# jie0530/act-plus-plus

Measured on AMD Instinct MI355X. Metric: policy steps/sec (4x480x640 cams, chunk=100, bs=8), higher is better.
Workload: dtype f32 (f16x3 split products: 3 fp16 MFMAs per fp32 product, fp32 accumulate); 1 GPU; ACT eval policy query: 4 cams 480x640 u8, chunk 100, hidden 512, ff 3200, 4 enc + 7 dec layers (layer 0 live), per-GPU batch 8, + temporal ensemble; per_gpu_batch=8, global_batch=8, parallelism=replicas x1

## Files before the change

act-plus-plus_amd/actmi/lib.py:

```python
import ctypes as C
import os

import torch

_HERE = os.path.dirname(os.path.abspath(__file__))
LIB_PATH = os.environ.get("ACTMI_LIB") or os.path.join(_HERE, "libactmi.so")

IMG_U8_NHWC = 0
IMG_F32_NCHW = 1


class ActmiConfig(C.Structure):
    _fields_ = [("struct_size", C.c_uint32)] + [(n, C.c_int32) for n in (
        "num_cams", "image_h", "image_w", "base_width", "hidden_dim", "nheads", "dim_feedforward", "enc_layers",
        "dec_layers", "num_queries", "state_dim", "action_dim", "latent_dim", "has_cvae_encoder", "max_batch",
        "enable_training")] + [("kl_weight", C.c_float)] + [(n, C.c_int32) for n in ("vq", "vq_class", "vq_dim")]


class ActmiPcdConfig(C.Structure):
    _fields_ = [("struct_size", C.c_uint32), ("max_points", C.c_int32), ("hidden_dim", C.c_int32), ("output_dim", C.c_int32)]


class GemmDesc(C.Structure):
    _fields_ = [
        ("A", C.c_void_p), ("lda", C.c_int64), ("mode", C.c_int32),
        ("H", C.c_int32), ("W", C.c_int32), ("Cin", C.c_int32), ("KH", C.c_int32), ("KW", C.c_int32),
        ("stride", C.c_int32), ("pad", C.c_int32), ("Ho", C.c_int32), ("Wo", C.c_int32),
        ("img_stride", C.c_int64),
        ("A_add", C.c_void_p), ("ld_add", C.c_int64), ("add_mod", C.c_int32), ("add_ncols", C.c_int32),
        ("Bw", C.c_void_p), ("ldb", C.c_int64),
        ("scale", C.c_void_p), ("bias", C.c_void_p), ("res", C.c_void_p), ("ldres", C.c_int64),
        ("res_mod", C.c_int32), ("relu", C.c_int32),
        ("C", C.c_void_p), ("ldc", C.c_int64), ("rowmap", C.c_void_p),
        ("M", C.c_int32), ("N", C.c_int32), ("K", C.c_int32), ("groups", C.c_int32),
        ("gA", C.c_int64), ("gB", C.c_int64), ("gSB", C.c_int64), ("gC", C.c_int64), ("gRes", C.c_int64),
        ("ta", C.c_int32), ("tb", C.c_int32), ("a_rowmap", C.c_void_p),
        ("B_add", C.c_void_p), ("ld_badd", C.c_int64), ("badd_mod", C.c_int32), ("splitk", C.c_int32),
        ("mask", C.c_void_p), ("ldmask", C.c_int64), ("C2", C.c_void_p), ("scale2", C.c_void_p),
        ("alpha", C.c_float), ("groups_inner", C.c_int32),
        ("gA2", C.c_int64), ("gB2", C.c_int64), ("gC2", C.c_int64), ("gRes2", C.c_int64),
        ("gMask", C.c_int64), ("gC2out", C.c_int64),
        ("drop_p", C.c_float), ("drop_seed", C.c_uint64), ("stamps", C.c_void_p), ("prec", C.c_int32), ("b_split", C.c_int32), ("b_scale", C.c_float), ("a_scale", C.c_float), ("a_scale_dev", C.c_void_p), ("b_scale_dev", C.c_void_p),
        ("split_stride", C.c_int64), ("amax_out", C.c_void_p),
        ("epi", C.c_int32), ("epi_scale", C.c_float), ("epi_row", C.c_void_p), ("gRow", C.c_int64), ("gRow2", C.c_int64),
        ("epi_colkill", C.c_void_p), ("gColkill", C.c_int64), ("tile_hint", C.c_int32),
        ("finite_flag", C.c_void_p), ("finite_bit", C.c_uint32),
        ("Ax", C.c_void_p), ("kx_begin", C.c_int32), ("Hx", C.c_int32), ("Wx", C.c_int32), ("Cx", C.c_int32),
        ("stride_x", C.c_int32), ("gAx", C.c_int64),
        ("A_alt", C.c_void_p), ("alt_ncols", C.c_int32), ("k_tap_inner", C.c_int32),
    ]


class AttnBwdDesc(C.Structure):
    _fields_ = [("q", C.c_void_p), ("k", C.c_void_p), ("v", C.c_void_p), ("o", C.c_void_p), ("d_o", C.c_void_p), ("lse", C.c_void_p),
                ("dq", C.c_void_p), ("dk", C.c_void_p), ("dv", C.c_void_p)] + \
               [(n, C.c_int64) for n in ("q_bs", "q_rs", "k_bs", "k_rs", "v_bs", "v_rs", "dq_bs", "dq_rs", "dk_bs", "dk_rs", "dv_bs", "dv_rs")] + \
               [("kpm", C.c_void_p), ("kpm_bs", C.c_int64)] + [(n, C.c_int32) for n in ("B", "H", "Nq", "Nk", "HD")] + \
               [("drop_p", C.c_float), ("drop_seed", C.c_uint64), ("delta_ws", C.c_void_p), ("do_scale", C.c_void_p), ("amax_out", C.c_void_p)]


class AttnDesc(C.Structure):
    _fields_ = [
        ("Q", C.c_void_p), ("q_bs", C.c_int64), ("q_rs", C.c_int64),
        ("K", C.c_void_p), ("k_bs", C.c_int64), ("k_rs", C.c_int64),
        ("V", C.c_void_p), ("v_bs", C.c_int64), ("v_rs", C.c_int64),
        ("O", C.c_void_p), ("o_bs", C.c_int64), ("o_rs", C.c_int64),
        ("kpm", C.c_void_p), ("kpm_bs", C.c_int64), ("lse", C.c_void_p),
        ("B", C.c_int32), ("H", C.c_int32), ("Nq", C.c_int32), ("Nk", C.c_int32), ("HD", C.c_int32),
        ("scale", C.c_float), ("ws", C.c_void_p), ("ws_floats", C.c_int64),
        ("drop_p", C.c_float), ("drop_seed", C.c_uint64), ("prec", C.c_int32), ("causal", C.c_int32),
    ]


_lib = None


def load():
    global _lib
    if _lib is not None:
        return _lib
    if not os.path.isfile(LIB_PATH):
        raise RuntimeError(
            f"{LIB_PATH} is missing: build the HIP extension first (python -c 'import __graft_entry__ as g; g.build()' "
            "or make -C act-plus-plus_amd/csrc). There is no CPU fallback for the ACT path.")
    lib = C.CDLL(LIB_PATH)
    vp, i32, i64, f32, f64 = C.c_void_p, C.c_int32, C.c_int64, C.c_float, C.c_double
    sigs = {
        "actmi_version": ([], i32),
        "actmi_create": ([C.POINTER(ActmiConfig), C.POINTER(vp)], i32),
        "actmi_create_ex": ([C.POINTER(ActmiConfig), C.POINTER(ActmiPcdConfig), C.POINTER(vp)], i32),
        "actmi_set_pointcloud": ([vp, vp, vp, i32, i32], i32),
        "actmi_destroy": ([vp], i32),
        "actmi_last_error": ([vp], C.c_char_p),
        "actmi_num_params": ([vp], i32),
        "actmi_param_info": ([vp, i32, C.POINTER(C.c_char_p), C.POINTER(i64), C.POINTER(i32), C.POINTER(i32)], i32),
        "actmi_set_param": ([vp, C.c_char_p, vp, C.POINTER(i64), i32, i32], i32),
        "actmi_get_param": ([vp, C.c_char_p, vp, i64, i32], i32),
        "actmi_param_ptr": ([vp, C.c_char_p, C.POINTER(vp), C.POINTER(i64)], i32),
        "actmi_finalize": ([vp, vp], i32),
        "actmi_set_forward_phase": ([vp, i32], i32),
        "actmi_forward_infer_vq": ([vp, vp, vp, i32, i32, vp, vp, vp], i32),
        "actmi_forward_infer": ([vp, vp, vp, i32, i32, vp, vp], i32),
        "actmi_forward_train": ([vp, vp, vp, i32, vp, vp, vp, C.c_uint64, f32, i32, vp, vp, vp, vp, vp], i32),
        "actmi_backward": ([vp, f32, vp], i32),
        "actmi_zero_grad": ([vp, vp], i32),
        "actmi_adamw_step": ([vp, f32, f32, f32, f32, f32, f32, i64, vp], i32),
        "actmi_adamw_step_range": ([vp, f32, f32, f32, f32, f32, f32, i64, i64, i64, vp], i32),
        "actmi_refresh_weights": ([vp, vp], i32),
        "actmi_param_arena": ([vp, C.POINTER(vp), C.POINTER(i64)], i32),
        "actmi_grad_ptr": ([vp, C.c_char_p, C.POINTER(vp), C.POINTER(i64)], i32),
        "actmi_grad_arena": ([vp, C.POINTER(vp), C.POINTER(i64)], i32),
        "actmi_grad_phase_range": ([vp, i32, C.POINTER(i64), C.POINTER(i64)], i32),
        "actmi_wait_grad_phase": ([vp, i32, vp], i32),
        "actmi_ensemble_step": ([vp, vp, vp, f64, vp, vp, i32, i32, i32, vp], i32),
        "actmi_op_gemm": ([C.POINTER(GemmDesc), vp], i32),
        "actmi_op_split16": ([vp, vp, C.c_int64, C.c_float, vp], i32),
        "actmi_op_permute_conv_k": ([vp, vp, C.c_int64, i32, i32, i32, vp], i32),
        "actmi_op_sample_onehot": ([vp, i32, i32, C.c_float, C.c_uint64, vp, vp, vp], i32),
        "actmi_op_pow2_scale": ([vp, C.c_int64, i32, i32, vp, vp], i32),
        "actmi_op_splitk_combine": ([vp, i32, C.c_int64, C.c_int64, i32, i32, vp, vp, vp, C.c_int64, i32, vp, C.c_int64, vp], i32),
        "actmi_op_attention": ([C.POINTER(AttnDesc), vp], i32),
        "actmi_op_attention_bwd": ([C.POINTER(AttnBwdDesc), vp], i32),
        "actmi_op_layernorm": ([vp, vp, i32, vp, vp, vp, vp, vp, i32, i32, f32, vp], i32),
        "actmi_op_maxpool3x3s2": ([vp, vp, i32, i32, i32, i32, vp], i32),
        "actmi_op_conv1": ([vp, i32, vp, vp, vp, vp, vp, i32, i32, i32, i32, i32, i32, vp], i32),
        "actmi_op_conv1_workspace_floats": ([i32, i32], C.c_int64),
        "actmi_op_conv1_prepare": ([vp, vp, i32, i32, i32, vp], i32),
        "actmi_op_conv1_prepared": ([vp, vp, vp, vp, vp, i32, i32, i32, i32, i32, i32, vp], i32),
        "actmi_op_conv3x3_c64": ([vp, vp, C.c_float, vp, vp, vp, vp, i32, i32, i32, i32, i32, vp], i32),
        "actmi_op_conv3x3_c64_dgrad": ([vp, vp, C.c_float, vp, vp, vp, vp, vp, vp, i32, i32, i32, i32, vp], i32),
        "actmi_op_wgrad7x7s2": ([vp, vp, vp, vp, C.c_int64, vp, i32, i32, i32, i32, vp], i32),
        "actmi_op_wgrad3x3_c64": ([vp, vp, vp, vp, C.c_int64, vp, i32, i32, i32, i32, vp], i32),
        "actmi_op_groupnorm": ([vp, vp, vp, vp, vp, vp, vp, i32, i32, i32, i32, f32, i32, i32, vp, C.c_int64, vp], i32),
        "actmi_op_spatial_softmax": ([vp, vp, i32, i32, i32, i32, f32, vp], i32),
        "actmi_op_unfold1d": ([vp, vp, i32, i32, i32, i32, i32, i32, i32, i32, vp], i32),
        "actmi_op_ddim_step": ([vp, vp, C.c_int64, f32, f32, f32, f32, i32, vp], i32),
        "actmi_op_mish": ([vp, vp, C.c_int64, vp], i32),
        "actmi_op_gelu": ([vp, vp, C.c_int64, vp], i32),
        "actmi_op_gelu_bwd": ([vp, vp, vp, C.c_int64, vp], i32),
        "actmi_op_dropout": ([vp, vp, C.c_int64, C.c_float, C.c_uint64, vp], i32),
        "actmi_op_small_attention": ([vp, vp, i32, i32, i32, i32, i32, C.c_float, C.c_uint64, vp], i32),
        "actmi_op_small_attention_bwd": ([vp, vp, vp, i32, i32, i32, i32, i32, C.c_float, C.c_uint64, vp], i32),
        "actmi_op_soft_ce_dim1": ([vp, vp, i32, i32, i32, vp, vp, vp, vp], i32),
        "actmi_op_argmax_l1": ([vp, vp, i32, i32, vp, vp, vp], i32),
        "actmi_op_layernorm_bwd": ([vp, vp, vp, vp, vp, vp, vp, i32, i32, C.c_float, vp, C.c_int64, vp], i32),
        "actmi_op_colsum": ([vp, C.c_int64, vp, i32, i32, vp, C.c_int64, vp], i32),
        "actmi_op_pcd_embed": ([vp, vp, vp, vp, vp, C.c_int64, i32, vp], i32),
        "actmi_op_colmax": ([vp, i32, i32, i32, C.c_int64, vp, vp, vp, C.c_int64, vp], i32),
        "actmi_op_sum_batch": ([vp, C.c_int64, C.c_int64, vp, i32, i32, i32, i32, vp], i32),
        "actmi_op_adamw": ([vp, vp, vp, vp, C.c_int64, C.c_float, C.c_float, C.c_float, C.c_float, C.c_float, C.c_int64, vp], i32),
        "actmi_op_u8_to_nhwc4": ([vp, vp, i32, i32, i32, i32, vp], i32),
        "actmi_op_last_error": ([], C.c_char_p),
        "actmi_debug_tensor": ([vp, C.c_char_p, C.POINTER(vp), C.POINTER(i64)], i32),
        "actmi_debug_stop_after": ([vp, C.c_char_p], i32),
        "actmi_set_gemm_prec": ([vp, i32], i32),
        "actmi_set_train_prec": ([vp, i32], i32),
        "actmi_get_flags": ([vp, C.POINTER(C.c_uint32), i32, vp], i32),
        "actmi_flags_ptr": ([vp, C.POINTER(vp)], i32),
        "actmi_profile_enable": ([i32], i32),
        "actmi_profile_reset": ([], i32),
        "actmi_profile_report": ([C.c_char_p, i32], i32),
    }
    for name, (args, res) in sigs.items():
        fn = getattr(lib, name)
        fn.argtypes = args
        fn.restype = res
    _lib = lib
    return lib


def declared_symbols(header_path):
    import re
    txt = open(header_path).read()
    return sorted(set(re.findall(r"\b(actmi_[a-z0-9_]+)\s*\(", txt)))


def current_stream_ptr():
    return C.c_void_p(torch.cuda.current_stream().cuda_stream)


def check(rc, handle=None, what=""):
    if rc != 0:
        lib = load()
        msg = lib.actmi_last_error(handle) if handle is not None else lib.actmi_op_last_error()
        raise RuntimeError(f"libactmi {what} failed (code {rc}): {msg.decode() if msg else ''}")


def profile_enable(on: bool):
    lib = load()
    lib.actmi_profile_reset() if on else None
    lib.actmi_profile_enable(1 if on else 0)


def profile_report():
    import json
    lib = load()
    buf = C.create_string_buffer(1 << 18)
    rc = lib.actmi_profile_report(buf, len(buf))
    if rc != 0:
        raise RuntimeError(f"actmi_profile_report failed ({rc})")
    return json.loads(buf.value.decode())
```

act-plus-plus_amd/actmi/ops.py:

```python
import ctypes as C

import torch

from . import lib as L


def _p(t):
    return C.c_void_p(t.data_ptr()) if t is not None else C.c_void_p(0)


PREC = {None: 0, "f32": 1, "f16x3": 2, "bf16": 3}


def split16(w, scale=1.0):
    lib = L.load()
    w = w.contiguous()
    out = torch.empty_like(w)
    L.check(lib.actmi_op_split16(_p(w), _p(out), w.numel(), float(scale), L.current_stream_ptr()), None, "op_split16")
    return out


def permute_conv_k(w_rows, taps, cin):
    lib = L.load()
    w_rows = w_rows.contiguous()
    out = torch.empty_like(w_rows)
    rows, ld = w_rows.numel() // w_rows.shape[-1], w_rows.shape[-1]
    L.check(lib.actmi_op_permute_conv_k(_p(w_rows), _p(out), rows, int(taps), int(cin), int(ld), L.current_stream_ptr()), None,
            "op_permute_conv_k")
    return out


def pow2_scale(x):
    lib = L.load()
    assert x.dim() == 2 and x.stride(1) == 1
    out = torch.zeros(2, dtype=torch.float32, device=x.device)
    L.check(lib.actmi_op_pow2_scale(_p(x), x.stride(0), x.shape[0], x.shape[1], _p(out), L.current_stream_ptr()), None,
            "op_pow2_scale")
    return out


def auto_splitk(M, N, K):
    tiles = ((M + 63) // 64) * ((N + 63) // 64)
    nk = (K + 31) // 32
    if tiles >= 768 or nk < 24:
        return 0
    s = min(8, (1536 + tiles - 1) // tiles, nk // 12)
    while s >= 2 and (s - 1) * ((nk + s - 1) // s) >= nk:
        s -= 1
    return s if s >= 2 else 0


def gemm(A, W, bias=None, scale=None, res=None, res_mod=0, relu=False, a_add=None, add_mod=0, add_ncols=0, rowmap=None,
         out=None, out_rows=None, drop_p=0.0, drop_seed=0, prec=None, w_split=False, a_scale=0.0, b_scale=0.0,
         a_scale_dev=None, b_scale_dev=None, splitk=0):
    lib = L.load()
    M, K = A.shape
    N = W.shape[0]
    if splitk == "auto":
        splitk = auto_splitk(M, N, K) if (rowmap is None and not res_mod and not drop_p and N % 4 == 0 and a_scale_dev is None
                                          and b_scale_dev is None) else 0
    if splitk and splitk > 1:
        assert rowmap is None and not res_mod and not drop_p
        part = torch.empty((splitk, M, N), dtype=torch.float32, device=A.device)
        d = L.GemmDesc()
        d.A, d.lda, d.mode = A.data_ptr(), A.stride(0), 0
        if a_add is not None:
            d.A_add, d.ld_add, d.add_mod, d.add_ncols = a_add.data_ptr(), a_add.stride(0), add_mod, add_ncols
        d.Bw, d.ldb = W.data_ptr(), W.stride(0)
        d.C, d.ldc = part.data_ptr(), N
        d.M, d.N, d.K, d.groups = M, N, K, 1
        d.splitk, d.split_stride = int(splitk), M * N
        d.prec, d.b_split, d.b_scale = PREC[prec], 1 if w_split else 0, float(w_split) if w_split else float(b_scale)
        d.a_scale = float(a_scale)
        L.check(lib.actmi_op_gemm(C.byref(d), L.current_stream_ptr()), None, "op_gemm")
        if out is None:
            out = torch.empty((M, N), dtype=torch.float32, device=A.device)
        L.check(lib.actmi_op_splitk_combine(part.data_ptr(), int(splitk), M * N, N, M, N, _p(scale), _p(bias), _p(res),
                                            res.stride(0) if res is not None else 0,
                                            2 if relu == "gelu" else (1 if relu else 0), out.data_ptr(), out.stride(0),
                                            L.current_stream_ptr()), None, "op_splitk_combine")
        return out
    if out is None:
        out = torch.zeros((out_rows or M, N), dtype=torch.float32, device=A.device)
    d = L.GemmDesc()
    d.A, d.lda, d.mode = A.data_ptr(), A.stride(0), 0
    if a_add is not None:
        d.A_add, d.ld_add, d.add_mod, d.add_ncols = a_add.data_ptr(), a_add.stride(0), add_mod, add_ncols
    d.Bw, d.ldb = W.data_ptr(), W.stride(0)
    d.scale = scale.data_ptr() if scale is not None else None
    d.bias = bias.data_ptr() if bias is not None else None
    if res is not None:
        d.res, d.ldres, d.res_mod = res.data_ptr(), res.stride(0), res_mod
    d.relu = 2 if relu == "gelu" else (1 if relu else 0)
    d.C, d.ldc = out.data_ptr(), out.stride(0)
    d.rowmap = rowmap.data_ptr() if rowmap is not None else None
    d.M, d.N, d.K, d.groups = M, N, K, 1
    d.drop_p, d.drop_seed = float(drop_p), int(drop_seed)
    d.prec, d.b_split, d.b_scale = PREC[prec], 1 if w_split else 0, float(w_split) if w_split else float(b_scale)
    d.a_scale = float(a_scale)
    d.a_scale_dev = a_scale_dev.data_ptr() if a_scale_dev is not None else None
    d.b_scale_dev = b_scale_dev.data_ptr() if b_scale_dev is not None else None
    L.check(lib.actmi_op_gemm(C.byref(d), L.current_stream_ptr()), None, "op_gemm")
    return out


def conv2d_with_second_source(y1, x, wf_split, w_scale, bias, stride_x=2, relu=True, splitk=0, k_tap_inner=False):
    lib = L.load()
    G, B, H, W, Cc = y1.shape
    _, _, Hx, Wx, Cx = x.shape
    Cout = wf_split.shape[1]
    Kf = 9 * Cc + Cx
    assert wf_split.numel() == G * Cout * Kf
    M = B * H * W

    def desc(C_ptr, ldc, gC):
        d = L.GemmDesc()
        d.A, d.mode = y1.data_ptr(), 1
        d.H, d.W, d.Cin, d.KH, d.KW, d.stride, d.pad, d.Ho, d.Wo = H, W, Cc, 3, 3, 1, 1, H, W
        d.img_stride = H * W * Cc
        d.Ax, d.kx_begin, d.Hx, d.Wx, d.Cx, d.stride_x, d.gAx = x.data_ptr(), 9 * Cc, Hx, Wx, Cx, stride_x, B * Hx * Wx * Cx
        d.Bw, d.ldb = wf_split.data_ptr(), Kf
        d.C, d.ldc = C_ptr, ldc
        d.M, d.N, d.K, d.groups = M, Cout, Kf, G
        d.gA, d.gB, d.gSB, d.gC = B * H * W * Cc, Cout * Kf, Cout, gC
        d.prec, d.b_split, d.b_scale = PREC["f16x3"], 1, float(w_scale)
        d.k_tap_inner = 1 if k_tap_inner else 0
        return d
    out = torch.empty((G, B, H, W, Cout), dtype=torch.float32, device=y1.device)
    if splitk and splitk > 1:
        part = torch.empty((G, splitk, M, Cout), dtype=torch.float32, device=y1.device)
        d = desc(part.data_ptr(), Cout, splitk * M * Cout)
        d.splitk, d.split_stride = int(splitk), M * Cout
        L.check(lib.actmi_op_gemm(C.byref(d), L.current_stream_ptr()), None, "op_gemm(conv + second source, split)")
        for g in range(G):
            L.check(lib.actmi_op_splitk_combine(part[g].data_ptr(), int(splitk), M * Cout, Cout, M, Cout, None, _p(bias[g]), None, 0,
                                                1 if relu else 0, out[g].data_ptr(), Cout, L.current_stream_ptr()), None, "combine")
        return out
    d = desc(out.data_ptr(), Cout, M * Cout)
    d.bias = bias.data_ptr()
    d.relu = 1 if relu else 0
    L.check(lib.actmi_op_gemm(C.byref(d), L.current_stream_ptr()), None, "op_gemm(conv + second source)")
    return out


def conv2d_nhwc(x, w_ohwi, scale=None, bias=None, res=None, relu=False, stride=1, pad=1, prec=None, w_split=False, b_scale=0.0,
                k_tap_inner=False):
    lib = L.load()
    G, B, H, W, Cin = x.shape
    _, Cout, KH, KW, _ = w_ohwi.shape
    Ho, Wo = (H + 2 * pad - KH) // stride + 1, (W + 2 * pad - KW) // stride + 1
    out = torch.empty((G, B, Ho, Wo, Cout), dtype=torch.float32, device=x.device)
    d = L.GemmDesc()
    d.A, d.mode = x.data_ptr(), 1
    d.H, d.W, d.Cin, d.KH, d.KW, d.stride, d.pad, d.Ho, d.Wo = H, W, Cin, KH, KW, stride, pad, Ho, Wo
    d.img_stride = H * W * Cin
    d.Bw, d.ldb = w_ohwi.data_ptr(), KH * KW * Cin
    d.scale = scale.data_ptr() if scale is not None else None
    d.bias = bias.data_ptr() if bias is not None else None
    if res is not None:
        d.res, d.ldres = res.data_ptr(), Cout
    d.relu = 1 if relu else 0
    d.C, d.ldc = out.data_ptr(), Cout
    d.M, d.N, d.K, d.groups = B * Ho * Wo, Cout, KH * KW * Cin, G
    d.gA, d.gB, d.gSB = B * H * W * Cin, Cout * KH * KW * Cin, Cout
    d.gC = d.gRes = B * Ho * Wo * Cout
    d.prec, d.b_split, d.b_scale = PREC[prec], 1 if w_split else 0, float(w_split) if w_split else float(b_scale)
    d.k_tap_inner = 1 if k_tap_inner else 0
    L.check(lib.actmi_op_gemm(C.byref(d), L.current_stream_ptr()), None, "op_gemm(conv)")
    return out


def sample_onehot(logits, temperature=1.0, seed=0, want_probs=False):
    lib = L.load()
    logits = logits.contiguous()
    n, V = logits.shape
    code = torch.empty_like(logits)
    probs = torch.empty_like(logits) if want_probs else None
    L.check(lib.actmi_op_sample_onehot(_p(logits), n, V, float(temperature), C.c_uint64(int(seed)), _p(probs), _p(code),
                                       L.current_stream_ptr()), None, "op_sample_onehot")
    return (code, probs) if want_probs else code


def conv1_prepare(w_oihw, lut_mode=1):
    lib = L.load()
    w_oihw = w_oihw.contiguous()
    Cc, Cout = w_oihw.shape[0], w_oihw.shape[1]
    ws = torch.zeros(int(lib.actmi_op_conv1_workspace_floats(Cc, Cout)), dtype=torch.float32, device=w_oihw.device)
    L.check(lib.actmi_op_conv1_prepare(_p(w_oihw), _p(ws), Cc, Cout, int(lut_mode), L.current_stream_ptr()), None, "op_conv1_prepare")
    return ws


def conv1_prepared(image_u8, ws, Cout, relu=False, scale=None, bias=None):
    lib = L.load()
    image_u8 = image_u8.contiguous()
    B, Cc, H, W, _ = image_u8.shape
    out = torch.empty((Cc, B, (H - 1) // 2 + 1, (W - 1) // 2 + 1, Cout), dtype=torch.float32, device=image_u8.device)
    L.check(lib.actmi_op_conv1_prepared(_p(image_u8), _p(ws), _p(scale), _p(bias), _p(out), B, Cc, H, W, Cout, 1 if relu else 0,
                                        L.current_stream_ptr()), None, "op_conv1_prepared")
    return out


def conv3x3_c64(x, w_ohwi, scale=None, bias=None, res=None, relu=False, w_scale=256.0, w16=None):
    lib = L.load()
    G, B, H, W, Cin = x.shape
    assert Cin == 64 and tuple(w_ohwi.shape[1:]) == (64, 3, 3, 64)
    out = torch.empty_like(x)
    if w16 is None:
        w16 = split16(w_ohwi, w_scale)
    scale = scale if scale is not None else torch.ones(G, 64, device=x.device)
    bias = bias if bias is not None else torch.zeros(G, 64, device=x.device)
    L.check(lib.actmi_op_conv3x3_c64(_p(x.contiguous()), _p(w16), float(w_scale), _p(scale.contiguous()), _p(bias.contiguous()),
                                     _p(res), _p(out), G, B, H, W, 1 if relu else 0, L.current_stream_ptr()), None,
            "op_conv3x3_c64")
    return out


def conv3x3_c64_dgrad(dy, wd_ohwi, dy_scale=None, res=None, mask=None, post_scale=None, amax_out=None, w_scale=256.0):
    lib = L.load()
    G, B, H, W, Cc = dy.shape
    assert Cc == 64 and tuple(wd_ohwi.shape[1:]) == (64, 3, 3, 64)
    dy = dy.contiguous()
    dx = torch.empty_like(dy)
    for t in (res, mask):
        assert t is None or (t.shape == dy.shape and t.is_contiguous())
    assert post_scale is None or (tuple(post_scale.shape) == (G, 64) and post_scale.is_contiguous())
    w16 = split16(wd_ohwi, w_scale)
    L.check(lib.actmi_op_conv3x3_c64_dgrad(_p(dy), _p(w16), float(w_scale), _p(dy_scale), _p(res),
                                           _p(mask), _p(post_scale), _p(amax_out), _p(dx), G, B, H, W, L.current_stream_ptr()),
            None, "op_conv3x3_c64_dgrad")
    return dx


def wgrad3x3_c64(dy, x, dy_scale=None):
    G, B, H, W, Cc = x.shape
    assert Cc == 64 and dy.shape == x.shape
    nwg = max(1, min(256 // G, B * ((W + 31) // 32)))
    ws = torch.empty(G * nwg * 64 * 576, device=x.device, dtype=torch.float32)
    dw = torch.empty(G, 64, 3, 3, 64, device=x.device, dtype=torch.float32)
    lib = L.load()
    L.check(lib.actmi_op_wgrad3x3_c64(_p(dy.contiguous()), _p(x.contiguous()), _p(dw), _p(ws), ws.numel(),
                                      _p(dy_scale) if dy_scale is not None else None, G, B, H, W, L.current_stream_ptr()),
            None, "op_wgrad3x3_c64")
    return dw


def wgrad7x7s2(dy, x4, dy_scale=None):
    G, B, H, W, Cc = x4.shape
    Ho, Wo = (H - 1) // 2 + 1, (W - 1) // 2 + 1
    assert Cc == 4 and tuple(dy.shape) == (G, B, Ho, Wo, 64)
    nwg = max(1, min(512 // G, B * ((Wo + 31) // 32)))
    ws = torch.empty(G * nwg * 64 * 196, device=x4.device, dtype=torch.float32)
    dw = torch.empty(G, 64, 7, 7, 4, device=x4.device, dtype=torch.float32)
    lib = L.load()
    L.check(lib.actmi_op_wgrad7x7s2(_p(dy.contiguous()), _p(x4.contiguous()), _p(dw), _p(ws), ws.numel(),
                                    _p(dy_scale) if dy_scale is not None else None, G, B, H, W, L.current_stream_ptr()),
            None, "op_wgrad7x7s2")
    return dw



def attention(q, k, v, nheads, kpm=None, q_shared=False, want_lse=False, split=True, drop_p=0.0, drop_seed=0, prec=None,
              causal=False):
    lib = L.load()
    B, Nk, D = k.shape
    Nq = q.shape[-2]
    hd = D // nheads
    out = torch.zeros((B, Nq, D), dtype=torch.float32, device=k.device)
    lse = torch.zeros((B, nheads, Nq), dtype=torch.float32, device=k.device) if want_lse else None
    d = L.AttnDesc()
    d.Q, d.q_bs, d.q_rs = q.data_ptr(), (0 if q_shared else q.stride(0)), q.stride(-2)
    d.K, d.k_bs, d.k_rs = k.data_ptr(), k.stride(0), k.stride(1)
    d.V, d.v_bs, d.v_rs = v.data_ptr(), v.stride(0), v.stride(1)
    d.O, d.o_bs, d.o_rs = out.data_ptr(), out.stride(0), out.stride(1)
    if kpm is not None:
        d.kpm, d.kpm_bs = kpm.data_ptr(), kpm.stride(0)
    d.lse = lse.data_ptr() if lse is not None else None
    if split:
        ws = torch.empty(8 * B * Nq * (D + 2 * nheads), dtype=torch.float32, device=k.device)
        d.ws, d.ws_floats = ws.data_ptr(), ws.numel()
    d.B, d.H, d.Nq, d.Nk, d.HD = B, nheads, Nq, Nk, hd
    d.scale = 1.0 / (hd ** 0.5)
    d.drop_p, d.drop_seed = float(drop_p), int(drop_seed)
    d.prec = PREC[prec]
    d.causal = 1 if causal else 0
    L.check(lib.actmi_op_attention(C.byref(d), L.current_stream_ptr()), None, "op_attention")
    return (out, lse) if want_lse else out


def attention_bwd(q, k, v, out, lse, dout, nheads, kpm=None, drop_p=0.0, drop_seed=0, do_scale=None, want_amax=False):
    lib = L.load()
    B, Nk, D = k.shape
    Nq = q.shape[1]
    dq = torch.empty((B, Nq, D), dtype=torch.float32, device=k.device)
    dk = torch.empty((B, Nk, D), dtype=torch.float32, device=k.device)
    dv = torch.empty((B, Nk, D), dtype=torch.float32, device=k.device)
    ws = torch.empty(B * nheads * Nq, dtype=torch.float32, device=k.device)
    amax = torch.zeros(1, dtype=torch.int32, device=k.device) if want_amax else None
    d = L.AttnBwdDesc()
    d.q, d.q_bs, d.q_rs = q.data_ptr(), q.stride(0), q.stride(1)
    d.k, d.k_bs, d.k_rs = k.data_ptr(), k.stride(0), k.stride(1)
    d.v, d.v_bs, d.v_rs = v.data_ptr(), v.stride(0), v.stride(1)
    d.o, d.d_o, d.lse = out.data_ptr(), dout.data_ptr(), lse.data_ptr()
    d.dq, d.dq_bs, d.dq_rs = dq.data_ptr(), dq.stride(0), dq.stride(1)
    d.dk, d.dk_bs, d.dk_rs = dk.data_ptr(), dk.stride(0), dk.stride(1)
    d.dv, d.dv_bs, d.dv_rs = dv.data_ptr(), dv.stride(0), dv.stride(1)
    if kpm is not None:
        d.kpm, d.kpm_bs = kpm.data_ptr(), kpm.stride(0)
    d.B, d.H, d.Nq, d.Nk, d.HD = B, nheads, Nq, Nk, D // nheads
    d.drop_p, d.drop_seed = float(drop_p), int(drop_seed)
    d.delta_ws = ws.data_ptr()
    d.do_scale = do_scale.data_ptr() if do_scale is not None else None
    d.amax_out = amax.data_ptr() if amax is not None else None
    L.check(lib.actmi_op_attention_bwd(C.byref(d), L.current_stream_ptr()), None, "op_attention_bwd")
    return (dq, dk, dv, amax) if want_amax else (dq, dk, dv)


def layernorm(x, w, b, res=None, res_mod=0, w2=None, b2=None, eps=1e-5):
    lib = L.load()
    M, D = x.shape
    y = torch.empty_like(x)
    L.check(lib.actmi_op_layernorm(_p(x), _p(res), res_mod, _p(w), _p(b), _p(w2), _p(b2), _p(y), M, D, eps,
                                   L.current_stream_ptr()), None, "op_layernorm")
    return y


def maxpool3x3s2(x):
    lib = L.load()
    n, H, W, Cc = x.shape
    Ho, Wo = (H + 2 - 3) // 2 + 1, (W + 2 - 3) // 2 + 1
    y = torch.empty((n, Ho, Wo, Cc), dtype=torch.float32, device=x.device)
    L.check(lib.actmi_op_maxpool3x3s2(_p(x), _p(y), n, H, W, Cc, L.current_stream_ptr()), None, "op_maxpool")
    return y


def conv1(image, w_oihw, scale, bias, prec=None):
    lib = L.load()
    image = image.contiguous()
    if image.dtype == torch.uint8:
        B, Cn, H, W, _ = image.shape
        fmt = L.IMG_U8_NHWC
    else:
        B, Cn, _, H, W = image.shape
        fmt = L.IMG_F32_NCHW
    Cout = w_oihw.shape[1]
    Ho, Wo = (H + 6 - 7) // 2 + 1, (W + 6 - 7) // 2 + 1
    out = torch.zeros((Cn, B, Ho, Wo, Cout), dtype=torch.float32, device=image.device)
    ws = torch.empty(Cn * Cout * 148 + 768, dtype=torch.float32, device=image.device)
    L.check(lib.actmi_op_conv1(_p(image), fmt, _p(w_oihw), _p(scale), _p(bias), _p(out), _p(ws), B, Cn, H, W, Cout,
                               PREC[prec], L.current_stream_ptr()), None, "op_conv1")
    return out


ACT = {None: 0, "none": 0, "relu": 1, "mish": 2}


_GN_WS = {}


def groupnorm(x, weight, bias, groups, eps=1e-5, act=None, res=None, res_after=False, film=None, out=None):
    lib = L.load()
    x = x.contiguous()
    n, Cc = x.shape[0], x.shape[-1]
    P = x.numel() // (n * Cc)
    if out is None:
        out = torch.empty_like(x)
    assert out.is_contiguous() and out.shape == x.shape
    fs, fb = (film[0].contiguous(), film[1].contiguous()) if film is not None else (None, None)
    rm = 0 if res is None else (2 if res_after else 1)
    key = (x.device, torch.cuda.current_stream(x.device).cuda_stream)
    ws = _GN_WS.get(key)
    if ws is None:
        ws = _GN_WS[key] = torch.empty(1 << 20, dtype=torch.float32, device=x.device)
    L.check(lib.actmi_op_groupnorm(_p(x), _p(res.contiguous() if res is not None else None), _p(fs), _p(fb), _p(weight), _p(bias),
                                   _p(out), n, P, Cc, int(groups), float(eps), ACT[act], rm, _p(ws), ws.numel(),
                                   L.current_stream_ptr()), None, "op_groupnorm")
    return out


def spatial_softmax(logits, H, W, temperature=1.0):
    lib = L.load()
    logits = logits.contiguous()
    n, P, K = logits.shape
    assert P == H * W
    out = torch.empty((n, K, 2), dtype=torch.float32, device=logits.device)
    L.check(lib.actmi_op_spatial_softmax(_p(logits), _p(out), n, H, W, K, float(temperature), L.current_stream_ptr()), None,
            "op_spatial_softmax")
    return out


def unfold1d(x, k, stride=1, pad=0, transposed=False):
    lib = L.load()
    x = x.contiguous()
    B, T, Cc = x.shape
    To = (T - 1) * stride - 2 * pad + k if transposed else (T + 2 * pad - k) // stride + 1
    out = torch.empty((B, To, k * Cc), dtype=torch.float32, device=x.device)
    L.check(lib.actmi_op_unfold1d(_p(x), _p(out), B, T, Cc, k, stride, pad, To, 1 if transposed else 0, L.current_stream_ptr()),
            None, "op_unfold1d")
    return out


def ddim_step(x, eps, alpha_t, alpha_prev, clip=True):
    lib = L.load()
    assert x.is_contiguous() and eps.is_contiguous() and x.numel() == eps.numel()
    L.check(lib.actmi_op_ddim_step(_p(x), _p(eps), x.numel(), float(alpha_t ** -0.5), float((1.0 - alpha_t) ** 0.5),
                                   float(alpha_prev ** 0.5), float(max(0.0, 1.0 - alpha_prev) ** 0.5), 1 if clip else 0,
                                   L.current_stream_ptr()), None, "op_ddim_step")
    return x


def mish(x):
    lib = L.load()
    x = x.contiguous()
    y = torch.empty_like(x)
    L.check(lib.actmi_op_mish(_p(x), _p(y), x.numel(), L.current_stream_ptr()), None, "op_mish")
    return y


def u8_to_nhwc4(image_u8):
    lib = L.load()
    image_u8 = image_u8.contiguous()
    B, Cam, H, W, _ = image_u8.shape
    out = torch.empty((Cam, B, H, W, 4), dtype=torch.float32, device=image_u8.device)
    L.check(lib.actmi_op_u8_to_nhwc4(_p(image_u8), _p(out), B, Cam, H, W, L.current_stream_ptr()), None, "op_u8_to_nhwc4")
    return out


def gemm_t(A, Bm, ta=False, tb=False, bias=None, res=None, out=None, prec="f32"):
    lib = L.load()
    if ta:
        K, M = A.shape
    else:
        M, K = A.shape
    N = Bm.shape[1] if tb else Bm.shape[0]
    assert (Bm.shape[0] if tb else Bm.shape[1]) == K, (A.shape, Bm.shape, ta, tb)
    if out is None:
        out = torch.empty((M, N), dtype=torch.float32, device=A.device)
    d = L.GemmDesc()
    d.A, d.lda, d.mode, d.ta = A.data_ptr(), A.stride(0), 0, 1 if ta else 0
    d.Bw, d.ldb, d.tb = Bm.data_ptr(), Bm.stride(0), 1 if tb else 0
    d.bias = bias.data_ptr() if bias is not None else None
    if res is not None:
        d.res, d.ldres = res.data_ptr(), res.stride(0)
    d.C, d.ldc = out.data_ptr(), out.stride(0)
    d.M, d.N, d.K, d.groups = M, N, K, 1
    d.prec = PREC[prec]
    L.check(lib.actmi_op_gemm(C.byref(d), L.current_stream_ptr()), None, "op_gemm")
    return out


def gelu(x):
    y = torch.empty_like(x)
    L.check(L.load().actmi_op_gelu(_p(x), _p(y), x.numel(), L.current_stream_ptr()), None, "op_gelu")
    return y


def gelu_bwd(x, dy):
    dx = torch.empty_like(x)
    L.check(L.load().actmi_op_gelu_bwd(_p(x), _p(dy), _p(dx), x.numel(), L.current_stream_ptr()), None, "op_gelu_bwd")
    return dx


def dropout(x, p, seed):
    y = torch.empty_like(x)
    L.check(L.load().actmi_op_dropout(_p(x), _p(y), x.numel(), float(p), int(seed), L.current_stream_ptr()), None, "op_dropout")
    return y


def small_attention(qkv, nheads, causal=True, drop_p=0.0, seed=0):
    n, T, D3 = qkv.shape
    D = D3 // 3
    out = torch.empty((n, T, D), dtype=torch.float32, device=qkv.device)
    L.check(L.load().actmi_op_small_attention(_p(qkv), _p(out), n, T, nheads, D // nheads, 1 if causal else 0, float(drop_p), int(seed),
                                              L.current_stream_ptr()), None, "op_small_attention")
    return out


def small_attention_bwd(qkv, dout, nheads, causal=True, drop_p=0.0, seed=0):
    n, T, D3 = qkv.shape
    D = D3 // 3
    dqkv = torch.empty_like(qkv)
    L.check(L.load().actmi_op_small_attention_bwd(_p(qkv), _p(dout), _p(dqkv), n, T, nheads, D // nheads, 1 if causal else 0,
                                                  float(drop_p), int(seed), L.current_stream_ptr()), None, "op_small_attention_bwd")
    return dqkv


def soft_ce_dim1(logits, target, want_grad=True):
    B, T, V = logits.shape
    loss = torch.empty(1, dtype=torch.float32, device=logits.device)
    ws = torch.empty(B * V, dtype=torch.float32, device=logits.device)
    dl = torch.empty_like(logits) if want_grad else None
    L.check(L.load().actmi_op_soft_ce_dim1(_p(logits), _p(target), B, T, V, _p(loss), _p(dl), _p(ws), L.current_stream_ptr()), None,
            "op_soft_ce_dim1")
    return loss, dl


def argmax_l1(logits, target):
    V = logits.shape[-1]
    rows = logits.numel() // V
    out = torch.empty(1, dtype=torch.float32, device=logits.device)
    ws = torch.empty(rows, dtype=torch.float32, device=logits.device)
    L.check(L.load().actmi_op_argmax_l1(_p(logits), _p(target), rows, V, _p(out), _p(ws), L.current_stream_ptr()), None, "op_argmax_l1")
    return out


def layernorm_bwd(x, w, dy, dw, db, ws, dx_add=None, eps=1e-5):
    M, D = x.shape
    dx = torch.empty_like(x)
    L.check(L.load().actmi_op_layernorm_bwd(_p(x), _p(w), _p(dy), _p(dx_add), _p(dx), _p(dw), _p(db), M, D, eps, _p(ws), ws.numel(),
                                            L.current_stream_ptr()), None, "op_layernorm_bwd")
    return dx


def colsum(src, out, ws):
    M, N = src.shape
    L.check(L.load().actmi_op_colsum(_p(src), src.stride(0), _p(out), M, N, _p(ws), ws.numel(), L.current_stream_ptr()), None, "op_colsum")


def pcd_embed(xyz, rgb, w0, b0):
    xyz, rgb = xyz.contiguous().view(-1, 3), rgb.contiguous().view(-1, 3)
    rows, H = xyz.shape[0], w0.shape[0]
    out = torch.empty((rows, H), dtype=torch.float32, device=xyz.device)
    L.check(L.load().actmi_op_pcd_embed(_p(xyz), _p(rgb), _p(w0.contiguous()), _p(b0.contiguous()), _p(out), rows, H,
                                        L.current_stream_ptr()), None, "op_pcd_embed")
    return out


def colmax(x, O=None, split=True):
    B, P, ld = x.shape
    O = ld if O is None else O
    out = torch.empty((B, O), dtype=torch.float32, device=x.device)
    arg = torch.empty((B, O), dtype=torch.int32, device=x.device)
    ws = torch.empty(2 * B * 64 * O, dtype=torch.float32, device=x.device) if split else None
    L.check(L.load().actmi_op_colmax(_p(x), B, P, O, ld, _p(out), _p(arg), _p(ws), ws.numel() if split else 0,
                                     L.current_stream_ptr()), None, "op_colmax")
    return out, arg


def sum_batch(src, dst, accumulate=False):
    B, Rr, D = src.shape
    L.check(L.load().actmi_op_sum_batch(_p(src), src.stride(0), src.stride(1), _p(dst), B, Rr, D, 1 if accumulate else 0,
                                        L.current_stream_ptr()), None, "op_sum_batch")


def adamw(p, g, m, v, lr, weight_decay, step, betas=(0.9, 0.999), eps=1e-8):
    L.check(L.load().actmi_op_adamw(_p(p), _p(g), _p(m), _p(v), p.numel(), float(lr), float(weight_decay), float(betas[0]),
                                    float(betas[1]), float(eps), int(step), L.current_stream_ptr()), None, "op_adamw")


class TemporalEnsemble:

    def __init__(self, num_episodes, num_queries, action_dim=16, k=0.01, device="cuda:0"):
        self.E, self.Q, self.A, self.k = num_episodes, num_queries, action_dim, float(k)
        self.ring = torch.zeros((self.E, self.Q, self.Q, self.A), dtype=torch.float32, device=device)
        self.t = torch.zeros((self.E,), dtype=torch.int32, device=device)
        self.out = torch.zeros((self.E, self.A), dtype=torch.float64, device=device)
        self.populated = torch.zeros((self.E, self.Q), dtype=torch.uint8, device=device)

    def reset(self):
        self.ring.zero_()
        self.t.zero_()

    def step(self, all_actions):
        lib = L.load()
        a = all_actions.contiguous()
        dev = self.ring.device
        if a.device != dev:
            raise ValueError(f"all_actions lives on {a.device} but this ensemble is bound to {dev}")
        with torch.cuda.device(dev):
            L.check(lib.actmi_ensemble_step(_p(self.ring), _p(self.t), _p(a), self.k, _p(self.out), _p(self.populated),
                                            self.E, self.Q, self.A, L.current_stream_ptr()), None, "ensemble_step")
        return self.out
```

act-plus-plus_amd/csrc/attn.hip:

```cpp
#include "common.h"
#include "dropout.h"
#include "split16.h"
#include <cstdio>
#include <cstdlib>

namespace {

constexpr bool ATTN_NOPF = true;
constexpr int KT = 64;
typedef _Float16 h16x8 __attribute__((ext_vector_type(8)));

__device__ __forceinline__ void attn_block_coords(int& bx, int& by, int& bz) {
    const int gx = gridDim.x, gy = gridDim.y;
    const int total = gx * gy * (int)gridDim.z;
    const int lin = ((int)blockIdx.z * gy + (int)blockIdx.y) * gx + (int)blockIdx.x;
    const int xcd = lin & 7, q = total >> 3, r = total & 7;
    const int base = (xcd < r) ? xcd * (q + 1) : r * (q + 1) + (xcd - r) * q;
    const int flat = base + (lin >> 3);
    bx = flat % gx;
    const int rest = flat / gx;
    by = rest % gy;
    bz = rest / gy;
}

template <int HD>
__global__ __launch_bounds__(256) void attn_f32_kernel(AttnArgs p, int nsplit, int chunk) {
    constexpr int HH = HD / 2;
    constexpr int DT = (HD + 31) / 32;
    constexpr int VD = DT * 32;
    constexpr int KS = HD + 4;
    __shared__ __attribute__((aligned(16))) float s_k[KT * KS];
    __shared__ __attribute__((aligned(16))) float s_v[KT * VD];

    const int t = threadIdx.x, lane = t & 63, wave = t >> 6;
    const int li = lane & 31, lh = lane >> 5;
    int bx, h, b;
    attn_block_coords(bx, h, b);
    const int split = bx % nsplit;
    const int q = (bx / nsplit) * 128 + wave * 32 + li;
    const int k_begin = split * chunk;
    const int k_end = (k_begin + chunk < p.Nk) ? k_begin + chunk : p.Nk;
    const bool qok = q < p.Nq;

    const float qscale = p.scale * 1.4426950408889634f;
    const float* Qp = p.Q + (int64_t)b * p.q_bs + (int64_t)(qok ? q : 0) * p.q_rs + h * HD + lh * HH;
    float qreg[HH];
#pragma unroll
    for (int s = 0; s < HH; s += 4) {
        f32x4 v = *reinterpret_cast<const f32x4*>(Qp + s);
#pragma unroll
        for (int j = 0; j < 4; ++j) qreg[s + j] = qok ? v[j] * qscale : 0.f;
    }
    const float* Kb = p.K + (int64_t)b * p.k_bs + h * HD;
    const float* Vb = p.V + (int64_t)b * p.v_bs + h * HD;
    const uint8_t* kpm = p.kpm ? p.kpm + (int64_t)b * p.kpm_bs : nullptr;

    f32x16 O[DT];
#pragma unroll
    for (int d = 0; d < DT; ++d)
#pragma unroll
        for (int e = 0; e < 16; ++e) O[d][e] = 0.f;
    float m_run = -INFINITY, l_run = 0.f;

    if (HD < VD) {
        for (int e = t; e < KT * VD; e += 256) s_v[e] = 0.f;
        __syncthreads();
    }

    __shared__ uint8_t s_dead[KT];
    constexpr int C4 = HD / 4;
    constexpr int NLD = (KT * C4 + 255) / 256;
    f32x4 pk[NLD], pv[NLD];
    auto fetch = [&](int kt0) {
#pragma unroll
        for (int i = 0; i < NLD; ++i) {
            const int e = t + 256 * i;
            const int kr = e / C4, c = e - kr * C4;
            const int key = kt0 + kr;
            const bool ok = e < KT * C4 && key < k_end;
            const int64_t koff = ok ? (int64_t)key * p.k_rs + c * 4 : 0;
            const int64_t voff = ok ? (int64_t)key * p.v_rs + c * 4 : 0;
            const f32x4 kv = *reinterpret_cast<const f32x4*>(Kb + koff);
            const f32x4 vv = *reinterpret_cast<const f32x4*>(Vb + voff);
            const f32x4 z = {0.f, 0.f, 0.f, 0.f};
            pk[i] = ok ? kv : z;
            pv[i] = ok ? vv : z;
        }
    };
    fetch(k_begin);
    for (int kt0 = k_begin; kt0 < k_end; kt0 += KT) {
#pragma unroll
        for (int i = 0; i < NLD; ++i) {
            const int e = t + 256 * i;
            if (e < KT * C4) {
                const int kr = e / C4, c = e - kr * C4;
                *reinterpret_cast<f32x4*>(&s_k[kr * KS + c * 4]) = pk[i];
                *reinterpret_cast<f32x4*>(&s_v[kr * VD + c * 4]) = pv[i];
            }
        }
        const bool ragged = kt0 + KT > k_end || kpm != nullptr;
        if (ragged && t < KT) {
            const int key = kt0 + t;
            s_dead[t] = (key >= k_end) || (kpm && kpm[key] != 0);
        }
        __syncthreads();
        if (kt0 + KT < k_end) fetch(kt0 + KT);
#pragma unroll
        for (int sub = 0; sub < KT / 32; ++sub) {
            const int kb = kt0 + sub * 32;
            if (kb < k_end) {
                f32x16 S;
#pragma unroll
                for (int e = 0; e < 16; ++e) S[e] = 0.f;
                const float* krow = &s_k[(sub * 32 + li) * KS + lh * HH];
#pragma unroll
                for (int s = 0; s < HH; s += 4) {
                    const f32x4 kv = *reinterpret_cast<const f32x4*>(krow + s);
#pragma unroll
                    for (int j = 0; j < 4; ++j)
                        S = __builtin_amdgcn_mfma_f32_32x32x2f32(kv[j], qreg[s + j], S, 0, 0, 0);
                }
                if (ragged) {
#pragma unroll
                    for (int e = 0; e < 16; ++e)
                        if (s_dead[sub * 32 + (e & 3) + 8 * (e >> 2) + 4 * lh]) S[e] = -INFINITY;
                }
                if (p.causal) {
#pragma unroll
                    for (int e = 0; e < 16; ++e)
                        if (kb + (e & 3) + 8 * (e >> 2) + 4 * lh > q) S[e] = -INFINITY;
                }
                float mt = S[0];
#pragma unroll
                for (int e = 1; e < 16; ++e) mt = fmaxf(mt, S[e]);
                mt = fmaxf(mt, __shfl_xor(mt, 32, 64));
                const float m_new = fmaxf(m_run, mt);
                const float m_safe = (m_new == -INFINITY) ? 0.f : m_new;
                const float alpha = __builtin_amdgcn_exp2f(m_run - m_safe);
                float rs = 0.f;
#pragma unroll
                for (int e = 0; e < 16; ++e) {
                    S[e] = __builtin_amdgcn_exp2f(S[e] - m_safe);
                    rs += S[e];
                }
                rs += __shfl_xor(rs, 32, 64);
                l_run = l_run * alpha + rs;
                m_run = m_new;
                if (p.drop_p > 0.f) {
                    const float ds = 1.f / (1.f - p.drop_p);
                    const uint64_t rowbase = (((uint64_t)b * p.H + h) * p.Nq + (qok ? q : 0)) * (uint64_t)p.Nk;
#pragma unroll
                    for (int e = 0; e < 16; ++e) {
                        const int key = kb + (e & 3) + 8 * (e >> 2) + 4 * lh;
                        S[e] = actmi_keep(p.drop_seed, rowbase + key, p.drop_p) ? S[e] * ds : 0.f;
                    }
                }
#pragma unroll
                for (int d = 0; d < DT; ++d)
#pragma unroll
                    for (int e = 0; e < 16; ++e) O[d][e] *= alpha;
#pragma unroll
                for (int e = 0; e < 16; ++e) {
                    const int kl = sub * 32 + (e & 3) + 8 * (e >> 2) + 4 * lh;
#pragma unroll
                    for (int d = 0; d < DT; ++d) {
                        const float vv = s_v[kl * VD + d * 32 + li];
                        O[d] = __builtin_amdgcn_mfma_f32_32x32x2f32(vv, S[e], O[d], 0, 0, 0);
                    }
                }
            }
        }
        __syncthreads();
    }
    if (qok) {
        if (nsplit == 1) {
            const float inv = 1.f / l_run;
            float* Op = p.O + (int64_t)b * p.o_bs + (int64_t)q * p.o_rs + h * HD;
#pragma unroll
            for (int d = 0; d < DT; ++d)
#pragma unroll
                for (int g = 0; g < 4; ++g) {
                    const int d0 = d * 32 + 8 * g + 4 * lh;
                    if (d0 < HD) {
                        f32x4 o = {O[d][4 * g] * inv, O[d][4 * g + 1] * inv, O[d][4 * g + 2] * inv, O[d][4 * g + 3] * inv};
                        *reinterpret_cast<f32x4*>(Op + d0) = o;
                    }
                }
            if (p.lse && lh == 0) p.lse[((int64_t)b * p.H + h) * p.Nq + q] = m_run * 0.6931471805599453f + logf(l_run);
        } else {
            const int64_t row = (((int64_t)split * p.B + b) * p.H + h) * p.Nq + q;
            float* Op = p.ws + row * HD;
            float* ml = p.ws + (int64_t)nsplit * p.B * p.H * p.Nq * HD + row * 2;
#pragma unroll
            for (int d = 0; d < DT; ++d)
#pragma unroll
                for (int g = 0; g < 4; ++g) {
                    const int d0 = d * 32 + 8 * g + 4 * lh;
                    if (d0 < HD) {
                        f32x4 o = {O[d][4 * g], O[d][4 * g + 1], O[d][4 * g + 2], O[d][4 * g + 3]};
                        *reinterpret_cast<f32x4*>(Op + d0) = o;
                    }
                }
            if (lh == 0) { ml[0] = m_run; ml[1] = l_run; }
        }
    }
}

template <int HD>
__global__ __launch_bounds__(256, 3) void attn_f16x3_kernel(AttnArgs p, int nsplit, int chunk) {
    constexpr int NS = HD / 16;
    constexpr int DT = (HD + 31) / 32;
    constexpr int VD = DT * 32;
    constexpr int KROW = 4 * HD + 16;
    constexpr int VROW = 4 * KT + 16;
    __shared__ __attribute__((aligned(16))) unsigned char s_k[KT * KROW];
    __shared__ __attribute__((aligned(16))) unsigned char s_vt[VD * VROW];
    __shared__ uint8_t s_dead[KT];

    const int t = threadIdx.x, lane = t & 63, wave = t >> 6;
    const int li = lane & 31, lh = lane >> 5;
    int bx, h, b;
    attn_block_coords(bx, h, b);
    const int split = bx % nsplit;
    const int q = (bx / nsplit) * 128 + wave * 32 + li;
    const int k_begin = split * chunk;
    const int k_end = (k_begin + chunk < p.Nk) ? k_begin + chunk : p.Nk;
    const bool qok = q < p.Nq;

    const float qscale = p.scale * 1.4426950408889634f;
    const float* Qp = p.Q + (int64_t)b * p.q_bs + (int64_t)(qok ? q : 0) * p.q_rs + h * HD + lh * 8;
    h16x8 qh[NS], ql[NS];
#pragma unroll
    for (int s = 0; s < NS; ++s) {
        f32x4 v0 = *reinterpret_cast<const f32x4*>(Qp + s * 16);
        f32x4 v1 = *reinterpret_cast<const f32x4*>(Qp + s * 16 + 4);
        const float sc = qok ? qscale : 0.f;
        v0 *= sc; v1 *= sc;
        uint2 h0, l0, h1, l1;
        split16(v0, h0, l0);
        split16(v1, h1, l1);
        qh[s] = __builtin_bit_cast(h16x8, uint4{h0.x, h0.y, h1.x, h1.y});
        ql[s] = __builtin_bit_cast(h16x8, uint4{l0.x, l0.y, l1.x, l1.y});
    }
    const float* Kb = p.K + (int64_t)b * p.k_bs + h * HD;
    const float* Vb = p.V + (int64_t)b * p.v_bs + h * HD;
    const uint8_t* kpm = p.kpm ? p.kpm + (int64_t)b * p.kpm_bs : nullptr;

    f32x16 O[DT];
#pragma unroll
    for (int d = 0; d < DT; ++d)
#pragma unroll
        for (int e = 0; e < 16; ++e) O[d][e] = 0.f;
    float m_run = -INFINITY, l_run = 0.f;

    if (HD < VD) {
        for (int e = t; e < VD * VROW / 4; e += 256) reinterpret_cast<uint32_t*>(s_vt)[e] = 0u;
        __syncthreads();
    }

    constexpr int C4 = HD / 4;
    constexpr int NLK = (KT * C4 + 255) / 256;
    constexpr int NLV = (KT / 2 * C4 + 255) / 256;
    f32x4 pk[NLK], pv[NLV][2];
    auto vc = [&](int e) { return ((e >> 5) % (C4 / 4)) * 4 + (e & 3); };
    auto vkp = [&](int e) { return ((e >> 5) / (C4 / 4)) * 8 + ((e >> 2) & 7); };
    auto fetch = [&](int kt0) {
        const f32x4 z = {0.f, 0.f, 0.f, 0.f};
#pragma unroll
        for (int i = 0; i < NLK; ++i) {
            const int e = t + 256 * i;
            const int kr = e / C4, c = e - kr * C4;
            const int key = kt0 + kr;
            const bool ok = e < KT * C4 && key < k_end;
            const f32x4 kv = *reinterpret_cast<const f32x4*>(Kb + (ok ? (int64_t)key * p.k_rs + c * 4 : 0));
            pk[i] = ok ? kv : z;
        }
#pragma unroll
        for (int i = 0; i < NLV; ++i) {
            const int e = t + 256 * i;
            const int kp = vkp(e), c = vc(e);
#pragma unroll
            for (int u = 0; u < 2; ++u) {
                const int key = kt0 + 2 * kp + u;
                const bool ok = e < KT / 2 * C4 && key < k_end;
                const f32x4 vv = *reinterpret_cast<const f32x4*>(Vb + (ok ? (int64_t)key * p.v_rs + c * 4 : 0));
                pv[i][u] = ok ? vv : z;
            }
        }
    };
    if (!ATTN_NOPF) fetch(k_begin);
    for (int kt0 = k_begin; kt0 < k_end; kt0 += KT) {
        if (ATTN_NOPF) fetch(kt0);
#pragma unroll
        for (int i = 0; i < NLK; ++i) {
            const int e = t + 256 * i;
            if (e < KT * C4) {
                const int kr = e / C4, c = e - kr * C4;
                uint2 hi, lo;
                split16(pk[i], hi, lo);
                *reinterpret_cast<uint2*>(s_k + kr * KROW + c * 8) = hi;
                *reinterpret_cast<uint2*>(s_k + kr * KROW + 2 * HD + c * 8) = lo;
            }
        }
#pragma unroll
        for (int i = 0; i < NLV; ++i) {
            const int e = t + 256 * i;
            if (e < KT / 2 * C4) {
                const int kp = vkp(e), c = vc(e);
                uint2 ha, la, hb, lb;
                split16(pv[i][0], ha, la);
                split16(pv[i][1], hb, lb);
                const int kl = 2 * kp, r = kl & 15;
                const int pos = (kl & ~15) | (r & 3) | ((r & 8) >> 1) | ((r & 4) << 1);
                unsigned char* dst = s_vt + (c * 4) * VROW + pos * 2;
                *reinterpret_cast<uint32_t*>(dst + 0 * VROW) = (ha.x & 0xffffu) | (hb.x << 16);
                *reinterpret_cast<uint32_t*>(dst + 1 * VROW) = (ha.x >> 16) | (hb.x & 0xffff0000u);
                *reinterpret_cast<uint32_t*>(dst + 2 * VROW) = (ha.y & 0xffffu) | (hb.y << 16);
                *reinterpret_cast<uint32_t*>(dst + 3 * VROW) = (ha.y >> 16) | (hb.y & 0xffff0000u);
                *reinterpret_cast<uint32_t*>(dst + 0 * VROW + 2 * KT) = (la.x & 0xffffu) | (lb.x << 16);
                *reinterpret_cast<uint32_t*>(dst + 1 * VROW + 2 * KT) = (la.x >> 16) | (lb.x & 0xffff0000u);
                *reinterpret_cast<uint32_t*>(dst + 2 * VROW + 2 * KT) = (la.y & 0xffffu) | (lb.y << 16);
                *reinterpret_cast<uint32_t*>(dst + 3 * VROW + 2 * KT) = (la.y >> 16) | (lb.y & 0xffff0000u);
            }
        }
        const bool ragged = kt0 + KT > k_end || kpm != nullptr;
        if (ragged && t < KT) {
            const int key = kt0 + t;
            s_dead[t] = (key >= k_end) || (kpm && kpm[key] != 0);
        }
        __syncthreads();
        if (!ATTN_NOPF && kt0 + KT < k_end) fetch(kt0 + KT);
#pragma unroll
        for (int sub = 0; sub < KT / 32; ++sub) {
            const int kb = kt0 + sub * 32;
            if (kb < k_end) {
                f32x16 S;
#pragma unroll
                for (int e = 0; e < 16; ++e) S[e] = 0.f;
                const unsigned char* krow = s_k + (sub * 32 + li) * KROW + lh * 16;
#pragma unroll
                for (int s = 0; s < NS; ++s) {
                    const h16x8 kh = __builtin_bit_cast(h16x8, *reinterpret_cast<const f32x4*>(krow + s * 32));
                    const h16x8 kl = __builtin_bit_cast(h16x8, *reinterpret_cast<const f32x4*>(krow + 2 * HD + s * 32));
                    S = __builtin_amdgcn_mfma_f32_32x32x16_f16(kl, qh[s], S, 0, 0, 0);
                    S = __builtin_amdgcn_mfma_f32_32x32x16_f16(kh, ql[s], S, 0, 0, 0);
                    S = __builtin_amdgcn_mfma_f32_32x32x16_f16(kh, qh[s], S, 0, 0, 0);
                }
                if (ragged) {
#pragma unroll
                    for (int e = 0; e < 16; ++e)
                        if (s_dead[sub * 32 + (e & 3) + 8 * (e >> 2) + 4 * lh]) S[e] = -INFINITY;
                }
                if (p.causal) {
#pragma unroll
                    for (int e = 0; e < 16; ++e)
                        if (kb + (e & 3) + 8 * (e >> 2) + 4 * lh > q) S[e] = -INFINITY;
                }
                float mt = S[0];
#pragma unroll
                for (int e = 1; e < 16; ++e) mt = fmaxf(mt, S[e]);
                mt = fmaxf(mt, __shfl_xor(mt, 32, 64));
                const float m_new = fmaxf(m_run, mt);
                const float m_safe = (m_new == -INFINITY) ? 0.f : m_new;
                const float alpha = __builtin_amdgcn_exp2f(m_run - m_safe);
                float rs = 0.f;
#pragma unroll
                for (int e = 0; e < 16; ++e) {
                    S[e] = __builtin_amdgcn_exp2f(S[e] - m_safe);
                    rs += S[e];
                }
                rs += __shfl_xor(rs, 32, 64);
                l_run = l_run * alpha + rs;
                m_run = m_new;
                if (p.drop_p > 0.f) {
                    const float ds = 1.f / (1.f - p.drop_p);
                    const uint64_t rowbase = (((uint64_t)b * p.H + h) * p.Nq + (qok ? q : 0)) * (uint64_t)p.Nk;
#pragma unroll
                    for (int e = 0; e < 16; ++e) {
                        const int key = kb + (e & 3) + 8 * (e >> 2) + 4 * lh;
                        S[e] = actmi_keep(p.drop_seed, rowbase + key, p.drop_p) ? S[e] * ds : 0.f;
                    }
                }
                h16x8 ph[2], pl[2];
#pragma unroll
                for (int g2 = 0; g2 < 2; ++g2) {
                    const f32x4 a0 = {S[8 * g2], S[8 * g2 + 1], S[8 * g2 + 2], S[8 * g2 + 3]};
                    const f32x4 a1 = {S[8 * g2 + 4], S[8 * g2 + 5], S[8 * g2 + 6], S[8 * g2 + 7]};
                    uint2 h0, l0, h1, l1;
                    split16(a0, h0, l0);
                    split16(a1, h1, l1);
                    ph[g2] = __builtin_bit_cast(h16x8, uint4{h0.x, h0.y, h1.x, h1.y});
                    pl[g2] = __builtin_bit_cast(h16x8, uint4{l0.x, l0.y, l1.x, l1.y});
                }
#pragma unroll
                for (int d = 0; d < DT; ++d) {
#pragma unroll
                    for (int e = 0; e < 16; ++e) O[d][e] *= alpha;
                    const unsigned char* vrow = s_vt + (d * 32 + li) * VROW + sub * 64 + lh * 16;
#pragma unroll
                    for (int g2 = 0; g2 < 2; ++g2) {
                        const h16x8 vh = __builtin_bit_cast(h16x8, *reinterpret_cast<const f32x4*>(vrow + g2 * 32));
                        const h16x8 vl = __builtin_bit_cast(h16x8, *reinterpret_cast<const f32x4*>(vrow + 2 * KT + g2 * 32));
                        O[d] = __builtin_amdgcn_mfma_f32_32x32x16_f16(vl, ph[g2], O[d], 0, 0, 0);
                        O[d] = __builtin_amdgcn_mfma_f32_32x32x16_f16(vh, pl[g2], O[d], 0, 0, 0);
                        O[d] = __builtin_amdgcn_mfma_f32_32x32x16_f16(vh, ph[g2], O[d], 0, 0, 0);
                    }
                }
            }
        }
        __syncthreads();
    }
    if (qok) {
        if (nsplit == 1) {
            const float inv = 1.f / l_run;
            float* Op = p.O + (int64_t)b * p.o_bs + (int64_t)q * p.o_rs + h * HD;
#pragma unroll
            for (int d = 0; d < DT; ++d)
#pragma unroll
                for (int g = 0; g < 4; ++g) {
                    const int d0 = d * 32 + 8 * g + 4 * lh;
                    if (d0 < HD) {
                        f32x4 o = {O[d][4 * g] * inv, O[d][4 * g + 1] * inv, O[d][4 * g + 2] * inv, O[d][4 * g + 3] * inv};
                        *reinterpret_cast<f32x4*>(Op + d0) = o;
                    }
                }
            if (p.lse && lh == 0) p.lse[((int64_t)b * p.H + h) * p.Nq + q] = m_run * 0.6931471805599453f + logf(l_run);
        } else {
            const int64_t row = (((int64_t)split * p.B + b) * p.H + h) * p.Nq + q;
            float* Op = p.ws + row * HD;
            float* ml = p.ws + (int64_t)nsplit * p.B * p.H * p.Nq * HD + row * 2;
#pragma unroll
            for (int d = 0; d < DT; ++d)
#pragma unroll
                for (int g = 0; g < 4; ++g) {
                    const int d0 = d * 32 + 8 * g + 4 * lh;
                    if (d0 < HD) {
                        f32x4 o = {O[d][4 * g], O[d][4 * g + 1], O[d][4 * g + 2], O[d][4 * g + 3]};
                        *reinterpret_cast<f32x4*>(Op + d0) = o;
                    }
                }
            if (lh == 0) { ml[0] = m_run; ml[1] = l_run; }
        }
    }
}


__global__ void attn_combine_kernel(AttnArgs p, int nsplit, int HD) {
    const int64_t idx = (int64_t)blockIdx.x * blockDim.x + threadIdx.x;
    const int D4 = HD / 4;
    const int64_t total = (int64_t)p.B * p.H * p.Nq * D4;
    if (idx >= total) return;
    const int d4 = (int)(idx % D4);
    const int64_t bhq = idx / D4;
    const int q = (int)(bhq % p.Nq);
    const int h = (int)((bhq / p.Nq) % p.H);
    const int b = (int)(bhq / ((int64_t)p.Nq * p.H));
    const int64_t per = (int64_t)p.B * p.H * p.Nq;
    const float* mlb = p.ws + (int64_t)nsplit * per * HD;
    float m = -INFINITY;
    for (int s = 0; s < nsplit; ++s) m = fmaxf(m, mlb[(s * per + bhq) * 2]);
    const float msafe = (m == -INFINITY) ? 0.f : m;
    float L = 0.f;
    f32x4 acc = {0.f, 0.f, 0.f, 0.f};
    for (int s = 0; s < nsplit; ++s) {
        const float w = __builtin_amdgcn_exp2f(mlb[(s * per + bhq) * 2] - msafe);
        L += mlb[(s * per + bhq) * 2 + 1] * w;
        acc += *reinterpret_cast<const f32x4*>(p.ws + (s * per + bhq) * HD + d4 * 4) * w;
    }
    const float inv = 1.f / L;
    *reinterpret_cast<f32x4*>(p.O + (int64_t)b * p.o_bs + (int64_t)q * p.o_rs + h * HD + d4 * 4) = acc * inv;
    if (p.lse && d4 == 0) p.lse[bhq] = msafe * 0.6931471805599453f + logf(L);
}

}

int launch_attention(const AttnArgs& a, hipStream_t st, std::string* err) {
    auto fail = [&](const char* m) { if (err) *err = std::string("attention: ") + m; return -2; };
    if (a.B <= 0 || a.Nq <= 0) return 0;
    if (a.Nk <= 0) return fail("Nk must be positive");
    if (a.causal && a.Nq != a.Nk) return fail("causal needs Nq == Nk");
    if ((a.q_rs & 3) || (a.k_rs & 3) || (a.v_rs & 3) || (a.o_rs & 3) || (a.q_bs & 3) || (a.k_bs & 3) || (a.v_bs & 3) ||
        (a.o_bs & 3))
        return fail("strides must be multiples of 4 floats");
    if (((uintptr_t)a.Q & 15) || ((uintptr_t)a.K & 15) || ((uintptr_t)a.V & 15) || ((uintptr_t)a.O & 15))
        return fail("pointers must be 16-byte aligned");
    static const int env_prec = env_gemm_prec(ACTMI_PREC_F32);
    const int prec = a.prec ? a.prec : env_prec;
    if (prec != ACTMI_PREC_F32 && prec != ACTMI_PREC_F16X3) return fail("bad prec");
    const bool f16 = prec == ACTMI_PREC_F16X3;
    const int qblocks = (a.Nq + 127) / 128;
    const int tiles = (a.Nk + KT - 1) / KT;
    int nsplit = 1;
    if (a.ws) {
        const long blocks = (long)qblocks * a.H * a.B;
        static const long target = getenv("ACTMI_ATTN_SPLIT_TARGET") ? atol(getenv("ACTMI_ATTN_SPLIT_TARGET")) : 1024;
        nsplit = (int)((target + blocks - 1) / blocks);
        if (nsplit < 1) nsplit = 1;
        if (nsplit > 8) nsplit = 8;
        if (nsplit > tiles / 2) nsplit = tiles / 2 > 0 ? tiles / 2 : 1;
        while (nsplit > 1 && (int64_t)nsplit * a.B * a.Nq * ((int64_t)a.H * a.HD + 2 * a.H) > a.ws_floats) --nsplit;
    }
    const int chunk = ((tiles + nsplit - 1) / nsplit) * KT;
    dim3 grid(qblocks * nsplit, a.H, a.B);
    if (prof_enabled()) {
        char nm[48];
        snprintf(nm, sizeof(nm), "attn_%s_kernel<%d>", f16 ? "f16x3" : "f32", a.HD);
        prof_begin(nm, 4.0 * a.B * a.H * (double)a.Nq * a.Nk * a.HD,
                   4.0 * a.B * a.H * a.HD * (2.0 * a.Nq + 2.0 * a.Nk), st);
    }
    if (f16) {
        switch (a.HD) {
            case 64: hipLaunchKernelGGL(attn_f16x3_kernel<64>, grid, dim3(256), 0, st, a, nsplit, chunk); break;
            case 32: hipLaunchKernelGGL(attn_f16x3_kernel<32>, grid, dim3(256), 0, st, a, nsplit, chunk); break;
            case 16: hipLaunchKernelGGL(attn_f16x3_kernel<16>, grid, dim3(256), 0, st, a, nsplit, chunk); break;
            default: return fail("head_dim must be 16, 32 or 64");
        }
    } else
    switch (a.HD) {
        case 64: hipLaunchKernelGGL(attn_f32_kernel<64>, grid, dim3(256), 0, st, a, nsplit, chunk); break;
        case 32: hipLaunchKernelGGL(attn_f32_kernel<32>, grid, dim3(256), 0, st, a, nsplit, chunk); break;
        case 16: hipLaunchKernelGGL(attn_f32_kernel<16>, grid, dim3(256), 0, st, a, nsplit, chunk); break;
        default: return fail("head_dim must be 16, 32 or 64");
    }
    if (nsplit > 1) {
        const int64_t total = (int64_t)a.B * a.H * a.Nq * (a.HD / 4);
        hipLaunchKernelGGL(attn_combine_kernel, dim3((unsigned)((total + 255) / 256)), dim3(256), 0, st, a, nsplit, a.HD);
    }
    prof_end(st);
    hipError_t e = hipGetLastError();
    if (e != hipSuccess) { if (err) *err = std::string("attention launch: ") + hipGetErrorString(e); return -3; }
    return 0;
}
```

act-plus-plus_amd/csrc/engine.hip:

```cpp
#include "engine.h"

#include <algorithm>
#include <cmath>
#include <cstdio>
#include <cstring>

namespace {

thread_local std::string g_create_error;

int conv_out(int x, int k, int s, int p) { return (x + 2 * p - k) / s + 1; }

void add_param(actmi_ctx* c, const std::string& key, std::vector<int64_t> shape, bool is_buffer) {
    Param p;
    p.key = key;
    p.shape = shape;
    p.numel = 1;
    for (auto d : shape) p.numel *= d;
    p.off = c->ptotal;
    p.is_buffer = is_buffer;
    c->ptotal += (p.numel + 63) & ~int64_t(63);
    c->index[key] = (int)c->params.size();
    c->params.push_back(p);
}

void add_mha(actmi_ctx* c, const std::string& p, int D) {
    add_param(c, p + "in_proj_weight", {3 * D, D}, false);
    add_param(c, p + "in_proj_bias", {3 * D}, false);
    add_param(c, p + "out_proj.weight", {D, D}, false);
    add_param(c, p + "out_proj.bias", {D}, false);
}

void add_ffn_norms(actmi_ctx* c, const std::string& p, int D, int F, int nnorm) {
    add_param(c, p + "linear1.weight", {F, D}, false);
    add_param(c, p + "linear1.bias", {F}, false);
    add_param(c, p + "linear2.weight", {D, F}, false);
    add_param(c, p + "linear2.bias", {D}, false);
    for (int i = 1; i <= nnorm; ++i) {
        add_param(c, p + "norm" + std::to_string(i) + ".weight", {D}, false);
        add_param(c, p + "norm" + std::to_string(i) + ".bias", {D}, false);
    }
}

void add_fbn(actmi_ctx* c, const std::string& p, int n) {
    for (const char* s : {"weight", "bias", "running_mean", "running_var"}) add_param(c, p + s, {n}, true);
}

void build_spec(actmi_ctx* c) {
    const actmi_config& g = c->cfg;
    const int D = g.hidden_dim, F = g.dim_feedforward, Q = g.num_queries, S = g.state_dim, A = g.action_dim,
              L = g.latent_dim, w0 = g.base_width;
    add_param(c, "pos_table", {1, Q + 2, D}, true);
    for (int i = 0; i < g.enc_layers; ++i) {
        std::string p = "transformer.encoder.layers." + std::to_string(i) + ".";
        add_mha(c, p + "self_attn.", D);
        add_ffn_norms(c, p, D, F, 2);
    }
    for (int i = 0; i < g.dec_layers; ++i) {
        std::string p = "transformer.decoder.layers." + std::to_string(i) + ".";
        add_mha(c, p + "self_attn.", D);
        add_mha(c, p + "multihead_attn.", D);
        add_ffn_norms(c, p, D, F, 3);
    }
    add_param(c, "transformer.decoder.norm.weight", {D}, false);
    add_param(c, "transformer.decoder.norm.bias", {D}, false);
    if (g.has_cvae_encoder) {
        for (int i = 0; i < g.enc_layers; ++i) {
            std::string p = "encoder.layers." + std::to_string(i) + ".";
            add_mha(c, p + "self_attn.", D);
            add_ffn_norms(c, p, D, F, 2);
        }
    }
    add_param(c, "action_head.weight", {A, D}, false);
    add_param(c, "action_head.bias", {A}, false);
    add_param(c, "is_pad_head.weight", {1, D}, false);
    add_param(c, "is_pad_head.bias", {1}, false);
    add_param(c, "query_embed.weight", {Q, D}, false);
    add_param(c, "input_proj.weight", {D, 8 * w0, 1, 1}, false);
    add_param(c, "input_proj.bias", {D}, false);
    for (int cam = 0; cam < g.num_cams; ++cam) {
        std::string p = "backbones." + std::to_string(cam) + ".0.body.";
        add_param(c, p + "conv1.weight", {w0, 3, 7, 7}, false);
        add_fbn(c, p + "bn1.", w0);
        int cin = w0;
        for (int li = 1; li <= 4; ++li) {
            const int cout = w0 << (li - 1);
            for (int bi = 0; bi < 2; ++bi) {
                std::string bp = p + "layer" + std::to_string(li) + "." + std::to_string(bi) + ".";
                add_param(c, bp + "conv1.weight", {cout, cin, 3, 3}, false);
                add_fbn(c, bp + "bn1.", cout);
                add_param(c, bp + "conv2.weight", {cout, cout, 3, 3}, false);
                add_fbn(c, bp + "bn2.", cout);
                if (bi == 0 && li > 1) {
                    add_param(c, bp + "downsample.0.weight", {cout, cin, 1, 1}, false);
                    add_fbn(c, bp + "downsample.1.", cout);
                }
                cin = cout;
            }
        }
    }
    add_param(c, "input_proj_robot_state.weight", {D, S}, false);
    add_param(c, "input_proj_robot_state.bias", {D}, false);
    if (c->has_pcd) {
        add_param(c, "input_proj_pointnet.weight", {D, c->pcd.output_dim}, false);
        add_param(c, "input_proj_pointnet.bias", {D}, false);
    }
    add_param(c, "cls_embed.weight", {1, D}, false);
    add_param(c, "encoder_action_proj.weight", {D, A}, false);
    add_param(c, "encoder_action_proj.bias", {D}, false);
    add_param(c, "encoder_joint_proj.weight", {D, S}, false);
    add_param(c, "encoder_joint_proj.bias", {D}, false);
    const int Lp = g.vq ? g.vq_class * g.vq_dim : 2 * L, Li = g.vq ? g.vq_class * g.vq_dim : L;
    add_param(c, "latent_proj.weight", {Lp, D}, false);
    add_param(c, "latent_proj.bias", {Lp}, false);
    add_param(c, "latent_out_proj.weight", {D, Li}, false);
    add_param(c, "latent_out_proj.bias", {D}, false);
    if (c->has_pcd) {
        const int Hp = c->pcd.hidden_dim, Op = c->pcd.output_dim;
        const int idx[4] = {0, 3, 6, 9}, nout[4] = {Hp, Hp, Hp, Op}, nin[4] = {6, Hp, Hp, Hp};
        for (int i = 0; i < 4; ++i) {
            const std::string p = "pcl_backbone.pointnet._mlp." + std::to_string(idx[i]) + ".";
            add_param(c, p + "weight", {nout[i], nin[i]}, false);
            add_param(c, p + "bias", {nout[i]}, false);
        }
    }
    add_param(c, "additional_pos_embed.weight", {c->n_extra, D}, false);
}

}

int dev_alloc_bytes(actmi_ctx* ctx, void** p, size_t bytes) {
    hipError_t e = hipMalloc(p, (bytes + 15) & ~(size_t)15);
    if (e != hipSuccess) {
        ctx->err = std::string("hipMalloc: ") + hipGetErrorString(e);
        return ACTMI_E_NOMEM;
    }
    ctx->allocs.push_back(*p);
    return 0;
}

int ctx_gemm(actmi_ctx* ctx, GemmArgs a, hipStream_t st, int ws_half, LnFuse* ln) {
    if (ln) ln->done = false;
    a.prec = engine_prec(ctx);
    const int64_t ws_part = (ctx->splitk_ws_floats / ctx->nbranch) & ~(int64_t)3;
    float* const ws = ctx->splitk_ws ? ctx->splitk_ws + (ws_half > 0 ? ws_half * ws_part : 0) : nullptr;
    const int64_t ws_floats = ws_half >= 0 ? ws_part : ctx->splitk_ws_floats;
    if (a.prec == ACTMI_PREC_F16X3 && a.tb == 0 && !a.b_split && a.Bw >= ctx->pbase && a.Bw < ctx->pbase + ctx->ptotal) {
        a.b_scale = engine_weight_scale(ctx, a.Bw);
        a.Bw = ctx->p16base + (a.Bw - ctx->pbase);
        a.b_split = 1;
    }
    constexpr int sk_target = 1536, sk_minnk = 12, sk_maxtiles = 768;
    constexpr int sk_target_long = 4864, sk_maxtiles_long = 1300, sk_long_nk = 128;
    if (ctx->fwd_splitk && ctx->splitk_ws && a.splitk <= 1 && a.tb == 0 && a.ta == 0 && (a.mode == 0 || a.mode == 1) &&
        !a.rowmap && !a.C2 && !a.mask && a.drop_p == 0.f && a.res_mod == 0 && a.groups_inner == 0 && !a.stamps) {
        const int groups = a.groups > 0 ? a.groups : 1;
        const int64_t tiles = (int64_t)((a.M + 63) / 64) * ((a.N + 63) / 64) * groups * (ws_half >= 0 ? ctx->policy_mult : 1);
        const int nk = (a.K + 31) / 32;
        int S = tiles < sk_maxtiles ? (int)((sk_target + tiles - 1) / tiles) : 1;
        if (S == 1 && tiles < sk_maxtiles_long && nk >= sk_long_nk) S = (int)((sk_target_long + tiles - 1) / tiles);
        if (ln && S == 1 && ctx->ln_split > 1 && nk >= 64 && tiles < 2 * sk_maxtiles) S = ctx->ln_split;
        if (S > 8) S = 8;
        if (S > nk / sk_minnk) S = nk / sk_minnk;
        while (S >= 2 && (S - 1) * ((nk + S - 1) / S) >= nk) --S;
        if (S >= 2 && (int64_t)a.M * a.N * groups * S <= ws_floats && (a.N & 3) == 0) return gemm_slices(ctx, a, S, ws, st, ln);
    }
    return launch_gemm(a, st, &ctx->err);
}

int gemm_slices(actmi_ctx* ctx, const GemmArgs& a, int S, float* ws, hipStream_t st, LnFuse* ln) {
    const int groups = a.groups > 0 ? a.groups : 1;
    const int64_t slice = (int64_t)a.M * a.N;
    GemmArgs p = a;
    p.scale = p.bias = p.res = nullptr;
    p.relu = 0;
    p.C = ws;
    p.ldc = a.N;
    p.gC = slice * S;
    p.splitk = S;
    p.split_stride = slice;
    int rc = launch_gemm(p, st, &ctx->err);
    if (rc) return rc;
    if (ln && groups == 1 && !a.scale && !a.relu && (!a.res || a.ldres == a.N)) {
        rc = launch_layernorm(ws, a.res, 0, ln->w, ln->b, ln->w2, ln->b2, ln->out, a.M, a.N, ln->eps, st, &ctx->err, S, slice,
                              a.bias, ln->extra);
        ln->done = rc == 0;
        return rc;
    }
    SplitCombineArgs c{};
    c.part = ws; c.nsplit = S; c.split_stride = slice; c.gP = slice * S; c.ldp = a.N;
    c.scale = a.scale; c.bias = a.bias; c.gSB = a.gSB;
    c.res = a.res; c.ldres = a.ldres; c.gRes = a.gRes;
    c.relu = a.relu;
    c.C = a.C; c.ldc = a.ldc; c.gC = a.gC;
    c.M = a.M; c.N = a.N; c.groups = groups;
    rc = launch_splitk_combine(c, st);
    if (rc) ctx->err = "splitk combine launch failed";
    return rc;
}

float engine_weight_scale(const actmi_ctx* ctx, const float* w) {
    const int64_t off = w - ctx->pbase;
    size_t lo = 0, hi = ctx->params.size();
    while (hi - lo > 1) {
        const size_t mid = (lo + hi) / 2;
        if (ctx->params[mid].off <= off) lo = mid; else hi = mid;
    }
    return lo < ctx->pscale.size() ? ctx->pscale[lo] : W16_SCALE;
}

int engine_calibrate_weight_scales(actmi_ctx* ctx, hipStream_t st) {
    const int np = (int)ctx->params.size();
    ctx->pscale.assign(np, W16_SCALE);
    if (ctx->gemm_prec != ACTMI_PREC_F16X3) return 0;
    CHK(launch_seg_amax(ctx->pbase, ctx->poff_dev, ctx->pnumel_dev, np, ctx->pamax_dev, st));
    std::vector<unsigned> bits(np);
    HIPCHK(hipMemcpyAsync(bits.data(), ctx->pamax_dev, np * sizeof(unsigned), hipMemcpyDeviceToHost, st));
    HIPCHK(hipStreamSynchronize(st));
    float gmax = 0.f;
    for (int i = 0; i < np; ++i) {
        float amax;
        memcpy(&amax, &bits[i], 4);
        if (!(amax <= 3.0e38f)) {
            ctx->err = "parameter " + ctx->params[i].key + " is not finite";
            return ACTMI_E_INVALID;
        }
        float sc = 4096.f;
        if (amax > 0.f) {
            int e;
            frexpf(amax, &e);
            const float fit = ldexpf(1.f, 14 - e);
            sc = fit < 4096.f ? fit : 4096.f;
        }
        if (!(sc >= 1.17549435e-38f) || !(amax * sc < 65504.f)) {
            ctx->err = "parameter " + ctx->params[i].key + " is too large for the f16x3 path (use gemm_prec f32)";
            return ACTMI_E_INVALID;
        }
        ctx->pscale[i] = sc;
        if (!ctx->params[i].is_buffer && amax > gmax) gmax = amax;
    }
    HIPCHK(hipMemcpyAsync(ctx->pscale_dev, ctx->pscale.data(), np * sizeof(float), hipMemcpyHostToDevice, st));
    auto key_scale = [&](const std::string& key) {
        auto it = ctx->index.find(key);
        return it == ctx->index.end() ? W16_SCALE : ctx->pscale[it->second];
    };
    ctx->conv1_wscale = 4096.f;
    for (auto& cl : ctx->convs) cl.w16_scale = 4096.f;
    for (int cam = 0; cam < ctx->cfg.num_cams; ++cam) {
        const std::string p = "backbones." + std::to_string(cam) + ".0.body.";
        ctx->conv1_wscale = std::min(ctx->conv1_wscale, key_scale(p + "conv1.weight"));
        for (auto& cl : ctx->convs) cl.w16_scale = std::min(cl.w16_scale, key_scale(p + cl.name + ".weight"));
    }
    ctx->bwd_wscale = W16_SCALE;
    while (gmax * ctx->bwd_wscale >= 16384.f && ctx->bwd_wscale > 1.f / 65536.f) ctx->bwd_wscale *= 0.5f;
    HIPCHK(hipStreamSynchronize(st));
    return 0;
}

namespace {

MhaW mha_w(actmi_ctx* c, const std::string& p) {
    MhaW m;
    m.in_w = c->P(p + "in_proj_weight");
    m.in_b = c->P(p + "in_proj_bias");
    m.out_w = c->P(p + "out_proj.weight");
    m.out_b = c->P(p + "out_proj.bias");
    return m;
}

void resolve_layers(actmi_ctx* c) {
    const actmi_config& g = c->cfg;
    auto enc = [&](const std::string& p) {
        EncW e;
        e.attn = mha_w(c, p + "self_attn.");
        e.l1w = c->P(p + "linear1.weight"); e.l1b = c->P(p + "linear1.bias");
        e.l2w = c->P(p + "linear2.weight"); e.l2b = c->P(p + "linear2.bias");
        e.n1w = c->P(p + "norm1.weight"); e.n1b = c->P(p + "norm1.bias");
        e.n2w = c->P(p + "norm2.weight"); e.n2b = c->P(p + "norm2.bias");
        return e;
    };
    c->enc.clear(); c->cvae.clear(); c->dec.clear();
    for (int i = 0; i < g.enc_layers; ++i) c->enc.push_back(enc("transformer.encoder.layers." + std::to_string(i) + "."));
    if (g.has_cvae_encoder)
        for (int i = 0; i < g.enc_layers; ++i) c->cvae.push_back(enc("encoder.layers." + std::to_string(i) + "."));
    for (int i = 0; i < g.dec_layers; ++i) {
        std::string p = "transformer.decoder.layers." + std::to_string(i) + ".";
        DecW d;
        d.self_attn = mha_w(c, p + "self_attn.");
        d.cross = mha_w(c, p + "multihead_attn.");
        d.l1w = c->P(p + "linear1.weight"); d.l1b = c->P(p + "linear1.bias");
        d.l2w = c->P(p + "linear2.weight"); d.l2b = c->P(p + "linear2.bias");
        d.n1w = c->P(p + "norm1.weight"); d.n1b = c->P(p + "norm1.bias");
        d.n2w = c->P(p + "norm2.weight"); d.n2b = c->P(p + "norm2.bias");
        d.n3w = c->P(p + "norm3.weight"); d.n3b = c->P(p + "norm3.bias");
        c->dec.push_back(d);
    }
    if (c->has_pcd) {
        const std::string p = "pcl_backbone.pointnet._mlp.";
        c->pcdw = PcdW{c->P(p + "0.weight"), c->P(p + "0.bias"), c->P(p + "3.weight"), c->P(p + "3.bias"),
                       c->P(p + "6.weight"), c->P(p + "6.bias"), c->P(p + "9.weight"), c->P(p + "9.bias"),
                       c->P("input_proj_pointnet.weight"), c->P("input_proj_pointnet.bias")};
    }
}

}

GemmArgs linear_args(const float* A, int64_t lda, int M, int K, const float* W, int N, const float* bias, float* C,
                     int64_t ldc) {
    GemmArgs a;
    memset(&a, 0, sizeof(a));
    a.A = A; a.lda = lda; a.M = M; a.K = K; a.N = N; a.Bw = W; a.ldb = K; a.bias = bias; a.C = C; a.ldc = ldc;
    a.groups = 1;
    return a;
}

static GemmArgs conv_args(const actmi_ctx* ctx, const ConvLayer& cl, int B, int c0, int nc, const float* in, float* out, int K,
                          const float* w, const float* w16, float w16_scale) {
    GemmArgs a;
    memset(&a, 0, sizeof(a));
    a.mode = 1;
    a.A = in; a.H = cl.H; a.W = cl.W; a.Cin = cl.cin; a.KH = a.KW = cl.k; a.stride = cl.stride; a.pad = cl.pad;
    a.Ho = cl.Ho; a.Wo = cl.Wo; a.img_stride = (int64_t)cl.H * cl.W * cl.cin;
    a.M = B * cl.Ho * cl.Wo; a.N = cl.cout; a.K = K;
    const bool split = engine_prec(ctx) == ACTMI_PREC_F16X3;
    a.Bw = (split ? w16 : w) + (int64_t)c0 * cl.cout * K; a.ldb = K;
    if (split) { a.b_split = 1; a.b_scale = w16_scale; a.k_tap_inner = cl.k_tap_inner ? 1 : 0; }
    a.C = out; a.ldc = cl.cout;
    a.groups = nc;
    a.gA = (int64_t)B * cl.H * cl.W * cl.cin; a.gB = (int64_t)cl.cout * K; a.gSB = cl.cout;
    a.gC = (int64_t)a.M * cl.cout;
    return a;
}

GemmArgs conv_gemm_args(const actmi_ctx* ctx, const ConvLayer& cl, int B, int c0, int nc, const float* in, float* out,
                        const float* res, int relu) {
    GemmArgs a = conv_args(ctx, cl, B, c0, nc, in, out, cl.K, cl.w, cl.w16, cl.w16_scale);
    a.scale = cl.scale + (int64_t)c0 * cl.cout; a.bias = cl.bias + (int64_t)c0 * cl.cout; a.res = res; a.ldres = cl.cout; a.relu = relu;
    a.gRes = a.gC;
    return a;
}

GemmArgs conv_fused_args(const actmi_ctx* ctx, const ConvLayer& cl, int B, int c0, int nc, const float* y1, const float* x,
                         float* out) {
    const ConvLayer& ds = ctx->convs[cl.ds_index];
    GemmArgs a = conv_args(ctx, cl, B, c0, nc, y1, out, cl.K + cl.Kx, cl.wf, cl.wf16, cl.wf16_scale);
    a.Ax = x; a.kx_begin = cl.K; a.Hx = ds.H; a.Wx = ds.W; a.Cx = ds.cin; a.stride_x = ds.stride;
    a.gAx = (int64_t)B * ds.H * ds.W * ds.cin;
    a.bias = cl.bias_f + (int64_t)c0 * cl.cout; a.relu = 1;
    return a;
}

Conv3Args conv3_args(const ConvLayer& cl, int B, int c0, int nc, const float* in, float* out, const float* res, int relu) {
    Conv3Args c;
    c.x = in; c.w16 = cl.w16 + (int64_t)c0 * cl.cout * cl.K; c.scale = cl.scale + (int64_t)c0 * cl.cout;
    c.bias = cl.bias + (int64_t)c0 * cl.cout; c.res = res; c.out = out;
    c.G = nc; c.B = B; c.H = cl.H; c.W = cl.W; c.relu = relu; c.w_scale = cl.w16_scale;
    return c;
}

Conv1Args stem_args(const actmi_ctx* ctx, const void* image, int fmt, int B) {
    const actmi_config& g = ctx->cfg;
    Conv1Args c1;
    c1.image = image; c1.fmt = fmt; c1.lut = ctx->lut; c1.w = ctx->conv1_w; c1.scale = ctx->conv1_scale;
    c1.bias = ctx->conv1_bias; c1.out = ctx->act1; c1.B = B; c1.C = g.num_cams; c1.H = g.image_h; c1.W = g.image_w;
    c1.Ho = ctx->H1; c1.Wo = ctx->W1; c1.Cout = g.base_width;
    c1.prec = ctx->gemm_prec;
    c1.wimg = ctx->conv1_wimg;
    c1.wscale = ctx->conv1_wscale;
    return c1;
}

AttnArgs packed_self_attn_args(const actmi_ctx* ctx, const float* qkv, float* out, int B, int n) {
    const int H = ctx->cfg.nheads, D = ctx->cfg.hidden_dim, hd = D / H;
    AttnArgs at;
    memset(&at, 0, sizeof(at));
    at.Q = qkv; at.q_bs = (int64_t)n * 3 * D; at.q_rs = 3 * D;
    at.K = qkv + D; at.k_bs = at.q_bs; at.k_rs = 3 * D;
    at.V = qkv + 2 * D; at.v_bs = at.q_bs; at.v_rs = 3 * D;
    at.O = out; at.o_bs = (int64_t)n * D; at.o_rs = D;
    at.kpm_bs = n;
    at.B = B; at.H = H; at.Nq = n; at.Nk = n; at.HD = hd; at.scale = 1.0f / sqrtf((float)hd);
    return at;
}

AttnArgs cross_attn_args(const actmi_ctx* ctx, const float* q, bool per_sample_q, const float* kv, float* out, int B) {
    const int H = ctx->cfg.nheads, D = ctx->cfg.hidden_dim, hd = D / H, Q = ctx->cfg.num_queries, N = ctx->N;
    AttnArgs at;
    memset(&at, 0, sizeof(at));
    at.Q = q; at.q_bs = per_sample_q ? (int64_t)Q * D : 0; at.q_rs = D;
    at.K = kv; at.k_bs = (int64_t)N * 2 * D; at.k_rs = 2 * D;
    at.V = kv + D; at.v_bs = at.k_bs; at.v_rs = 2 * D;
    at.O = out; at.o_bs = (int64_t)Q * D; at.o_rs = D;
    at.B = B; at.H = H; at.Nq = Q; at.Nk = N; at.HD = hd; at.scale = 1.0f / sqrtf((float)hd);
    return at;
}

void u8_lut(float* lut, bool normalize) {
    const float mean[3] = {0.485f, 0.456f, 0.406f}, stdv[3] = {0.229f, 0.224f, 0.225f};
    for (int c = 0; c < 3; ++c)
        for (int v = 0; v < 256; ++v) {
            const float x = (float)((double)v / 255.0);
            lut[c * 256 + v] = normalize ? (x - mean[c]) / stdv[c] : x;
        }
}

int64_t backbone_cam_stride(actmi_ctx* ctx) {
    const std::string p1 = "backbones." + std::to_string(ctx->cfg.num_cams > 1 ? 1 : 0) + ".0.body.";
    return ctx->P(p1 + "conv1.weight") - ctx->P("backbones.0.0.body.conv1.weight");
}

float* actmi_ctx::P(const std::string& key) {
    auto it = index.find(key);
    if (it == index.end()) return nullptr;
    return pbase + params[it->second].off;
}


namespace {

bool env_on(const char* name) {
    const char* e = getenv(name);
    return !(e && e[0] == '0');
}
int env_int(const char* name, int unset) {
    const char* e = getenv(name);
    return e ? atoi(e) : unset;
}

void read_switches(actmi_ctx* ctx) {
    ctx->gemm_prec = env_gemm_prec(ACTMI_PREC_F16X3);
    const char* tp = getenv("ACTMI_TRAIN_PREC");
    if (tp && tp[0] == 'b') ctx->train_prec = ACTMI_PREC_BF16;
    ctx->conv1_vpool = env_on("ACTMI_CONV1_VPOOL");
    ctx->fwd_splitk = env_on("ACTMI_FWD_SPLITK");
    ctx->act_calib = env_on("ACTMI_ACT_CALIB");
    ctx->cam_pipe = env_on("ACTMI_CAM_PIPE");
    ctx->ln_split = env_int("ACTMI_LN_SPLIT", ctx->ln_split);
    ctx->nbranch = std::min(std::max(env_int("ACTMI_BRANCHES", ctx->nbranch), 2), 4);
}

int create_device_state(actmi_ctx* ctx) {
    const actmi_config& g = ctx->cfg;
    if (ctx->ptotal & 3) { ctx->err = "parameter arena not a multiple of 4 floats"; return ACTMI_E_LAUNCH; }
    ALLOC(ctx->pbase, ctx->ptotal);
    HIPCHK(hipMemset(ctx->pbase, 0, ctx->ptotal * sizeof(float)));
    ALLOC(ctx->p16base, ctx->ptotal);
    ctx->splitk_ws_floats = (int64_t)256 << 18;
    ALLOC(ctx->splitk_ws, ctx->splitk_ws_floats);
    {
        const int np = (int)ctx->params.size();
        std::vector<int> seg((size_t)(ctx->ptotal / 64), 0);
        std::vector<int64_t> off(np), numel(np);
        for (int i = 0; i < np; ++i) {
            off[i] = ctx->params[i].off; numel[i] = ctx->params[i].numel;
            const int64_t g0 = ctx->params[i].off / 64, g1 = (i + 1 < np ? ctx->params[i + 1].off : ctx->ptotal) / 64;
            for (int64_t g = g0; g < g1; ++g) seg[(size_t)g] = i;
        }
        ALLOC(ctx->pseg64, (int64_t)seg.size()); ALLOC(ctx->poff_dev, np); ALLOC(ctx->pnumel_dev, np);
// ... 222 lines not shown
                             (int64_t)C * cl.cout * (cl.K + cl.Kx) <= ctx->splitk_ws_floats;
            CHK(split_conv_image(ctx, cl, cl.w, cl.w16, cl.K, cl.w16_scale, ctx->flags, st));
        }
        for (const ConvLayer& cl : ctx->convs)
            if (cl.wf) {
                const ConvLayer& ds = ctx->convs[cl.ds_index];
                CHK(launch_fold_cat_w(cl.w, cl.scale, cl.bias, ds.w, ds.scale, ds.bias, cl.wf, cl.bias_f, C, cl.cout, cl.K, cl.Kx, st));
                CHK(split_conv_image(ctx, cl, cl.wf, cl.wf16, cl.K + cl.Kx, cl.wf16_scale, after_step ? ctx->flags : nullptr, st));
            }
    }
    HIPCHK(hipMemcpyAsync(ctx->pos_tokens, ctx->P("additional_pos_embed.weight"), (size_t)ctx->n_extra * D * sizeof(float),
                          hipMemcpyDeviceToDevice, st));
    {
        const DecW& d = ctx->dec[0];
        GemmArgs a = linear_args(d.self_attn.in_b + 2 * D, D, 1, D, d.self_attn.out_w, D, d.self_attn.out_b, ctx->dec_sa, D);
        CHK(ctx_gemm(ctx, a, st));
        CHK(launch_layernorm(ctx->dec_sa, nullptr, 0, d.n1w, d.n1b, nullptr, nullptr, ctx->dec_t1, 1, D, 1e-5f, st, &ctx->err));
        GemmArgs q = linear_args(ctx->P("query_embed.weight"), D, Q, D, d.cross.in_w, D, d.cross.in_b, ctx->dec_q, D);
        q.A_add = ctx->dec_t1; q.ld_add = D; q.add_mod = 1; q.add_ncols = D;
        CHK(ctx_gemm(ctx, q, st));
    }
    return 0;
}

int engine_finalize(actmi_ctx* ctx, hipStream_t st) {
    ctx->err.clear();
    const int C = ctx->cfg.num_cams;
    if (ctx->train) CHK(train_fit_prec(ctx));
    {
        std::vector<float> lut(768);
        u8_lut(lut.data(), true);
        HIPCHK(hipMemcpyAsync(ctx->lut, lut.data(), 768 * sizeof(float), hipMemcpyHostToDevice, st));
        HIPCHK(hipStreamSynchronize(st));
    }
    CHK(build_pos_tokens(ctx));
    CHK(engine_calibrate_weight_scales(ctx, st));
    CHK(engine_prepare_weights(ctx, st));
    if (ctx->gemm_prec == ACTMI_PREC_F16X3) {
        std::vector<ConvLayer*> fl;
        for (auto& cl : ctx->convs) if (cl.wf) fl.push_back(&cl);
        if (!fl.empty()) {
            HIPCHK(hipMemsetAsync(ctx->wf_scale_slots, 0, 2 * fl.size() * sizeof(float), st));
            for (size_t i = 0; i < fl.size(); ++i) {
                const int Kf = fl[i]->K + fl[i]->Kx;
                CHK(launch_pow2_scale(fl[i]->wf, Kf, C * fl[i]->cout, Kf, ctx->wf_scale_slots + 2 * i, st));
            }
            std::vector<float> sc(2 * fl.size());
            HIPCHK(hipMemcpyAsync(sc.data(), ctx->wf_scale_slots, sc.size() * sizeof(float), hipMemcpyDeviceToHost, st));
            HIPCHK(hipStreamSynchronize(st));
            for (size_t i = 0; i < fl.size(); ++i) {
                ConvLayer& cl = *fl[i];
                const float v = sc[2 * i];
                if (!(v > 0.f) || !(v <= 3.0e38f)) { ctx->err = "fused weights of " + cl.name + " are not finite"; return ACTMI_E_INVALID; }
                cl.wf16_scale = v < 4096.f ? v : 4096.f;
                CHK(split_conv_image(ctx, cl, cl.wf, cl.wf16, cl.K + cl.Kx, cl.wf16_scale, ctx->flags, st));
            }
        }
    }
    HIPCHK(hipStreamSynchronize(st));
    CHK(engine_calibrate_activations(ctx, st));
    ctx->finalized = true;
    return 0;
}


int engine_measure_act_scale(actmi_ctx* ctx, const float* x, int64_t rows, int cols, hipStream_t st, float* out) {
    *out = 1.f;
    if (rows <= 0 || rows > 0x7fffffff) return 0;
    float* slot = ctx->act_scale_slot;
    HIPCHK(hipMemsetAsync(slot, 0, 2 * sizeof(float), st));
    CHK(launch_pow2_scale(x, cols, (int)rows, cols, slot, st));
    float s = 1.f;
    HIPCHK(hipMemcpyAsync(&s, slot, sizeof(float), hipMemcpyDeviceToHost, st));
    HIPCHK(hipStreamSynchronize(st));
    if (s > 131072.f || s <= 4.f) *out = s * (1.f / 16.f);
    return 0;
}

int engine_calibrate_activations(actmi_ctx* ctx, hipStream_t st) {
    for (auto& cl : ctx->convs) cl.a_scale = 1.f;
    ctx->ip_a_scale = 1.f;
    if (ctx->gemm_prec != ACTMI_PREC_F16X3 || !ctx->act_calib) return 0;
    const actmi_config& g = ctx->cfg;
    const size_t nbytes = (size_t)g.num_cams * g.image_h * g.image_w * 3;
    std::vector<unsigned char> img(nbytes);
    uint32_t x = 0x9E3779B9u;
    for (size_t i = 0; i < nbytes; ++i) { x = x * 1664525u + 1013904223u; img[i] = (unsigned char)(x >> 24); }
    void* dimg = nullptr;
    if (hipMalloc(&dimg, nbytes) != hipSuccess) { ctx->err = "hipMalloc (calibration frame)"; return ACTMI_E_NOMEM; }
    int rc = hipMemcpy(dimg, img.data(), nbytes, hipMemcpyHostToDevice) == hipSuccess ? 0 : ACTMI_E_LAUNCH;
    if (rc == 0) {
        ctx->calibrating = true;
        const std::string keep = ctx->stop_stage;
        ctx->stop_stage.clear();
        rc = engine_backbone(ctx, dimg, ACTMI_IMG_U8_NHWC, 1, st);
        ctx->stop_stage = keep;
        ctx->calibrating = false;
        if (hipStreamSynchronize(st) != hipSuccess && rc == 0) rc = ACTMI_E_LAUNCH;
    }
    (void)hipFree(dimg);
    ctx->dbg.clear();
    return rc;
}

template <class Body>
static int run_branches(actmi_ctx* ctx, int nb, hipStream_t st, Body body) {
    ctx->policy_mult = nb;
    int rc = 0;
    hipError_t he = hipEventRecord(ctx->ev_pfork, st);
    const char* he_where = "hipEventRecord(fork)";
    bool forked[4] = {false, false, false, false};
    for (int i = nb - 1; i >= 0; --i) {
        if (rc != 0 || he != hipSuccess) break;
        hipStream_t bs = i ? ctx->pipe_streams[i - 1] : st;
        if (i) {
            he = hipStreamWaitEvent(bs, ctx->ev_pfork, 0);
            if (he != hipSuccess) { he_where = "hipStreamWaitEvent(fork)"; break; }
            forked[i] = true;
        }
        rc = body(i, bs);
    }
    for (int i = 1; i < nb; ++i) {
        if (!forked[i]) continue;
        hipError_t e = hipEventRecord(ctx->ev_pjoins[i - 1], ctx->pipe_streams[i - 1]);
        if (e == hipSuccess) e = hipStreamWaitEvent(st, ctx->ev_pjoins[i - 1], 0);
        if (e != hipSuccess && he == hipSuccess) { he = e; he_where = "branch join"; }
    }
    ctx->policy_mult = 1;
    if (rc != 0) return rc;
    if (he != hipSuccess) {
        if (ctx->err.empty()) ctx->err = std::string(he_where) + ": " + hipGetErrorString(he);
        return ACTMI_E_LAUNCH;
    }
    return 0;
}

int engine_backbone(actmi_ctx* ctx, const void* image, int fmt, int B, hipStream_t st) {
    const actmi_config& g = ctx->cfg;
    const int C = g.num_cams, w0 = g.base_width, D = g.hidden_dim;
    Conv1Args c1 = stem_args(ctx, image, fmt, B);
    const bool vpool = ctx->conv1_vpool && ctx->stop_stage != "conv1" && ctx->gemm_prec == ACTMI_PREC_F16X3 && (ctx->H1 & 1) == 0 &&
                       (w0 & 3) == 0 && ctx->H2 == ctx->H1 / 2;
    c1.vpool = vpool ? 1 : 0;
    CHK(launch_conv1(c1, st, &ctx->err));
    if (vpool) CHK(launch_hpool(ctx->act1, ctx->buf[0], C * B * ctx->H2, ctx->W1, w0, ctx->W2, st));
    else CHK(launch_maxpool(ctx->act1, ctx->buf[0], C * B, ctx->H1, ctx->W1, w0, ctx->H2, ctx->W2, st));
    ctx->dbg.clear();
    ctx->dbg["conv1"] = {ctx->act1, (int64_t)C * B * ctx->H1 * ctx->W1 * w0};
    ctx->dbg["maxpool"] = {ctx->buf[0], (int64_t)C * B * ctx->H2 * ctx->W2 * w0};
    if (ctx->stop_stage == "conv1" || ctx->stop_stage == "maxpool") return 1;
    auto run_conv_on = [&](ConvLayer& cl, const float* in, float* out, const float* res, int relu, hipStream_t cs, int c0,
                           int nc, int half) -> int {
        const int cl_index = (int)(&cl - ctx->convs.data());
        if (ctx->calibrating) {
            CHK(engine_measure_act_scale(ctx, in, (int64_t)nc * B * cl.H * cl.W, cl.cin, cs, &cl.a_scale));
            HIPCHK(hipMemcpyAsync(ctx->act_scale_dev + cl_index, &cl.a_scale, sizeof(float), hipMemcpyHostToDevice, cs));
            HIPCHK(hipStreamSynchronize(cs));
        }
        if (ctx->gemm_prec == ACTMI_PREC_F16X3 && cl.direct) {
            Conv3Args c3 = conv3_args(cl, B, c0, nc, in, out, res, relu);
            if (cl.a_scale != 1.f) c3.x_scale_dev = ctx->act_scale_dev + cl_index;
            return launch_conv3x3_c64(c3, cs, &ctx->err);
        }
        GemmArgs a = conv_gemm_args(ctx, cl, B, c0, nc, in, out, res, relu);
        if (ctx->gemm_prec == ACTMI_PREC_F16X3 && cl.a_scale != 1.f) a.a_scale = cl.a_scale;
        return ctx_gemm(ctx, a, cs, half);
    };
    const bool pipe = ctx->cam_pipe && C >= 2 && !prof_enabled() && ctx->stop_stage.empty() && !ctx->calibrating;
    const bool fork_ds = ctx->side_stream != nullptr && !pipe && !ctx->calibrating;
    auto run_layers = [&](int c0, int nc, hipStream_t ls, int half) -> int {
        const int64_t hb = (int64_t)c0 * B * ctx->H2 * ctx->W2 * w0;
        float *cur = ctx->buf[0] + hb, *s1 = ctx->buf[1] + hb, *s2 = ctx->buf[2] + hb;
        auto run_conv = [&](ConvLayer& cl, const float* in, float* out, const float* res, int relu) -> int {
            return run_conv_on(cl, in, out, res, relu, ls, c0, nc, half);
        };
        size_t ci = 0;
        for (int li = 1; li <= 4; ++li) {
            for (int bi = 0; bi < 2; ++bi) {
                ConvLayer& k1 = ctx->convs[ci++];
                ConvLayer& k2 = ctx->convs[ci++];
                const bool has_ds = (bi == 0 && li > 1);
                if (has_ds && k2.wf && ctx->gemm_prec == ACTMI_PREC_F16X3 && !ctx->calibrating && k2.a_scale == 1.f &&
                    ctx->convs[k2.ds_index].a_scale == 1.f) {
                    ++ci;
                    CHK(run_conv(k1, cur, s1, nullptr, 1));
                    CHK(ctx_gemm(ctx, conv_fused_args(ctx, k2, B, c0, nc, s1, cur, s2), ls, half));
                    std::swap(cur, s2);
                } else if (has_ds) {
                    ConvLayer& ds = ctx->convs[ci++];
                    if (fork_ds) {
                        HIPCHK(hipEventRecord(ctx->ev_fork, ls));
                        HIPCHK(hipStreamWaitEvent(ctx->side_stream, ctx->ev_fork, 0));
                        const int r1 = run_conv_on(ds, cur, s2, nullptr, 0, ctx->side_stream, c0, nc, half);
                        const hipError_t e1 = hipEventRecord(ctx->ev_join, ctx->side_stream);
                        const int r2 = r1 == 0 ? run_conv(k1, cur, s1, nullptr, 1) : 0;
                        const hipError_t e2 = e1 == hipSuccess ? hipStreamWaitEvent(ls, ctx->ev_join, 0) : e1;
                        CHK(r1);
                        CHK(r2);
                        HIPCHK(e1);
                        HIPCHK(e2);
                    } else {
                        CHK(run_conv(k1, cur, s1, nullptr, 1));
                        CHK(run_conv(ds, cur, s2, nullptr, 0));
                    }
                    CHK(run_conv(k2, s1, cur, s2, 1));
                } else {
                    CHK(run_conv(k1, cur, s1, nullptr, 1));
                    CHK(run_conv(k2, s1, s2, cur, 1));
                    std::swap(cur, s2);
                }
                if (bi == 1 && c0 == 0) {
                    const std::string nm = "layer" + std::to_string(li);
                    ctx->dbg[nm] = {cur, (int64_t)C * B * k2.Ho * k2.Wo * k2.cout};
                    if (ctx->stop_stage == nm) return 1;
                }
            }
        }
        GemmArgs ip = linear_args(cur, 8 * w0, nc * B * ctx->P_, 8 * w0, ctx->P("input_proj.weight"), D, ctx->P("input_proj.bias"),
                                  ctx->X, D);
        ip.rowmap = ctx->rowmap + (int64_t)c0 * B * ctx->P_;
        if (ctx->calibrating) {
            CHK(engine_measure_act_scale(ctx, cur, (int64_t)nc * B * ctx->P_, 8 * w0, ls, &ctx->ip_a_scale));
            HIPCHK(hipStreamSynchronize(ls));
        }
        if (ctx->gemm_prec == ACTMI_PREC_F16X3 && ctx->ip_a_scale != 1.f) ip.a_scale = ctx->ip_a_scale;
        return ctx_gemm(ctx, ip, ls, half);
    };
    if (ctx->rowmap_B != B) {
        CHK(launch_build_rowmap(ctx->rowmap, B, C, ctx->fh, ctx->fw, ctx->N, ctx->n_extra, st));
        ctx->rowmap_B = B;
    }
    if (pipe) {
        const int nb = C < ctx->nbranch ? C : ctx->nbranch;
        const int rc = run_branches(ctx, nb, st, [&](int i, hipStream_t bs) -> int {
            const int c0 = i * C / nb, c1 = (i + 1) * C / nb;
            return run_layers(c0, c1 - c0, bs, i);
        });
        if (rc != 0) return rc;
    } else {
        const int rc = run_layers(0, C, st, -1);
        if (rc != 0) return rc;
    }
    return 0;
}

int engine_take_pointcloud(actmi_ctx* ctx, int B, const float** xyz, const float** rgb, int* P) {
    *xyz = *rgb = nullptr;
    *P = 0;
    if (!ctx->has_pcd) return 0;
    if (!ctx->pcd_xyz || !ctx->pcd_rgb) {
        ctx->err = "this handle has a point-cloud branch: bind the clouds of every forward with actmi_set_pointcloud";
        return ACTMI_E_STATE;
    }
    if (ctx->pcd_B != B) {
        ctx->err = "forward of batch " + std::to_string(B) + " but the bound point clouds hold " + std::to_string(ctx->pcd_B) + " samples";
        return ACTMI_E_STATE;
    }
    *xyz = ctx->pcd_xyz; *rgb = ctx->pcd_rgb; *P = ctx->pcd_P;
    ctx->pcd_xyz = ctx->pcd_rgb = nullptr;
    return 0;
}

int engine_pointnet(actmi_ctx* ctx, const float* xyz, const float* rgb, int B, int P, hipStream_t st) {
    const int Hp = ctx->pcd.hidden_dim, Op = ctx->pcd.output_dim, D = ctx->cfg.hidden_dim, R = B * P;
    const PcdW& w = ctx->pcdw;
    float *a = ctx->pcd_act[0], *b = ctx->pcd_act[1];
    if (launch_pcd_embed(xyz, rgb, nullptr, w.w0, w.b0, a, nullptr, R, Hp, st) != 0) { ctx->err = "pcd_embed launch failed"; return ACTMI_E_LAUNCH; }
    GemmArgs l3 = linear_args(a, Hp, R, Hp, w.w3, Hp, w.b3, b, Hp);
    l3.relu = 2;
    CHK(ctx_gemm(ctx, l3, st));
    GemmArgs l6 = linear_args(b, Hp, R, Hp, w.w6, Hp, w.b6, a, Hp);
    l6.relu = 2;
    CHK(ctx_gemm(ctx, l6, st));
    CHK(ctx_gemm(ctx, linear_args(a, Hp, R, Hp, w.w9, Op, w.b9, b, Op), st));
    if (launch_colmax(b, B, P, Op, Op, ctx->pcd_feat, ctx->pcd_arg, ctx->pcd_ws, ctx->pcd_ws_floats, st) != 0) {
        ctx->err = "colmax launch failed";
        return ACTMI_E_LAUNCH;
    }
    CHK(ctx_gemm(ctx, linear_args(ctx->pcd_feat, Op, B, Op, w.pw, D, w.pb, ctx->X + 2 * D, (int64_t)ctx->N * D), st));
    ctx->dbg["pcd_feat"] = {ctx->pcd_feat, (int64_t)B * Op};
    ctx->dbg["pcd_argmax"] = {reinterpret_cast<const float*>(ctx->pcd_arg), (int64_t)B * Op};
    return 0;
}

struct TView {
    float *X, *XP, *QKV, *ATT, *Y, *X1, *Hb, *dO, *dY, *dT2, *dH, *hs, *attn_ws;
    int64_t attn_ws_floats;
    int half;
};
static TView make_view(const actmi_ctx* ctx, int b0, int nb, int half) {
    const actmi_config& g = ctx->cfg;
    const int64_t D = g.hidden_dim, F = g.dim_feedforward, Q = g.num_queries, N = ctx->N;
    const int64_t ws_per = ctx->attn_ws_floats / g.max_batch;
    TView v;
    v.X = ctx->X + b0 * N * D; v.XP = ctx->XP + b0 * N * D; v.QKV = ctx->QKV + b0 * N * 3 * D; v.ATT = ctx->ATT + b0 * N * D; v.Y = ctx->Y + b0 * N * D;
    v.X1 = ctx->X1 + b0 * N * D; v.Hb = ctx->Hb + b0 * N * F;
    v.dO = ctx->dO + b0 * Q * D; v.dY = ctx->dY + b0 * Q * D; v.dT2 = ctx->dT2 + b0 * Q * D; v.dH = ctx->dH + b0 * Q * F;
    v.hs = ctx->hs + b0 * Q * D;
    v.attn_ws = ctx->attn_ws + b0 * ws_per; v.attn_ws_floats = (half < 0) ? ctx->attn_ws_floats : nb * ws_per;
    v.half = half;
    return v;
}

int engine_encoder_layer(actmi_ctx* ctx, const EncW& w, const TView& V, const float* pos, int B, int n, const uint8_t* kpm,
                         hipStream_t st, bool xp_in, bool xp_out) {
    float* x = V.X;
    const actmi_config& g = ctx->cfg;
    const int D = g.hidden_dim, F = g.dim_feedforward, M = B * n;
    GemmArgs qkv = linear_args(x, D, M, D, w.attn.in_w, 3 * D, w.attn.in_b, V.QKV, 3 * D);
    if (xp_in) { qkv.A_alt = V.XP; qkv.alt_ncols = 2 * D; }
    else { qkv.A_add = pos; qkv.ld_add = D; qkv.add_mod = n; qkv.add_ncols = 2 * D; }
    CHK(ctx_gemm(ctx, qkv, st, V.half));
    AttnArgs at = packed_self_attn_args(ctx, V.QKV, V.ATT, B, n);
    at.kpm = kpm;
    at.ws = V.attn_ws; at.ws_floats = V.attn_ws_floats;
    at.prec = ctx->gemm_prec;
    CHK(launch_attention(at, st, &ctx->err));
    GemmArgs op = linear_args(V.ATT, D, M, D, w.attn.out_w, D, w.attn.out_b, V.Y, D);
    op.res = x; op.ldres = D;
    LnFuse ln1{w.n1w, w.n1b, nullptr, nullptr, V.X1, 1e-5f, false};
    CHK(ctx_gemm(ctx, op, st, V.half, &ln1));
    if (!ln1.done) CHK(launch_layernorm(V.Y, nullptr, 0, w.n1w, w.n1b, nullptr, nullptr, V.X1, M, D, 1e-5f, st, &ctx->err));
    GemmArgs f1 = linear_args(V.X1, D, M, D, w.l1w, F, w.l1b, V.Hb, F);
    f1.relu = 1;
    CHK(ctx_gemm(ctx, f1, st, V.half));
    GemmArgs f2 = linear_args(V.Hb, F, M, F, w.l2w, D, w.l2b, V.Y, D);
    f2.res = V.X1; f2.ldres = D;
    LnExtra ex;
    if (xp_out) { ex.y2 = V.XP; ex.add2 = pos; ex.add2_mod = n; }
    LnFuse ln2{w.n2w, w.n2b, nullptr, nullptr, x, 1e-5f, false, xp_out ? &ex : nullptr};
    CHK(ctx_gemm(ctx, f2, st, V.half, &ln2));
    if (!ln2.done)
        CHK(launch_layernorm(V.Y, nullptr, 0, w.n2w, w.n2b, nullptr, nullptr, x, M, D, 1e-5f, st, &ctx->err, 1, 0, nullptr,
                             xp_out ? &ex : nullptr));
    return 0;
}

int engine_decoder_infer(actmi_ctx* ctx, const TView& V, int B, float* a_hat, hipStream_t st, bool xp_in) {
    const actmi_config& g = ctx->cfg;
    const int D = g.hidden_dim, F = g.dim_feedforward, Q = g.num_queries, N = ctx->N;
    const DecW& d = ctx->dec[0];
    float* KV = V.QKV;
    GemmArgs kv = linear_args(V.X, D, B * N, D, d.cross.in_w + (int64_t)D * D, 2 * D, d.cross.in_b + D, KV, 2 * D);
    if (xp_in) { kv.A_alt = V.XP; kv.alt_ncols = D; }
    else { kv.A_add = ctx->pos_tokens; kv.ld_add = D; kv.add_mod = N; kv.add_ncols = D; }
    CHK(ctx_gemm(ctx, kv, st, V.half));
    AttnArgs at = cross_attn_args(ctx, ctx->dec_q, false, KV, V.dO, B);
    at.ws = V.attn_ws; at.ws_floats = V.attn_ws_floats;
    at.prec = ctx->gemm_prec;
    CHK(launch_attention(at, st, &ctx->err));
    const int M = B * Q;
    GemmArgs op = linear_args(V.dO, D, M, D, d.cross.out_w, D, d.cross.out_b, V.dY, D);
    op.res = ctx->dec_t1; op.ldres = D; op.res_mod = 1;
    CHK(ctx_gemm(ctx, op, st, V.half));
    CHK(launch_layernorm(V.dY, nullptr, 0, d.n2w, d.n2b, nullptr, nullptr, V.dT2, M, D, 1e-5f, st, &ctx->err));
    GemmArgs f1 = linear_args(V.dT2, D, M, D, d.l1w, F, d.l1b, V.dH, F);
    f1.relu = 1;
    CHK(ctx_gemm(ctx, f1, st, V.half));
    GemmArgs f2 = linear_args(V.dH, F, M, F, d.l2w, D, d.l2b, V.dY, D);
    f2.res = V.dT2; f2.ldres = D;
    LnExtra hx;
    const bool head_in_ln = g.action_dim <= 64;
    if (head_in_ln) {
        hx.head_out = a_hat; hx.head_w = ctx->P("action_head.weight"); hx.head_b = ctx->P("action_head.bias"); hx.head_n = g.action_dim;
        hx.flag = ctx->flags; hx.flag_bit = ACTMI_FLAG_OUTPUT;
    }
    LnFuse ln3{d.n3w, d.n3b, ctx->P("transformer.decoder.norm.weight"), ctx->P("transformer.decoder.norm.bias"), V.hs, 1e-5f, false,
               head_in_ln ? &hx : nullptr};
    CHK(ctx_gemm(ctx, f2, st, V.half, &ln3));
    if (!ln3.done)
        CHK(launch_layernorm(V.dY, nullptr, 0, d.n3w, d.n3b, ctx->P("transformer.decoder.norm.weight"),
                             ctx->P("transformer.decoder.norm.bias"), V.hs, M, D, 1e-5f, st, &ctx->err, 1, 0, nullptr,
                             head_in_ln ? &hx : nullptr));
    if (!head_in_ln) {
        GemmArgs ah = linear_args(V.hs, D, M, D, ctx->P("action_head.weight"), g.action_dim, ctx->P("action_head.bias"),
                                  a_hat, g.action_dim);
        ah.finite_flag = ctx->flags; ah.finite_bit = ACTMI_FLAG_OUTPUT;
        CHK(ctx_gemm(ctx, ah, st, V.half));
    }
    if (V.half <= 0) ctx->dbg["hs"] = {ctx->hs, (int64_t)ctx->last_B * Q * D};
    return 0;
}

int engine_forward_infer(actmi_ctx* ctx, const float* qpos, const void* image, int fmt, int B, float* a_hat,
                         hipStream_t st, const float* vq_sample) {
    ctx->err.clear();
    if (!ctx->finalized) { ctx->err = "forward before finalize"; return ACTMI_E_STATE; }
    if (B < 1 || B > ctx->cfg.max_batch) { ctx->err = "batch exceeds max_batch"; return ACTMI_E_INVALID; }
    if (fmt != ACTMI_IMG_U8_NHWC && fmt != ACTMI_IMG_F32_NCHW) { ctx->err = "bad image format"; return ACTMI_E_INVALID; }
    const actmi_config& g = ctx->cfg;
    const int D = g.hidden_dim, N = ctx->N;
    const float *pc_xyz = nullptr, *pc_rgb = nullptr;
    int pc_P = 0;
    if (ctx->fwd_phase != 2) CHK(engine_take_pointcloud(ctx, B, &pc_xyz, &pc_rgb, &pc_P));
    if (ctx->fwd_phase != 2) {
        const int rc = engine_backbone(ctx, image, fmt, B, st);
        if (rc == 1) return 0;
        if (rc != 0) return rc;
        float* fill_dst = nullptr;
        if (g.vq && vq_sample) {
            const int K = g.vq_class * g.vq_dim;
            GemmArgs lz = linear_args(vq_sample, K, B, K, ctx->P("latent_out_proj.weight"), D, ctx->P("latent_out_proj.bias"),
                                      ctx->X, (int64_t)N * D);
            CHK(ctx_gemm(ctx, lz, st));
        } else {
            fill_dst = ctx->X;
        }
        CHK(launch_small_linear(qpos, g.state_dim, ctx->P("input_proj_robot_state.weight"),
                                ctx->P("input_proj_robot_state.bias"), ctx->X + D, (int64_t)N * D, B, D, g.state_dim, st, fill_dst,
                                ctx->P("latent_out_proj.bias"), 0));
        if (ctx->has_pcd) CHK(engine_pointnet(ctx, pc_xyz, pc_rgb, B, pc_P, st));
        if (ctx->fwd_phase == 1) { ctx->last_B = B; return 0; }
    } else if (B != ctx->last_B) {
        ctx->err = "forward phase 2 without a phase 1 of the same batch before it";
        return ACTMI_E_STATE;
    }
    ctx->dbg["src"] = {ctx->X, (int64_t)B * N * D};
    if (ctx->stop_stage == "src") return 0;
    ctx->last_B = B;
    auto run_transformer = [&](int b0, int nb, hipStream_t ts, int half) -> int {
        const TView V = make_view(ctx, b0, nb, half);
        const bool xp_qkv = ((2 * D) % 128) == 0, xp_kv = (D % 128) == 0;
        for (int l = 0; l < g.enc_layers; ++l)
            CHK(engine_encoder_layer(ctx, ctx->enc[l], V, ctx->pos_tokens, nb, N, nullptr, ts, l > 0 && xp_qkv,
                                     l + 1 < g.enc_layers ? xp_qkv : xp_kv));
        return engine_decoder_infer(ctx, V, nb, a_hat + (int64_t)b0 * g.num_queries * g.action_dim, ts, xp_kv);
    };
    const bool tpipe = ctx->cam_pipe && B >= 2 && !prof_enabled() && ctx->stop_stage.empty();
    ctx->dbg["memory"] = {ctx->X, (int64_t)B * N * D};
    if (tpipe) {
        const int nb = B < ctx->nbranch ? B : ctx->nbranch;
        const int rc = run_branches(ctx, nb, st, [&](int i, hipStream_t bs) -> int {
            const int b0 = i * B / nb, b1 = (i + 1) * B / nb;
            return run_transformer(b0, b1 - b0, bs, i);
        });
        if (rc != 0) return rc;
    } else {
        CHK(run_transformer(0, B, st, -1));
    }
    return 0;
}
```

act-plus-plus_amd/csrc/gemm.hip:

```cpp
#include "common.h"
#include "dropout.h"
#include "split16.h"
#include <cstdio>
#include <string>
#include <cstdlib>
#include <type_traits>

namespace {

constexpr int BK = 32;
constexpr int NPL = BK / 4;

enum { A_N = 0, A_CONV = 1, A_DGRAD = 2, A_T = 3, A_NADD = 4 };
enum { B_N = 0, B_T = 1, B_WGRAD = 2 };

enum { PREC_F32 = 0, PREC_F16X3 = 1, PREC_BF16 = 2 };
constexpr int ACTMI_PREC_DEFAULT_IS = ACTMI_PREC_F32;

#ifndef ACTMI_LDS_PAD
#define ACTMI_LDS_PAD 1
#endif
constexpr int LDS_PAD = ACTMI_LDS_PAD;

template <int BM, int BN, int PREC>
constexpr int stage_f4() { return NPL * ((BM + LDS_PAD) + (BN + LDS_PAD)); }

typedef _Float16 h16x4 __attribute__((ext_vector_type(4)));
typedef _Float16 h16x8 __attribute__((ext_vector_type(8)));
typedef __bf16 bf16x2 __attribute__((ext_vector_type(2)));
typedef __bf16 bf16x8 __attribute__((ext_vector_type(8)));

__device__ __forceinline__ uint2 pack_bf16x4(const f32x4 v) {
    const bf16x2 a = {(__bf16)v[0], (__bf16)v[1]}, b = {(__bf16)v[2], (__bf16)v[3]};
    return uint2{__builtin_bit_cast(unsigned, a), __builtin_bit_cast(unsigned, b)};
}

__device__ __forceinline__ int swz_row(int r) { return r ^ ((r >> 3) & 3); }

__device__ __forceinline__ f32x4 ld4(const float* p) { return *reinterpret_cast<const f32x4*>(p); }

template <int BM, int BN, int WM, int WN, int AMODE, int BMODE, int PREC, int BSPLIT, int UNMASKED, int XS = 0>
__global__ __launch_bounds__((BM / WM) * (BN / WN) * 64, (PREC && BM * BN <= 128 * 64 && (AMODE == 0  || AMODE == 3 ) && !(AMODE == 0 && BMODE == 1)) ? 3 : 2)
    void gemm_f32_kernel(GemmArgs p, int tiles_m, int tiles_n) {
    constexpr int NT = (BM / WM) * (BN / WN) * 64;
    constexpr int RPP = NT / 8;
    constexpr int TM = WM / 32, TN = WN / 32;
    constexpr int WAVES_N = BN / WN;
    constexpr int PSA = BM + LDS_PAD, PSB = BN + LDS_PAD;
    constexpr int STAGE = stage_f4<BM, BN, PREC>();
    constexpr int NLA = (AMODE == A_T) ? 4 : BM / RPP;
    constexpr int NLB = (BMODE != B_N) ? 4 : BN / RPP;
    static_assert(BM % RPP == 0 && BN % RPP == 0, "tile rows must be a multiple of the rows staged per pass");
    extern __shared__ __attribute__((aligned(16))) char smem_raw[];
    f32x4* smem = reinterpret_cast<f32x4*>(smem_raw);

    const int nwg = tiles_m * tiles_n;
    const int splitk = p.splitk > 1 ? p.splitk : 1;
    int bid, zz;
    {
        const int total = nwg * (int)gridDim.z;
        const int lin = blockIdx.z * gridDim.x + blockIdx.x;
        const int xcd = lin & 7, q = total >> 3, r = total & 7;
        const int base = (xcd < r) ? xcd * (q + 1) : r * (q + 1) + (xcd - r) * q;
        const int flat = base + (lin >> 3);
        zz = flat / nwg;
        bid = flat - zz * nwg;
    }
    constexpr int GROUP_M = 8;
    const int width = GROUP_M * tiles_n;
    const int group_id = bid / width;
    const int first_m = group_id * GROUP_M;
    const int gsz = (tiles_m - first_m < GROUP_M) ? tiles_m - first_m : GROUP_M;
    const int in_group = bid - group_id * width;
    const int m0 = (first_m + in_group % gsz) * BM;
    const int n0 = (in_group / gsz) * BN;
    const int split = zz % splitk;
    const int g = zz / splitk;
    int64_t offA, offB, offC, offRes;
    if (p.groups_inner > 0) {
        const int g1 = g / p.groups_inner, g2 = g % p.groups_inner;
        offA = g1 * p.gA + g2 * p.gA2; offB = g1 * p.gB + g2 * p.gB2;
        offC = g1 * p.gC + g2 * p.gC2; offRes = g1 * p.gRes + g2 * p.gRes2;
    } else {
        offA = (int64_t)g * p.gA; offB = (int64_t)g * p.gB; offC = (int64_t)g * p.gC; offRes = (int64_t)g * p.gRes;
    }
    const float* __restrict__ A = ((AMODE == A_N) && p.A_alt != nullptr && n0 < p.alt_ncols ? p.A_alt : p.A) + offA;
    const float* __restrict__ Bw = p.Bw + offB;

    uint64_t* stamp = p.stamps ? p.stamps + ((int64_t)blockIdx.z * gridDim.x + blockIdx.x) * 4 : nullptr;
    if (stamp && threadIdx.x == 0) {
        stamp[0] = __builtin_amdgcn_s_memtime();
        const unsigned hw = __builtin_amdgcn_s_getreg((4 ) | (0 << 6) | (31 << 11));
        const unsigned xcc = __builtin_amdgcn_s_getreg((20 ) | (0 << 6) | (31 << 11));
        stamp[1] = ((uint64_t)xcc << 32) | hw;
    }
    unsigned* const amax_out = UNMASKED ? nullptr : p.amax_out;
    unsigned* const fflag = UNMASKED ? nullptr : p.finite_flag;
    const bool track = amax_out != nullptr || fflag != nullptr;
    const unsigned amax_seen = amax_out ? __hip_atomic_load(amax_out, __ATOMIC_RELAXED, __HIP_MEMORY_SCOPE_AGENT) : 0u;
    const int nk_total = (p.K + BK - 1) / BK;
    const int tps = (nk_total + splitk - 1) / splitk;
    const int kt_begin = split * tps;
    const int kt_end = (kt_begin + tps < nk_total) ? kt_begin + tps : nk_total;
    if (kt_begin >= kt_end) return;
    const int t = threadIdx.x;
    const int lane = t & 63, wave = t >> 6;
    const int li = lane & 31, lh = lane >> 5;
    const int wrow0 = (wave / WAVES_N) * WM;
    const int wcol0 = (wave % WAVES_N) * WN;
    int arow[TM], bcol[TN];
#pragma unroll
    for (int i = 0; i < TM; ++i) arow[i] = (AMODE == A_T) ? swz_row(wrow0 + i * 32 + li) : wrow0 + i * 32 + li;
#pragma unroll
    for (int j = 0; j < TN; ++j) bcol[j] = (BMODE != B_N) ? swz_row(wcol0 + j * 32 + li) : wcol0 + j * 32 + li;
    const int cidx = t & 7;
    const int srow = t >> 3;

    const float* a_ptr[NLA];
    const float* add_ptr[NLA];
    int a_hi0[NLA], a_wi0[NLA];
    bool a_ok[NLA];
    const bool conv_fast = AMODE == A_CONV && (p.Cin % BK) == 0 && p.KH * p.KW <= 32 &&
                           (int64_t)p.H * p.W * p.Cin < ((int64_t)1 << 30);
    unsigned a_tapmask[AMODE == A_CONV ? NLA : 1];
    int a_off0[AMODE == A_CONV ? NLA : 1];
    int a_offx[XS ? NLA : 1];
    const float* __restrict__ Axg = XS ? p.Ax + (int64_t)g * p.gAx : nullptr;
    const int ktx = XS ? p.kx_begin / BK : 0x7fffffff;
    const float conv_inv_tpr = (AMODE == A_CONV && conv_fast) ? 1.0f / (float)(p.Cin / BK) : 0.f;
    const float conv_inv_kw = (AMODE == A_CONV || AMODE == A_DGRAD) ? 1.0f / (float)p.KW : 0.f;
    const float conv_inv_ntap = (AMODE == A_CONV) ? 1.0f / (float)(p.KH * p.KW) : 0.f;
    const int dg_cq = (AMODE == A_DGRAD) ? p.K / (p.KH * p.KW) : BK;
    const bool dgrad_fast = AMODE == A_DGRAD && (dg_cq % BK) == 0 && (p.stride == 1 || p.stride == 2) &&
                            (int64_t)p.Ho * p.Wo * dg_cq < ((int64_t)1 << 30);
    const float dg_inv_tpr = (AMODE == A_DGRAD) ? 1.0f / (float)(dg_cq / BK > 0 ? dg_cq / BK : 1) : 0.f;
    unsigned conv_rep = 0;
    if (AMODE == A_CONV && conv_fast)
        for (int r = 0; r < p.KH; ++r) conv_rep |= 1u << (r * p.KW);
    const bool use_add = (AMODE == A_NADD) && n0 < p.add_ncols;
    const int a_og = t % (BM / 4), a_kg = t / (BM / 4);
    if (AMODE == A_T) {
    } else {
#pragma unroll
        for (int i = 0; i < NLA; ++i) {
            const int m = m0 + srow + RPP * i;
            a_ok[i] = m < p.M;
            const int mm = a_ok[i] ? m : 0;
            add_ptr[i] = nullptr;
            a_hi0[i] = a_wi0[i] = 0;
            if (AMODE == A_N || AMODE == A_NADD) {
                const int64_t ar = p.a_rowmap ? p.a_rowmap[mm] : mm;
                a_ptr[i] = A + ar * p.lda;
                if (AMODE == A_NADD) add_ptr[i] = p.A_add + (int64_t)(mm % p.add_mod) * p.ld_add;
            } else if (AMODE == A_CONV) {
                const int hw = p.Ho * p.Wo;
                const int b = mm / hw, rem = mm - b * hw;
                const int ho = rem / p.Wo, wo = rem - ho * p.Wo;
                a_ptr[i] = A + (int64_t)b * p.img_stride;
                a_hi0[i] = ho * p.stride - p.pad;
                a_wi0[i] = wo * p.stride - p.pad;
                if (conv_fast) {
                    const int r_lo = a_hi0[i] < 0 ? -a_hi0[i] : 0, q_lo = a_wi0[i] < 0 ? -a_wi0[i] : 0;
                    int r_hi = p.H - a_hi0[i], q_hi = p.W - a_wi0[i];
                    r_hi = r_hi < p.KH ? (r_hi > 0 ? r_hi : 0) : p.KH;
                    q_hi = q_hi < p.KW ? (q_hi > 0 ? q_hi : 0) : p.KW;
                    const unsigned colmask = (r_lo < r_hi && q_lo < q_hi) ? (((1u << q_hi) - 1u) & ~((1u << q_lo) - 1u)) : 0u;
                    const unsigned rowsel = (unsigned)((((uint64_t)1 << (r_hi * p.KW)) - 1u) & ~(((uint64_t)1 << (r_lo * p.KW)) - 1u));
                    a_tapmask[i] = a_ok[i] ? (rowsel & (colmask * conv_rep)) : 0u;
                    a_off0[i] = (a_hi0[i] * p.W + a_wi0[i]) * p.Cin + cidx * 4;
                    if (XS) a_offx[i] = ((b * p.Hx + ho * p.stride_x) * p.Wx + wo * p.stride_x) * p.Cx + cidx * 4;
                }
            } else {
                const int hw = p.H * p.W;
                const int b = mm / hw, rem = mm - b * hw;
                const int hi = rem / p.W, wi = rem - hi * p.W;
                a_ptr[i] = A + (int64_t)b * p.img_stride;
                a_hi0[i] = hi + p.pad;
                a_wi0[i] = wi + p.pad;
            }
        }
    }
    const float* b_ptr[NLB];
    bool b_ok[NLB];
    const int b_og = t % (BN / 4), b_kg = t / (BN / 4);
    int wg_r = 0, wg_s = 0, wg_c = 0;
    const float wg_inv_hw = (BMODE == B_WGRAD) ? 1.0f / (float)(p.Ho * p.Wo) : 0.f;
    const float wg_inv_wo = (BMODE == B_WGRAD) ? 1.0f / (float)p.Wo : 0.f;
    if (BMODE == B_N) {
#pragma unroll
        for (int i = 0; i < NLB; ++i) {
            const int n = n0 + srow + RPP * i;
            b_ok[i] = n < p.N;
            b_ptr[i] = Bw + (int64_t)(b_ok[i] ? n : 0) * p.ldb;
        }
    } else if (BMODE == B_WGRAD) {
        const int j0 = n0 + b_og * 4;
        const int rs = j0 / p.Cin;
        wg_c = j0 - rs * p.Cin;
        wg_r = rs / p.KW;
        wg_s = rs - wg_r * p.KW;
    }

    struct Regs {
        f32x4 ra[NLA], rb[NLB], rx[AMODE == A_NADD ? NLA : 1];
        bool ra_ok[NLA], rb_ok[NLB];
    };
    Regs R0;
    const f32x4 zero4 = {0.f, 0.f, 0.f, 0.f};
    auto ldb4 = [](const float* base, unsigned offb) { return *reinterpret_cast<const f32x4*>(reinterpret_cast<const char*>(base) + offb); };
    auto ubase = [](const float* q) {
        const uint64_t u = reinterpret_cast<uint64_t>(q);
        return reinterpret_cast<const float*>(((uint64_t)(unsigned)__builtin_amdgcn_readfirstlane((int)(u >> 32)) << 32) |
                                              (unsigned)__builtin_amdgcn_readfirstlane((int)(unsigned)u));
    };
    const bool at_interior = AMODE == A_T && m0 + BM <= p.M;
    const bool bt_interior = BMODE == B_T && n0 + BN <= p.N && p.B_add == nullptr;
    const unsigned at_offb = AMODE == A_T ? ((unsigned)(a_kg * 4) * (unsigned)p.lda + (unsigned)(m0 + a_og * 4)) * 4u : 0u;
    const unsigned bt_offb = BMODE == B_T ? ((unsigned)(b_kg * 4) * (unsigned)p.ldb + (unsigned)(n0 + b_og * 4)) * 4u : 0u;

    auto load_tile = [&](int kt, auto& R) {
        if (AMODE == A_T) {
            if (a_kg < NPL && at_interior && (kt + 1) * BK <= p.K) {
                const float* __restrict__ rb = ubase(A + (int64_t)kt * BK * p.lda);
#pragma unroll
                for (int j = 0; j < 4; ++j) R.ra[j] = ldb4(rb + (int64_t)j * p.lda, at_offb);
            } else if (a_kg < NPL) {
                const int o = m0 + a_og * 4;
#pragma unroll
                for (int j = 0; j < 4; ++j) {
                    const int kk = kt * BK + a_kg * 4 + j;
                    f32x4 v = zero4;
                    if (kk < p.K) {
                        const float* src = A + (int64_t)kk * p.lda + o;
                        if (o + 3 < p.M) v = ld4(src);
                        else {
#pragma unroll
                            for (int e = 0; e < 4; ++e) if (o + e < p.M) v[e] = src[e];
                        }
                    }
                    R.ra[j] = v;
                }
            }
        } else {
            const int k = kt * BK + cidx * 4;
            const bool kok = k < p.K;
            if (AMODE == A_N || AMODE == A_NADD) {
                const int kc = kok ? k : 0;
#pragma unroll
                for (int i = 0; i < NLA; ++i) {
                    R.ra[i] = ld4(a_ptr[i] + kc);
                    if (AMODE == A_NADD) R.rx[i] = ld4(add_ptr[i] + kc);
                    R.ra_ok[i] = a_ok[i] && kok;
                }
            } else if (XS && kt >= ktx) {
                const int dk = (kt - ktx) * BK;
#pragma unroll
                for (int i = 0; i < NLA; ++i) {
                    R.ra[i] = ld4(Axg + (a_ok[i] ? a_offx[i] + dk : 0));
                    R.ra_ok[i] = a_ok[i];
                }
            } else if (AMODE == A_CONV && conv_fast) {
                const int tpr = p.Cin / BK;
                const int ntap = p.KH * p.KW;
                int rs, cb;
                if (p.k_tap_inner) {
                    const int cbi = (int)(((float)kt + 0.5f) * conv_inv_ntap);
                    rs = kt - cbi * ntap;
                    cb = cbi * BK;
                } else {
                    rs = (int)(((float)kt + 0.5f) * conv_inv_tpr);
                    cb = (kt - rs * tpr) * BK;
                }
                const int r = (int)(((float)rs + 0.5f) * conv_inv_kw);
                const int q = rs - r * p.KW;
                const int delta = (r * p.W + q) * p.Cin + cb;
#pragma unroll
                for (int i = 0; i < NLA; ++i) {
                    const bool inb = (a_tapmask[i] >> rs) & 1u;
                    const int off = inb ? a_off0[i] + delta : 0;
                    R.ra[i] = ld4(a_ptr[i] + off);
                    R.ra_ok[i] = inb;
                }
            } else if (AMODE == A_CONV) {
                const int rs = k / p.Cin;
                const int c = k - rs * p.Cin;
                const int r = rs / p.KW;
                const int s = rs - r * p.KW;
#pragma unroll
                for (int i = 0; i < NLA; ++i) {
                    const int hi = a_hi0[i] + r, wi = a_wi0[i] + s;
                    const bool inb = a_ok[i] && kok && (unsigned)hi < (unsigned)p.H && (unsigned)wi < (unsigned)p.W;
                    const int64_t off = inb ? ((int64_t)hi * p.W + wi) * p.Cin + c : 0;
                    R.ra[i] = ld4(a_ptr[i] + off);
                    R.ra_ok[i] = inb;
                }
            } else if (dgrad_fast) {
                const int tpr = dg_cq / BK;
                const int rs = (int)(((float)kt + 0.5f) * dg_inv_tpr);
                const int nb = (kt - rs * tpr) * BK + cidx * 4;
                const int r = (int)(((float)rs + 0.5f) * conv_inv_kw);
                const int q = rs - r * p.KW;
                const int sh = p.stride - 1;
#pragma unroll
                for (int i = 0; i < NLA; ++i) {
                    const int hn = a_hi0[i] - r, wn = a_wi0[i] - q;
                    const int ho = hn >> sh, wo = wn >> sh;
                    const bool ok = a_ok[i] && hn >= 0 && wn >= 0 && ((hn | wn) & sh) == 0 && ho < p.Ho && wo < p.Wo;
                    const int off = ok ? (ho * p.Wo + wo) * dg_cq + nb : 0;
                    R.ra[i] = ld4(a_ptr[i] + off);
                    R.ra_ok[i] = ok;
                }
            } else {
                const int Cq = p.K / (p.KH * p.KW);
                const int rs = k / Cq;
                const int n = k - rs * Cq;
                const int r = rs / p.KW;
                const int s = rs - r * p.KW;
#pragma unroll
                for (int i = 0; i < NLA; ++i) {
                    const int hn = a_hi0[i] - r, wn = a_wi0[i] - s;
                    f32x4 v = zero4;
                    if (a_ok[i] && kok && hn >= 0 && wn >= 0) {
                        const int ho = hn / p.stride, wo = wn / p.stride;
                        if (ho * p.stride == hn && wo * p.stride == wn && ho < p.Ho && wo < p.Wo)
                            v = ld4(a_ptr[i] + ((int64_t)ho * p.Wo + wo) * Cq + n);
                    }
                    R.ra[i] = v;
                    R.ra_ok[i] = true;
                }
            }
        }
        if (BMODE == B_N) {
            const int k = kt * BK + cidx * 4;
            const bool kok = k < p.K;
            const int kc = kok ? k : 0;
#pragma unroll
            for (int i = 0; i < NLB; ++i) {
                R.rb[i] = ld4(b_ptr[i] + kc);
                R.rb_ok[i] = b_ok[i] && kok;
            }
        } else if (BMODE == B_T) {
            if (AMODE == A_T && b_kg < NPL && bt_interior && (kt + 1) * BK <= p.K) {
                const float* __restrict__ rb = ubase(Bw + (int64_t)kt * BK * p.ldb);
#pragma unroll
// ... 111 lines not shown
                    if (BMODE == B_WGRAD) v = f32x4{R.rb_ok[0] ? v[0] : 0.f, R.rb_ok[1] ? v[1] : 0.f, R.rb_ok[2] ? v[2] : 0.f, R.rb_ok[3] ? v[3] : 0.f};
                    uint2 hi, lo;
                    const int row = swz_row(b_og * 4 + i);
                    if (PREC == PREC_BF16) sb8[(((b_kg >> 1) * 2 + 0) * PSB + row) * 2 + (b_kg & 1)] = pack_bf16x4(v);
                    else {
                    split16(v, hi, lo);
                    sb8[(((b_kg >> 1) * 2 + 0) * PSB + row) * 2 + (b_kg & 1)] = hi;
                    sb8[(((b_kg >> 1) * 2 + 1) * PSB + row) * 2 + (b_kg & 1)] = lo;
                    }
                }
            }
        }
    };
    auto store_tile = [&](int stage, auto& R) {
        f32x4* sa = smem + stage * STAGE;
        f32x4* sb = sa + NPL * PSA;
        if (AMODE == A_T) {
            if (a_kg < NPL) {
#pragma unroll
                for (int i = 0; i < 4; ++i) {
                    const f32x4 v = {R.ra[0][i], R.ra[1][i], R.ra[2][i], R.ra[3][i]};
                    sa[a_kg * PSA + swz_row(a_og * 4 + i)] = v;
                }
            }
        } else {
#pragma unroll
            for (int i = 0; i < NLA; ++i) {
                f32x4 v = R.ra[i];
                if (AMODE == A_NADD) { if (use_add) v += R.rx[i]; }
                v = R.ra_ok[i] ? v : zero4;
                sa[cidx * PSA + srow + RPP * i] = v;
            }
        }
        if (BMODE == B_N) {
#pragma unroll
            for (int i = 0; i < NLB; ++i) sb[cidx * PSB + srow + RPP * i] = R.rb_ok[i] ? R.rb[i] : zero4;
        } else {
            if (b_kg < NPL) {
#pragma unroll
                for (int i = 0; i < 4; ++i) {
                    f32x4 v = {R.rb[0][i], R.rb[1][i], R.rb[2][i], R.rb[3][i]};
                    if (BMODE == B_WGRAD) v = f32x4{R.rb_ok[0] ? v[0] : 0.f, R.rb_ok[1] ? v[1] : 0.f, R.rb_ok[2] ? v[2] : 0.f, R.rb_ok[3] ? v[3] : 0.f};
                    sb[b_kg * PSB + swz_row(b_og * 4 + i)] = v;
                }
            }
        }
    };

    f32x16 acc[TM][TN];
#pragma unroll
    for (int i = 0; i < TM; ++i)
#pragma unroll
        for (int j = 0; j < TN; ++j)
#pragma unroll
            for (int e = 0; e < 16; ++e) acc[i][j][e] = 0.f;

    const int nsteps = kt_end - kt_begin;
    if constexpr (PREC != PREC_F32) {
        auto compute16 = [&](int cur) {
            const f32x4* sa = smem + cur * STAGE;
            const f32x4* sb = sa + NPL * PSA;
            f32x4 ah[2][TM], al[2][TM], bh[2][TN], bl[2][TN];
#pragma unroll
            for (int s2 = 0; s2 < 2; ++s2) {
                const int kg = 2 * s2 + lh;
#pragma unroll
                for (int i = 0; i < TM; ++i) {
                    ah[s2][i] = sa[(kg * 2 + 0) * PSA + arow[i]];
                    if (PREC == PREC_F16X3) al[s2][i] = sa[(kg * 2 + 1) * PSA + arow[i]];
                }
#pragma unroll
                for (int j = 0; j < TN; ++j) {
                    bh[s2][j] = sb[(kg * 2 + 0) * PSB + bcol[j]];
                    if (PREC == PREC_F16X3) bl[s2][j] = sb[(kg * 2 + 1) * PSB + bcol[j]];
                }
            }
            if constexpr (PREC == PREC_BF16) {
#pragma unroll
                for (int s2 = 0; s2 < 2; ++s2)
#pragma unroll
                    for (int i = 0; i < TM; ++i)
#pragma unroll
                        for (int j = 0; j < TN; ++j)
                            acc[i][j] = __builtin_amdgcn_mfma_f32_32x32x16_bf16(__builtin_bit_cast(bf16x8, ah[s2][i]),
                                                                                __builtin_bit_cast(bf16x8, bh[s2][j]), acc[i][j], 0, 0, 0);
                return;
            }
#pragma unroll
            for (int s2 = 0; s2 < 2; ++s2)
#pragma unroll
                for (int i = 0; i < TM; ++i)
#pragma unroll
                    for (int j = 0; j < TN; ++j) {
                        const h16x8 xh = __builtin_bit_cast(h16x8, ah[s2][i]), xl = __builtin_bit_cast(h16x8, al[s2][i]);
                        const h16x8 yh = __builtin_bit_cast(h16x8, bh[s2][j]), yl = __builtin_bit_cast(h16x8, bl[s2][j]);
                        acc[i][j] = __builtin_amdgcn_mfma_f32_32x32x16_f16(xl, yh, acc[i][j], 0, 0, 0);
                        acc[i][j] = __builtin_amdgcn_mfma_f32_32x32x16_f16(xh, yl, acc[i][j], 0, 0, 0);
                        acc[i][j] = __builtin_amdgcn_mfma_f32_32x32x16_f16(xh, yh, acc[i][j], 0, 0, 0);
                    }
        };
        auto run = [&](auto maskedc) {
            Regs R1;
            const int kt_last = kt_end - 1;
            auto ld = [&](int kt, auto& R) { load_tile(kt < kt_last ? kt : kt_last, R); };
            constexpr bool HOT = (AMODE == A_N || AMODE == A_NADD || AMODE == A_CONV) && BMODE == B_N;
            auto weave = [&]() {
                if (HOT) {
#pragma unroll
                    for (int r = 0; r < 6 * TM * TN; ++r) {
                        __builtin_amdgcn_sched_group_barrier(0x008, 1, 0);
                        __builtin_amdgcn_sched_group_barrier(0x006, 5, 0);
                        __builtin_amdgcn_sched_group_barrier(0x080, 2, 0);
                        __builtin_amdgcn_sched_group_barrier(0x020, 1, 0);
                    }
                }
            };
            ld(kt_begin, R0);
            ld(kt_begin + 1, R1);
            store16(0, R0, maskedc);
            __syncthreads();
            int s_ = 0;
            for (; s_ + 1 < nsteps; s_ += 2) {
                ld(kt_begin + s_ + 2, R0);
                compute16(0);
                store16(1, R1, maskedc);
                weave();
                __syncthreads();
                ld(kt_begin + s_ + 3, R1);
                compute16(1);
                store16(0, R0, maskedc);
                weave();
                __syncthreads();
            }
            if (s_ < nsteps) {
                compute16(0);
                __syncthreads();
            }
        };
        if constexpr (UNMASKED != 0) run(std::false_type{});
        else run(std::true_type{});
    } else {
    load_tile(kt_begin, R0);
    store_tile(0, R0);
    __syncthreads();
    auto kstep = [&](int s_, auto par, auto pf) {
        constexpr bool PF = decltype(pf)::value;
        constexpr int cur = decltype(par)::value;
        const int kt = kt_begin + s_;
        const f32x4* sa = smem + cur * STAGE;
        const f32x4* sb = sa + NPL * PSA;
        f32x4 af[2][TM], bf[2][TN];
#pragma unroll
        for (int i = 0; i < TM; ++i) af[0][i] = sa[lh * PSA + arow[i]];
#pragma unroll
        for (int j = 0; j < TN; ++j) bf[0][j] = sb[lh * PSB + bcol[j]];
        constexpr bool HOT = (AMODE == A_N || AMODE == A_NADD || AMODE == A_CONV) && BMODE == B_N;
        if (PF) load_tile(kt + 1, R0);
        auto kblock = [&](auto kbc) {
            constexpr int kb = decltype(kbc)::value;
            if (kb + 1 < NPL / 2) {
#pragma unroll
                for (int i = 0; i < TM; ++i) af[(kb + 1) & 1][i] = sa[(2 * (kb + 1) + lh) * PSA + arow[i]];
#pragma unroll
                for (int j = 0; j < TN; ++j) bf[(kb + 1) & 1][j] = sb[(2 * (kb + 1) + lh) * PSB + bcol[j]];
            }
#pragma unroll
            for (int e = 0; e < 4; ++e)
#pragma unroll
                for (int i = 0; i < TM; ++i)
#pragma unroll
                    for (int j = 0; j < TN; ++j)
                        acc[i][j] = __builtin_amdgcn_mfma_f32_32x32x2f32(af[kb & 1][i][e], bf[kb & 1][j][e], acc[i][j], 0, 0, 0);
            if (HOT) {
#pragma unroll
                for (int r = 0; r < 4 * TM * TN; ++r) {
                    __builtin_amdgcn_sched_group_barrier(0x008, 1, 0);
                    __builtin_amdgcn_sched_group_barrier(0x006, kb == 0 ? 10 : 2, 0);
                    __builtin_amdgcn_sched_group_barrier(0x020, 1, 0);
                    __builtin_amdgcn_sched_group_barrier(0x100, 1, 0);
                }
                __builtin_amdgcn_sched_barrier(0);
            }
        };
        kblock(std::integral_constant<int, 0>{});
        kblock(std::integral_constant<int, 1>{});
        kblock(std::integral_constant<int, 2>{});
        kblock(std::integral_constant<int, 3>{});
        static_assert(NPL / 2 == 4, "k-block unroll assumes BK = 32");
        if (PF) store_tile(cur ^ 1, R0);
        __syncthreads();
    };
    using P0 = std::integral_constant<int, 0>;
    using P1 = std::integral_constant<int, 1>;
    int s_ = 0;
    for (; s_ + 2 < nsteps; s_ += 2) {
        kstep(s_, P0{}, std::true_type{});
        kstep(s_ + 1, P1{}, std::true_type{});
    }
    if (nsteps - s_ == 2) {
        kstep(s_, P0{}, std::true_type{});
        kstep(s_ + 1, P1{}, std::false_type{});
    } else {
        kstep(s_, P0{}, std::false_type{});
    }
    }

    if (stamp && threadIdx.x == 0) stamp[2] = __builtin_amdgcn_s_memtime();
    const float* scale = p.scale ? p.scale + (int64_t)g * p.gSB : nullptr;
    const float* bias = p.bias ? p.bias + (int64_t)g * p.gSB : nullptr;
    const float* res = p.res ? p.res + offRes : nullptr;
    const float* mask = p.mask ? p.mask + (int64_t)g * p.gMask : nullptr;
    const int64_t ldmask = p.ldmask ? p.ldmask : p.ldc;
    float* C = p.C + offC + (int64_t)split * p.split_stride;
    float* C2 = p.C2 ? p.C2 + (int64_t)g * p.gC2out : nullptr;
    float alpha = p.alpha != 0.f ? p.alpha : 1.f;
    if (PREC != PREC_F32) {
        if (p.b_scale != 0.f) alpha /= p.b_scale;
        if (p.a_scale != 0.f) alpha /= p.a_scale;
        if (p.a_scale_dev) alpha /= *p.a_scale_dev;
        if (!BSPLIT && p.b_scale_dev) alpha /= *p.b_scale_dev;
    }
    const bool has_mask = mask != nullptr, has_map = p.rowmap != nullptr;
    const int epi = UNMASKED ? 0 : p.epi;
    const float* erow = nullptr;
    const uint8_t* ekill = nullptr;
    if (epi != 0) {
        if (p.groups_inner > 0) {
            const int g1 = g / p.groups_inner, g2 = g % p.groups_inner;
            erow = p.epi_row + g1 * p.gRow + g2 * p.gRow2;
            ekill = p.epi_colkill ? p.epi_colkill + g1 * p.gColkill : nullptr;
        } else {
            erow = p.epi_row + (int64_t)g * p.gRow;
            ekill = p.epi_colkill ? p.epi_colkill + (int64_t)g * p.gColkill : nullptr;
        }
    }
    const bool has_res = res != nullptr && epi != 2;
    const float drop_scale = p.drop_p > 0.f ? 1.f / (1.f - p.drop_p) : 1.f;
    const bool simple = !has_map && (splitk <= 1 || p.split_stride != 0) && !C2 && !(p.drop_p > 0.f) && p.res_mod == 0 &&
                        (!has_mask || (int64_t)p.M * ldmask < (int64_t)1 << 31) &&
                        (int64_t)p.M * p.ldc < (int64_t)1 << 31 && (!res || (int64_t)p.M * p.ldres < (int64_t)1 << 31);
    unsigned amx = 0;
    auto amax_flush = [&]() {
        if (!track) return;
        for (int o = 32; o > 0; o >>= 1) amx = max(amx, (unsigned)__shfl_xor((int)amx, o, 64));
        if (fflag && lane == 0 && amx >= 0x7f800000u) atomicOr(fflag, p.finite_bit);
        if (!amax_out) return;
        if (lane == 0 && amx > amax_seen) atomicMax(amax_out, amx);
    };
    if (simple) {
        const bool relu = p.relu == 1, gelu = p.relu == 2;

        const bool vec = n0 + BN <= p.N && (p.ldc & 3) == 0 && ((uintptr_t)C & 15) == 0 &&
                         (!res || ((p.ldres & 3) == 0 && ((uintptr_t)res & 15) == 0)) &&
                         (!has_mask || ((ldmask & 3) == 0 && ((uintptr_t)mask & 15) == 0)) &&
                         (!scale || ((uintptr_t)scale & 15) == 0) && (!bias || ((uintptr_t)bias & 15) == 0);
        if (vec) {
            constexpr int RS = WN + 8;
            constexpr int LPR = WN / 4;
            constexpr int RPI = 64 / LPR;
            static_assert(4 * 32 * RS * 4 <= 2 * STAGE * 16 || (BM / WM) * (BN / WN) * 32 * RS * 4 <= 2 * STAGE * 16, "epilogue scratch must fit the stage");
            float* scr = reinterpret_cast<float*>(smem) + wave * (32 * RS);
            const int c4 = lane % LPR, r0 = lane / LPR;
            const int ncol = n0 + wcol0 + c4 * 4;
            const f32x4 one4 = {1.f, 1.f, 1.f, 1.f};
            const f32x4 sc4 = scale ? ld4(scale + ncol) : one4;
            const f32x4 bi4 = bias ? ld4(bias + ncol) : zero4;
#pragma unroll
            for (int i = 0; i < TM; ++i) {
#pragma unroll
                for (int j = 0; j < TN; ++j)
#pragma unroll
                    for (int e = 0; e < 16; ++e)
                        scr[((e & 3) + 8 * (e >> 2) + 4 * lh) * RS + j * 32 + li] = acc[i][j][e];
                const int mbase = m0 + wrow0 + i * 32;
#pragma unroll
                for (int q = 0; q < 32 / RPI; ++q) {
                    const int r = q * RPI + r0;
                    const int m = mbase + r;
                    f32x4 v = *reinterpret_cast<const f32x4*>(scr + r * RS + c4 * 4);
                    v = v * alpha * sc4 + bi4;
                    if (m < p.M) {
                        if (epi == 1) {
                            const float rsub = erow[m];
#pragma unroll
                            for (int e = 0; e < 4; ++e) v[e] = (ekill && ekill[ncol + e] != 0) ? 0.f : expf(v[e] - rsub);
                        } else if (epi == 2) {
                            const f32x4 pr = ld4(res + (uint32_t)(m * (int)p.ldres + ncol));
                            v = pr * (v - erow[m]) * p.epi_scale;
                        }
                        if (has_res) v += ld4(res + (uint32_t)(m * (int)p.ldres + ncol));
                        if (has_mask) {
                            const f32x4 mk = ld4(mask + (uint32_t)(m * (int)ldmask + ncol));
#pragma unroll
                            for (int e = 0; e < 4; ++e) v[e] = mk[e] > 0.f ? v[e] : 0.f;
                        }
                        if (relu) {
#pragma unroll
                            for (int e = 0; e < 4; ++e) v[e] = fmaxf(v[e], 0.f);
                        }
                        if (gelu) {
#pragma unroll
                            for (int e = 0; e < 4; ++e) v[e] = 0.5f * v[e] * (1.f + erff(v[e] * 0.70710678118654752f));
                        }
                        *reinterpret_cast<f32x4*>(C + (uint32_t)(m * (int)p.ldc + ncol)) = v;
                        if (track) {
#pragma unroll
                            for (int e = 0; e < 4; ++e) amx = max(amx, __float_as_uint(v[e]) & 0x7fffffffu);
                        }
                    }
                }
            }
            amax_flush();
            if (stamp && threadIdx.x == 0) stamp[3] = __builtin_amdgcn_s_memtime();
            return;
        }
#pragma unroll
        for (int j = 0; j < TN; ++j) {
            const int n = n0 + wcol0 + j * 32 + li;
            const bool nok = n < p.N;
            const float sc = (scale && nok) ? scale[n] : 1.f;
            const float bi = (bias && nok) ? bias[n] : 0.f;
#pragma unroll
            for (int i = 0; i < TM; ++i) {
                const int mb = m0 + wrow0 + i * 32 + 4 * lh;
                float rv[16];
                if (has_res) {
#pragma unroll
                    for (int e = 0; e < 16; ++e) {
                        const int m = mb + (e & 3) + 8 * (e >> 2);
                        const int mc = m < p.M ? m : 0;
                        rv[e] = nok ? res[(uint32_t)(mc * (int)p.ldres + n)] : 0.f;
                    }
                }
#pragma unroll
                for (int e = 0; e < 16; ++e) {
                    const int m = mb + (e & 3) + 8 * (e >> 2);
                    float v = acc[i][j][e] * alpha * sc + bi;
                    if (epi != 0 && nok && m < p.M) {
                        if (epi == 1) v = (ekill && ekill[n] != 0) ? 0.f : expf(v - erow[m]);
                        else v = res[(uint32_t)(m * (int)p.ldres + n)] * (v - erow[m]) * p.epi_scale;
                    }
                    if (has_res) v += rv[e];
                    if (has_mask && nok && m < p.M) { if (!(mask[(uint32_t)(m * (int)ldmask + n)] > 0.f)) v = 0.f; }
                    v = relu ? fmaxf(v, 0.f) : v;
                    if (gelu) v = 0.5f * v * (1.f + erff(v * 0.70710678118654752f));
                    if (nok && m < p.M) {
                        C[(uint32_t)(m * (int)p.ldc + n)] = v;
                        if (track) amx = max(amx, __float_as_uint(v) & 0x7fffffffu);
                    }
                }
                __builtin_amdgcn_sched_barrier(0);
            }
        }
        amax_flush();
        if (stamp && threadIdx.x == 0) stamp[3] = __builtin_amdgcn_s_memtime();
        return;
    }
#pragma unroll
    for (int j = 0; j < TN; ++j) {
        const int n = n0 + wcol0 + j * 32 + li;
        const bool nok = n < p.N;
        const float sc = (scale && nok) ? scale[n] : 1.f;
        const float bi = (bias && nok) ? bias[n] : 0.f;
        const float sc2 = (C2 && nok) ? p.scale2[(int64_t)g * p.gSB + n] : 1.f;
#pragma unroll
        for (int i = 0; i < TM; ++i) {
            int orow[16];
            bool ok[16];
#pragma unroll
            for (int e = 0; e < 16; ++e) {
                const int m = m0 + wrow0 + i * 32 + (e & 3) + 8 * (e >> 2) + 4 * lh;
                ok[e] = nok && m < p.M;
                orow[e] = m;
                if (has_map && ok[e]) orow[e] = p.rowmap[m];
            }
            float rv[16], mv[16];
#pragma unroll
            for (int e = 0; e < 16; ++e) {
                const int m = m0 + wrow0 + i * 32 + (e & 3) + 8 * (e >> 2) + 4 * lh;
                rv[e] = 0.f;
                mv[e] = 1.f;
                if (has_res && ok[e]) rv[e] = res[(int64_t)(p.res_mod ? (m % p.res_mod) : m) * p.ldres + n];
                if (has_mask && ok[e]) mv[e] = mask[(int64_t)m * ldmask + n];
            }
#pragma unroll
            for (int e = 0; e < 16; ++e) {
                if (ok[e]) {
                    float v = acc[i][j][e] * alpha;
                    v = scale ? v * sc + bi : v + bi;
                    const int64_t o = (int64_t)orow[e] * p.ldc + n;
                    if (p.drop_p > 0.f) {
                        if (p.relu && !has_res) v = fmaxf(v, 0.f);
                        v = actmi_keep(p.drop_seed, (uint64_t)(offC + o), p.drop_p) ? v * drop_scale : 0.f;
                    }
                    v += rv[e];
                    if (!(mv[e] > 0.f)) v = 0.f;
                    if (p.relu) v = fmaxf(v, 0.f);
                    if (splitk > 1 && p.split_stride == 0) atomicAdd(&C[o], v);
                    else C[o] = v;
                    if (track) amx = max(amx, __float_as_uint(v) & 0x7fffffffu);
                    if (C2) C2[o] = v * sc2;
                }
            }
            __builtin_amdgcn_sched_barrier(0);
        }
    }
    amax_flush();
    if (stamp && threadIdx.x == 0) stamp[3] = __builtin_amdgcn_s_memtime();
}

template <int BM, int BN, int WM, int WN, int AMODE, int BMODE, int PREC, int BSPLIT, int UNMASKED, int XS = 0>
int launch_cfg_u(const GemmArgs& a, hipStream_t st) {
    const int tiles_m = (a.M + BM - 1) / BM, tiles_n = (a.N + BN - 1) / BN;
    static const int lds_pad = getenv("ACTMI_GEMM_LDSPAD") ? atoi(getenv("ACTMI_GEMM_LDSPAD")) : 0;
    const int smem = 2 * stage_f4<BM, BN, PREC>() * 16 + lds_pad;
    auto kern = gemm_f32_kernel<BM, BN, WM, WN, AMODE, BMODE, PREC, BSPLIT, UNMASKED, XS>;
    static bool attr_set = false;
    if (!attr_set) {
        hipError_t e = hipFuncSetAttribute(reinterpret_cast<const void*>(kern),
                                           hipFuncAttributeMaxDynamicSharedMemorySize, smem);
        if (e != hipSuccess) return (int)e;
        attr_set = true;
    }
    const int splitk = a.splitk > 1 ? a.splitk : 1;
    dim3 grid(tiles_m * tiles_n, 1, (a.groups > 0 ? a.groups : 1) * splitk);
    if (prof_enabled()) {
        char nm[128];
        static const bool by_shape = getenv("ACTMI_PROF_SHAPES") && getenv("ACTMI_PROF_SHAPES")[0] == '1';
        if (by_shape)
            snprintf(nm, sizeof(nm), "gemm_%s_kernel<%d,%d,%d,%d,%d,%d%s>[M=%d,N=%d,K=%d,g=%d,sk=%d,wgs=%d]", PREC == PREC_BF16 ? "bf16" : PREC ? "f16x3" : "f32",
                     BM, BN, WM, WN, AMODE, BMODE, XS ? ",xs" : "", a.M, a.N, a.K, a.groups, splitk, tiles_m * tiles_n * a.groups * splitk);
        else
            snprintf(nm, sizeof(nm), "gemm_%s_kernel<%d,%d,%d,%d,%d,%d%s>", PREC == PREC_BF16 ? "bf16" : PREC ? "f16x3" : "f32", BM, BN, WM, WN, AMODE, BMODE, XS ? ",xs" : "");
        const double g = a.groups;
        double abytes;
        if (AMODE == A_CONV) abytes = (double)(a.M / (a.Ho * a.Wo)) * a.H * a.W * a.Cin + (XS ? (double)a.M * a.Cx : 0.0);
        else if (AMODE == A_DGRAD) abytes = (double)(a.M / (a.H * a.W)) * a.Ho * a.Wo * (a.K / (a.KH * a.KW));
        else abytes = (double)a.M * a.K;
        const double bbytes = (BMODE == B_WGRAD) ? (double)(a.K / (a.Ho * a.Wo)) * a.H * a.W * a.Cin : (double)a.N * a.K;
        prof_begin(nm, 2.0 * a.M * a.N * a.K * g, 4.0 * g * ((double)a.M * a.N + abytes + bbytes), st);
    }
    hipLaunchKernelGGL(kern, grid, dim3((BM / WM) * (BN / WN) * 64), smem, st, a, tiles_m, tiles_n);
    prof_end(st);
    return (int)hipGetLastError();
}

template <int BM, int BN, int WM, int WN, int AMODE, int BMODE, int PREC, int BSPLIT>
int launch_cfg_b(const GemmArgs& a, hipStream_t st) {
    constexpr bool HOT = PREC != PREC_F32 && BMODE == B_N && (AMODE == A_N || AMODE == A_NADD || AMODE == A_CONV);
    if constexpr (HOT) {
        const bool one_a = (a.a_scale == 0.f || a.a_scale == 1.f) && !a.a_scale_dev;
        const bool one_b = BSPLIT || ((a.b_scale == 0.f || a.b_scale == 1.f) && !a.b_scale_dev);
        const bool unmasked_ok = (a.K % BK) == 0 && one_a && one_b && a.epi == 0 && !a.amax_out && !a.finite_flag;
        if constexpr (AMODE == A_CONV && BSPLIT == 1) {
            if (a.Ax) return unmasked_ok ? launch_cfg_u<BM, BN, WM, WN, AMODE, BMODE, PREC, BSPLIT, 1, 1>(a, st) : -1001;
        }
        if (unmasked_ok) return launch_cfg_u<BM, BN, WM, WN, AMODE, BMODE, PREC, BSPLIT, 1>(a, st);
    }
    if (a.Ax) return -1001;
    return launch_cfg_u<BM, BN, WM, WN, AMODE, BMODE, PREC, BSPLIT, 0>(a, st);
}

template <int BM, int BN, int WM, int WN, int AMODE, int BMODE, int PREC>
int launch_cfg(const GemmArgs& a, hipStream_t st) {
    constexpr bool CAN_BSPLIT = PREC == PREC_F16X3 && BMODE == B_N && (AMODE == A_N || AMODE == A_NADD || AMODE == A_CONV);
    if constexpr (CAN_BSPLIT) {
        if (a.b_split) return launch_cfg_b<BM, BN, WM, WN, AMODE, BMODE, PREC, 1>(a, st);
    }
    return launch_cfg_b<BM, BN, WM, WN, AMODE, BMODE, PREC, 0>(a, st);
}

double tile_cost(int M, int N, int K, int nz, int BM, int BN, double eff, double fixed) {
    const long tiles = (long)((M + BM - 1) / BM) * ((N + BN - 1) / BN) * nz;
    const long full = tiles / 512, f = tiles - full * 512;
    double rounds = 2.0 * full + (f == 0 ? 0.0 : (f <= 256 ? 1.0 : 1.0 + (double)(f - 256) / 256.0));
    if (tiles <= 256) rounds *= 1.3;
    const double nk = (double)((K + BK - 1) / BK);
    return rounds * ((double)BM * BN / (128.0 * 128.0)) * (fixed + nk / eff);
}

template <int AMODE, int BMODE, int PREC>
int launch_modes(const GemmArgs& a, hipStream_t st) {
    const int nz = a.groups > 0 ? a.groups : 1;
    const int Ks = a.splitk > 1 ? (a.K + a.splitk - 1) / a.splitk : a.K;
    const int nzs = nz * (a.splitk > 1 ? a.splitk : 1);
    const double fixed = PREC ? 10.0 : 2.5;
    const double cL = tile_cost(a.M, a.N, Ks, nzs, 128, 128, 1.00, fixed);
    const double cM = tile_cost(a.M, a.N, Ks, nzs, 128, 64, PREC ? ((AMODE == A_N || AMODE == A_T) ? 0.83 : 0.74) : 0.95, fixed);
    const double cS = tile_cost(a.M, a.N, Ks, nzs, 64, 64, PREC ? 0.68 : 0.88, fixed);
    double eL = -cL, eM = -cM, eS = -cS;
    if (!PREC) {
        auto eff = [&](int BM, int BN, double factor) {
            const long tiles = (long)((a.M + BM - 1) / BM) * ((a.N + BN - 1) / BN) * nzs;
            const long rounds = (tiles + 255) / 256;
            return factor * ((double)a.M * a.N * nzs) / ((double)rounds * 256 * BM * BN);
        };
        eL = eff(128, 128, 1.00); eM = eff(128, 64, 0.95); eS = eff(64, 64, 0.88);
    }
    static const std::string hints = getenv("ACTMI_TILE_HINTS") ? getenv("ACTMI_TILE_HINTS") : "";
    if (!hints.empty() && a.tile_hint == 0) {
        char key[64];
        snprintf(key, sizeof(key), "%d,%d,%d=", a.M, a.N, a.K);
        const size_t pos = hints.find(key);
        if (pos != std::string::npos && (pos == 0 || hints[pos - 1] == ';')) {
            const char c = hints[pos + strlen(key)];
            if (c == 'L') return launch_cfg<128, 128, 64, 64, AMODE, BMODE, PREC>(a, st);
            if (c == 'M') return launch_cfg<128, 64, 64, 32, AMODE, BMODE, PREC>(a, st);
            if (c == 'S') return launch_cfg<64, 64, 32, 32, AMODE, BMODE, PREC>(a, st);
        }
    }
    static const char* force = getenv("ACTMI_GEMM_CFG");
    if (force && force[0] == 'L') return launch_cfg<128, 128, 64, 64, AMODE, BMODE, PREC>(a, st);
    if (force && force[0] == 'M') return launch_cfg<128, 64, 64, 32, AMODE, BMODE, PREC>(a, st);
    if (force && force[0] == 'S') return launch_cfg<64, 64, 32, 32, AMODE, BMODE, PREC>(a, st);
    if (a.tile_hint == 1) return launch_cfg<128, 128, 64, 64, AMODE, BMODE, PREC>(a, st);
    if (a.tile_hint == 2) return launch_cfg<128, 64, 64, 32, AMODE, BMODE, PREC>(a, st);
    if (a.tile_hint == 3) return launch_cfg<64, 64, 32, 32, AMODE, BMODE, PREC>(a, st);
    if (eL >= eM && eL >= eS) return launch_cfg<128, 128, 64, 64, AMODE, BMODE, PREC>(a, st);
    if (eM >= eS) return launch_cfg<128, 64, 64, 32, AMODE, BMODE, PREC>(a, st);
    return launch_cfg<64, 64, 32, 32, AMODE, BMODE, PREC>(a, st);
}

}

#ifdef ACTMI_GEMM_TU_BF16
int launch_gemm_bf16(int amode, int bmode, bool has_add, const GemmArgs& a, hipStream_t st) {
    int rc;
#define ACTMI_DISPATCH(PREC)                                                                                       \
    if (amode == A_N && bmode == B_N && has_add) rc = launch_modes<A_NADD, B_N, PREC>(a, st);                      \
    else if (amode == A_N && bmode == B_N) rc = launch_modes<A_N, B_N, PREC>(a, st);                               \
    else if (amode == A_CONV && bmode == B_N) rc = launch_modes<A_CONV, B_N, PREC>(a, st);                         \
    else if (amode == A_DGRAD && bmode == B_N) rc = launch_modes<A_DGRAD, B_N, PREC>(a, st);                       \
    else if (amode == A_N && bmode == B_T) rc = launch_modes<A_N, B_T, PREC>(a, st);                               \
    else if (amode == A_T && bmode == B_T) rc = launch_modes<A_T, B_T, PREC>(a, st);                               \
    else if (amode == A_T && bmode == B_WGRAD) rc = launch_modes<A_T, B_WGRAD, PREC>(a, st);                       \
    else if (amode == A_T && bmode == B_N) rc = launch_modes<A_T, B_N, PREC>(a, st);                               \
    else rc = -1002;
    ACTMI_DISPATCH(PREC_BF16)
#undef ACTMI_DISPATCH
    return rc;
}
#else
int launch_gemm_bf16(int amode, int bmode, bool has_add, const GemmArgs& a, hipStream_t st);

int env_gemm_prec(int unset) {
    const char* e = getenv("ACTMI_GEMM_PREC");
    if (!e) return unset;
    return (e[0] == 'f' && e[1] == '3') ? ACTMI_PREC_F32 : ACTMI_PREC_F16X3;
}

int launch_gemm(const GemmArgs& a_in, hipStream_t st, std::string* err) {
    GemmArgs a = a_in;
    if (a.groups <= 0) a.groups = 1;
    if (a.M <= 0 || a.N <= 0) return 0;
    auto fail = [&](const char* m) { if (err) *err = std::string("gemm: ") + m; return -2; };
    if (a.K <= 0) return fail("K must be positive");
    if (((uintptr_t)a.A & 15) || ((uintptr_t)a.Bw & 15)) return fail("A/B must be 16-byte aligned");
    if (a.epi != 0) {
        if (a.epi != 1 && a.epi != 2) return fail("bad epi");
        if (!a.epi_row) return fail("epi needs epi_row");
        if (a.epi == 2 && !a.res) return fail("epi 2 needs res (the factor P)");
        if (a.rowmap) return fail("epi is not available with a row map");
        if (a.C2) return fail("epi is not available with a second output (C2)");
        if (a.drop_p > 0.f) return fail("epi is not available with dropout");
        if (a.res_mod != 0) return fail("epi is not available with res_mod");
        if (a.splitk > 1 && a.split_stride == 0) return fail("epi is not available with an atomic split-K");
        const int64_t lim = (int64_t)1 << 31, ldmask = a.ldmask ? a.ldmask : a.ldc;
        if ((int64_t)a.M * a.ldc >= lim || (a.res && (int64_t)a.M * a.ldres >= lim) || (a.mask && (int64_t)a.M * ldmask >= lim))
            return fail("epi needs M*ldc, M*ldres and M*ldmask below 2^31");
    }
    if (a.splitk > 1 && (a.bias || a.res || a.mask || a.relu || a.C2 || a.scale)) return fail("split-K supports a plain accumulate only");
    if (a.split_stride != 0) {
        if (a.splitk <= 1) return fail("split_stride needs splitk > 1");
        const int nk = (a.K + BK - 1) / BK, tps = (nk + a.splitk - 1) / a.splitk;
        if ((a.splitk - 1) * tps >= nk) return fail("split_stride: every split must own at least one K tile");
    }
    if (a.relu == 2 && (a.rowmap || a.C2 || a.drop_p > 0.f || a.res_mod != 0)) return fail("GELU is only available in the plain epilogue");
    if (a.relu < 0 || a.relu > 2) return fail("bad activation");
    if (a.C2 && !a.scale2) return fail("C2 needs scale2");
    int amode, bmode = a.tb;
    if (a.ta) {
        if (a.mode != 0) return fail("ta requires mode 0");
        if (a.lda & 3) return fail("lda must be a multiple of 4");
        if (a.A_add || a.a_rowmap) return fail("addend / row gather not supported with ta");
        amode = A_T;
    } else {
        if (a.mode == 0) {
            if (a.lda & 3) return fail("lda must be a multiple of 4");
            if ((a.K & 3) && a.lda < ((a.K + 3) & ~3)) return fail("K % 4 != 0 needs rows padded to a multiple of 4");
            if (a.A_add && ((a.ld_add & 3) || a.add_mod <= 0 || ((uintptr_t)a.A_add & 15))) return fail("bad addend");
            if (a.A_alt && (a.A_add || a.a_rowmap || (a.alt_ncols % 128) || ((uintptr_t)a.A_alt & 15))) return fail("A_alt: no addend / row gather, alt_ncols a multiple of 128");
            amode = A_N;
        } else if (a.mode == 1) {
            if (a.K & 3) return fail("K must be a multiple of 4");
            if (a.Cin & 3) return fail("Cin must be a multiple of 4");
            if (a.Ax) {
                if (a.kx_begin != a.KH * a.KW * a.Cin || a.K != a.kx_begin + a.Cx) return fail("second source: K must be KH*KW*Cin + Cx, kx_begin = KH*KW*Cin");
                if ((a.Cin % BK) || (a.Cx % BK) || a.KH * a.KW > 32) return fail("second source: Cin and Cx must be multiples of 32");
                if (a.stride_x < 1 || (a.Ho - 1) * a.stride_x >= a.Hx || (a.Wo - 1) * a.stride_x >= a.Wx) return fail("second source: the strided pixel grid leaves the map");
                const int64_t nimg = a.M / ((int64_t)a.Ho * a.Wo);
                if (nimg * a.Hx * a.Wx * a.Cx >= ((int64_t)1 << 31) || (int64_t)a.H * a.W * a.Cin >= ((int64_t)1 << 30)) return fail("second source: map too large for 32-bit offsets");
                if ((uintptr_t)a.Ax & 15) return fail("second source must be 16-byte aligned");
            } else if (a.K != a.KH * a.KW * a.Cin) return fail("K != KH*KW*Cin");
            if (a.A_add || a.a_rowmap) return fail("addend not supported in conv mode");
            if (a.M % (a.Ho * a.Wo)) return fail("M must be images*Ho*Wo");
            if (a.k_tap_inner && ((a.Cin % BK) || a.KH * a.KW > 32 || (int64_t)a.H * a.W * a.Cin >= ((int64_t)1 << 30)))
                return fail("k_tap_inner needs Cin % 32 == 0 (the uniform-tap loader)");
            amode = A_CONV;
        } else if (a.mode == 2) {
            if (a.K % (a.KH * a.KW) || ((a.K / (a.KH * a.KW)) & 3)) return fail("dgrad: K must be KH*KW*Cout, Cout % 4 == 0");
            if (a.M % (a.H * a.W)) return fail("dgrad: M must be images*H*W");
            amode = A_DGRAD;
        } else return fail("bad mode");
    }
    if (bmode == 0) {
        if ((a.ldb & 3) || (a.K & 3)) return fail("ldb and K must be multiples of 4 for a contraction-contiguous B");
    } else if (bmode == 1) {
        if (a.ldb & 3) return fail("ldb must be a multiple of 4");
        if (a.B_add && ((a.ld_badd & 3) || a.badd_mod <= 0)) return fail("bad B addend");
    } else if (bmode == 2) {
        if ((a.Cin & 3) || a.N != a.KH * a.KW * a.Cin) return fail("wgrad: N must be KH*KW*Cin, Cin % 4 == 0");
        if (a.K % (a.Ho * a.Wo)) return fail("wgrad: K must be images*Ho*Wo");
        if (!a.ta) return fail("wgrad: A (dY) must be given in [m][n] storage (ta=1)");
    } else return fail("bad tb");
    int rc;
    static const int env_prec = env_gemm_prec(ACTMI_PREC_DEFAULT_IS);
    const int prec = a.prec ? a.prec : env_prec;
    if (prec != ACTMI_PREC_F32 && prec != ACTMI_PREC_F16X3 && prec != ACTMI_PREC_BF16) return fail("bad prec");
    if (a.b_split && (prec != ACTMI_PREC_F16X3 || bmode != B_N || !(amode == A_N || amode == A_CONV)))
        return fail("b_split needs prec f16x3 and the forward operand forms");
#define ACTMI_DISPATCH(PREC)                                                                                       \
    if (amode == A_N && bmode == B_N && a.A_add) rc = launch_modes<A_NADD, B_N, PREC>(a, st);                      \
    else if (amode == A_N && bmode == B_N) rc = launch_modes<A_N, B_N, PREC>(a, st);                               \
    else if (amode == A_CONV && bmode == B_N) rc = launch_modes<A_CONV, B_N, PREC>(a, st);                         \
    else if (amode == A_DGRAD && bmode == B_N) rc = launch_modes<A_DGRAD, B_N, PREC>(a, st);                       \
    else if (amode == A_N && bmode == B_T) rc = launch_modes<A_N, B_T, PREC>(a, st);                               \
    else if (amode == A_T && bmode == B_T) rc = launch_modes<A_T, B_T, PREC>(a, st);                               \
    else if (amode == A_T && bmode == B_WGRAD) rc = launch_modes<A_T, B_WGRAD, PREC>(a, st);                       \
    else if (amode == A_T && bmode == B_N) rc = launch_modes<A_T, B_N, PREC>(a, st);                               \
    else return fail("operand form combination not instantiated");
    if (prec == ACTMI_PREC_BF16) {
        if (a.Ax) return fail("a second source (Ax) needs prec f16x3");
        rc = launch_gemm_bf16(amode, bmode, a.A_add != nullptr, a, st);
        if (rc == -1002) return fail("operand form combination not instantiated");
    } else if (prec == ACTMI_PREC_F16X3) { ACTMI_DISPATCH(PREC_F16X3) } else { ACTMI_DISPATCH(PREC_F32) }
#undef ACTMI_DISPATCH
    if (rc == -1001) return fail("a second source (Ax) needs prec f16x3, pre-split weights (b_split), K % 32 == 0 and a plain epilogue");
    if (rc != 0 && err) *err = std::string("gemm launch: ") + hipGetErrorString((hipError_t)rc);
    return rc == 0 ? 0 : -3;
}
#endif
```

include/actmi.h:

```cpp
#ifndef ACTMI_H
#define ACTMI_H

#include <stdint.h>

#ifdef __cplusplus
extern "C" {
#endif

#define ACTMI_VERSION 110

#define ACTMI_OK 0
#define ACTMI_E_INVALID (-1)
#define ACTMI_E_SHAPE (-2)
#define ACTMI_E_LAUNCH (-3)
#define ACTMI_E_STATE (-4)
#define ACTMI_E_NOMEM (-5)

#define ACTMI_IMG_U8_NHWC 0
#define ACTMI_IMG_F32_NCHW 1

typedef struct actmi_ctx* actmi_handle;

typedef struct actmi_config {
    uint32_t struct_size;
    int32_t num_cams;
    int32_t image_h, image_w;
    int32_t base_width;
    int32_t hidden_dim, nheads, dim_feedforward;
    int32_t enc_layers, dec_layers;
    int32_t num_queries, state_dim, action_dim, latent_dim;
    int32_t has_cvae_encoder;
    int32_t max_batch;
    int32_t enable_training;
    float kl_weight;
    int32_t vq, vq_class, vq_dim;
} actmi_config;

#define ACTMI_PREC_F32 1
#define ACTMI_PREC_F16X3 2
#define ACTMI_PREC_BF16 3

typedef struct actmi_gemm_desc {
    const float* A;
    int64_t lda;
    int32_t mode;
    int32_t H, W, Cin, KH, KW, stride, pad, Ho, Wo;
    int64_t img_stride;
    const float* A_add;
    int64_t ld_add;
    int32_t add_mod;
    int32_t add_ncols;
    const float* Bw;
    int64_t ldb;
    const float* scale;
    const float* bias;
    const float* res;
    int64_t ldres;
    int32_t res_mod;
    int32_t relu;
    float* C;
    int64_t ldc;
    const int32_t* rowmap;
    int32_t M, N, K;
    int32_t groups;
    int64_t gA, gB, gSB, gC, gRes;
    int32_t ta;
    int32_t tb;
    const int32_t* a_rowmap;
    const float* B_add;
    int64_t ld_badd;
    int32_t badd_mod;
    int32_t splitk;
    const float* mask;
    int64_t ldmask;
    float* C2;
    const float* scale2;
    float alpha;
    int32_t groups_inner;
    int64_t gA2, gB2, gC2, gRes2;
    int64_t gMask, gC2out;
    float drop_p;
    uint64_t drop_seed;
    uint64_t* stamps;
    int32_t prec;
    int32_t b_split;
    float b_scale;
    float a_scale;
    const float* a_scale_dev;
    const float* b_scale_dev;
    int64_t split_stride;
    uint32_t* amax_out;
    int32_t epi;
    float epi_scale;
    const float* epi_row;
    int64_t gRow, gRow2;
    const uint8_t* epi_colkill;
    int64_t gColkill;
    int32_t tile_hint;
    uint32_t* finite_flag;
    uint32_t finite_bit;
    const float* Ax;
    int32_t kx_begin, Hx, Wx, Cx, stride_x;
    int64_t gAx;
    const float* A_alt;
    int32_t alt_ncols;
    int32_t k_tap_inner;
} actmi_gemm_desc;

typedef struct actmi_attn_desc {
    const float* Q; int64_t q_bs, q_rs;
    const float* K; int64_t k_bs, k_rs;
    const float* V; int64_t v_bs, v_rs;
    float* O; int64_t o_bs, o_rs;
    const uint8_t* kpm; int64_t kpm_bs;
    float* lse;
    int32_t B, H, Nq, Nk, HD;
    float scale;
    float* ws;
    int64_t ws_floats;
    float drop_p;
    uint64_t drop_seed;
    int32_t prec;
    int32_t causal;
} actmi_attn_desc;

int actmi_version(void);

int actmi_create(const actmi_config* cfg, actmi_handle* out);

typedef struct actmi_pcd_config {
    uint32_t struct_size;
    int32_t max_points;
    int32_t hidden_dim;
    int32_t output_dim;
} actmi_pcd_config;
int actmi_create_ex(const actmi_config* cfg, const actmi_pcd_config* pcd, actmi_handle* out);
int actmi_set_pointcloud(actmi_handle h, const float* xyz, const float* rgb, int B, int P);
int actmi_destroy(actmi_handle h);
const char* actmi_last_error(actmi_handle h);

int actmi_num_params(actmi_handle h);
int actmi_param_info(actmi_handle h, int index, const char** key, int64_t* shape4, int* ndim, int* is_buffer);
int actmi_set_param(actmi_handle h, const char* key, const void* src, const int64_t* shape, int ndim, int is_device);
int actmi_get_param(actmi_handle h, const char* key, void* dst, int64_t nbytes, int is_device);
int actmi_param_ptr(actmi_handle h, const char* key, void** dev_ptr, int64_t* numel);
int actmi_finalize(actmi_handle h, void* stream);

int actmi_forward_infer(actmi_handle h, const float* qpos , const void* image, int image_fmt, int B,
                        float* a_hat , void* stream);

int actmi_set_forward_phase(actmi_handle h, int phase);

int actmi_forward_infer_vq(actmi_handle h, const float* qpos, const void* image, int image_fmt, int B,
                           const float* vq_sample, float* a_hat, void* stream);

int actmi_forward_train(actmi_handle h, const float* qpos, const void* image, int image_fmt,
                        const float* actions , const uint8_t* is_pad ,
                        const float* eps , uint64_t dropout_seed, float dropout_p, int B,
                        float* losses , float* a_hat, float* mu, float* logvar, void* stream);
int actmi_backward(actmi_handle h, float loss_scale, void* stream);
int actmi_zero_grad(actmi_handle h, void* stream);
int actmi_adamw_step(actmi_handle h, float lr, float lr_backbone, float weight_decay, float beta1, float beta2,
                     float eps, int64_t step, void* stream);
int actmi_adamw_step_range(actmi_handle h, float lr, float lr_backbone, float weight_decay, float beta1, float beta2,
                           float eps, int64_t step, int64_t offset, int64_t count, void* stream);
int actmi_refresh_weights(actmi_handle h, void* stream);
int actmi_param_arena(actmi_handle h, void** dev_ptr, int64_t* nfloats);
int actmi_grad_ptr(actmi_handle h, const char* key, void** dev_ptr, int64_t* numel);
int actmi_grad_arena(actmi_handle h, void** dev_ptr, int64_t* nfloats);

int actmi_grad_phase_range(actmi_handle h, int phase, int64_t* offset, int64_t* count);
int actmi_wait_grad_phase(actmi_handle h, int phase, void* stream);

int actmi_ensemble_step(float* ring, int32_t* tcount, const float* chunk, double k, double* out, uint8_t* populated,
                        int E, int Q, int A, void* stream);

int actmi_op_gemm(const actmi_gemm_desc* d, void* stream);
int actmi_op_split16(const float* src, float* dst, int64_t nfloats, float scale, void* stream);
int actmi_op_permute_conv_k(const float* src, float* dst, int64_t rows, int taps, int cin, int ld, void* stream);
int actmi_op_pow2_scale(const float* x, int64_t ld, int M, int N, float* out, void* stream);
int actmi_op_splitk_combine(const float* part, int nsplit, int64_t split_stride, int64_t ldp, int M, int N, const float* scale,
                            const float* bias, const float* res, int64_t ldres, int relu, float* out, int64_t ldc, void* stream);
int actmi_op_sample_onehot(const float* logits, int n, int V, float temperature, uint64_t seed, float* probs, float* code,
                           void* stream);
int actmi_op_attention(const actmi_attn_desc* d, void* stream);
typedef struct actmi_attn_bwd_desc {
    const float *q, *k, *v, *o, *d_o, *lse;
    float *dq, *dk, *dv;
    int64_t q_bs, q_rs, k_bs, k_rs, v_bs, v_rs, dq_bs, dq_rs, dk_bs, dk_rs, dv_bs, dv_rs;
    const uint8_t* kpm;
    int64_t kpm_bs;
    int32_t B, H, Nq, Nk, HD;
    float drop_p;
    uint64_t drop_seed;
    float* delta_ws;
    const float* do_scale;
    uint32_t* amax_out;
} actmi_attn_bwd_desc;
int actmi_op_attention_bwd(const actmi_attn_bwd_desc* d, void* stream);
int actmi_op_layernorm(const float* x, const float* res, int res_mod, const float* w, const float* b, const float* w2,
                       const float* b2, float* y, int M, int D, float eps, void* stream);
int actmi_op_maxpool3x3s2(const float* in_nhwc, float* out_nhwc, int nimg, int H, int W, int C, void* stream);
int actmi_op_conv1(const void* image, int image_fmt, const float* w_oihw, const float* scale, const float* bias,
                   float* out, float* workspace , int B, int C, int H, int W, int Cout,
                   int prec , void* stream);
int64_t actmi_op_conv1_workspace_floats(int C, int Cout);
int actmi_op_conv1_prepare(const float* w_oihw, float* workspace, int C, int Cout, int lut_mode, void* stream);
int actmi_op_conv1_prepared(const void* image_u8, const float* workspace, const float* scale, const float* bias, float* out,
                            int B, int C, int H, int W, int Cout, int relu, void* stream);
int actmi_op_conv3x3_c64(const float* x, const float* w16, float w_scale, const float* scale, const float* bias,
                         const float* res, float* out, int G, int B, int H, int W, int relu, void* stream);
int actmi_op_conv3x3_c64_dgrad(const float* dy, const float* w16, float w_scale, const float* dy_scale_dev, const float* res,
                               const float* mask, const float* post_scale, uint32_t* amax_out, float* dx, int G, int B, int H,
                               int W, void* stream);
int actmi_op_wgrad3x3_c64(const float* dy, const float* x, float* dw, float* ws, int64_t ws_floats, const float* dy_scale_dev, int G,
                          int B, int H, int W, void* stream);

int actmi_op_wgrad7x7s2(const float* dy, const float* x4, float* dw, float* ws, int64_t ws_floats, const float* dy_scale_dev, int G,
                        int B, int H, int W, void* stream);

int actmi_op_groupnorm(const float* x, const float* res, const float* film_scale, const float* film_bias, const float* w,
                       const float* b, float* out, int n, int P, int C, int G, float eps, int act, int res_mode, float* ws,
                       int64_t ws_floats, void* stream);
int actmi_op_spatial_softmax(const float* logits, float* out, int n, int H, int W, int K, float temperature, void* stream);
int actmi_op_unfold1d(const float* x, float* out, int B, int T, int C, int k, int stride, int pad, int To, int transposed,
                      void* stream);
int actmi_op_ddim_step(float* x, const float* eps, int64_t n, float inv_sqrt_at, float sqrt_1m_at, float sqrt_aprev,
                       float sqrt_1m_aprev, int clip, void* stream);
int actmi_op_mish(const float* x, float* y, int64_t n, void* stream);
int actmi_op_u8_to_nhwc4(const uint8_t* image, float* out, int B, int Cam, int H, int W, void* stream);
int actmi_op_gelu(const float* x, float* y, int64_t n, void* stream);
int actmi_op_gelu_bwd(const float* x, const float* dy, float* dx, int64_t n, void* stream);
int actmi_op_dropout(const float* x, float* y, int64_t n, float p, uint64_t seed, void* stream);
int actmi_op_small_attention(const float* qkv, float* out, int n, int T, int H, int HD, int causal, float drop_p, uint64_t seed,
                             void* stream);
int actmi_op_small_attention_bwd(const float* qkv, const float* dout, float* dqkv, int n, int T, int H, int HD, int causal,
                                 float drop_p, uint64_t seed, void* stream);
int actmi_op_soft_ce_dim1(const float* logits, const float* target, int B, int T, int V, float* loss, float* dlogits, float* ws,
                          void* stream);
int actmi_op_argmax_l1(const float* logits, const float* target, int rows, int V, float* out, float* ws, void* stream);
int actmi_op_layernorm_bwd(const float* x, const float* w, const float* dy, const float* dx_add, float* dx, float* dw, float* db,
                           int M, int D, float eps, float* ws, int64_t ws_floats, void* stream);
int actmi_op_colsum(const float* src, int64_t ld, float* out, int M, int N, float* ws, int64_t ws_floats, void* stream);
int actmi_op_pcd_embed(const float* xyz, const float* rgb, const float* w0, const float* b0, float* out, int64_t rows, int H,
                       void* stream);
int actmi_op_colmax(const float* x, int B, int P, int O, int64_t ld, float* out, int32_t* argmax, float* ws, int64_t ws_floats,
                    void* stream);
int actmi_op_sum_batch(const float* src, int64_t batch_stride, int64_t ld, float* dst, int B, int R, int D, int accumulate,
                       void* stream);
int actmi_op_adamw(float* p, const float* g, float* m, float* v, int64_t n, float lr, float weight_decay, float beta1, float beta2,
                   float eps, int64_t step, void* stream);
const char* actmi_op_last_error(void);

int actmi_debug_tensor(actmi_handle h, const char* name, const float** dev_ptr, int64_t* numel);
int actmi_debug_stop_after(actmi_handle h, const char* stage);
int actmi_set_gemm_prec(actmi_handle h, int prec);
int actmi_set_train_prec(actmi_handle h, int prec);

#define ACTMI_FLAG_OUTPUT 1u
#define ACTMI_FLAG_WEIGHT 2u
#define ACTMI_FLAG_LOSS 4u
int actmi_get_flags(actmi_handle h, uint32_t* host_flags, int clear, void* stream);
int actmi_flags_ptr(actmi_handle h, void** dev_ptr);

int actmi_profile_enable(int on);
int actmi_profile_reset(void);
int actmi_profile_report(char* buf, int buflen);

#ifdef __cplusplus
}
#endif
#endif
```

Before: 1788 policy steps/s.

## Emit pre-split fp16 K/V from projection GEMM and use transposed LDS reads in attention

The QKV and cross-attention KV projection GEMMs can now write K/V columns already split into fp16 hi/lo halves in their epilogue, so the f16x3 attention kernel skips its own split step when loading K and V tiles. The attention kernel also stores V row-major in LDS and reads it through ds_read_tr16 transposed loads, replacing the scattered transposed packing writes. The tradeoff is a slightly costlier GEMM epilogue, a split-K fast path that is disabled for these projections, and a tile_hint that may be forced when D is not a multiple of 128.

Result: no change. 1799 policy steps/s, median of 6 (+0.6%).

```diff
diff --git a/act-plus-plus_amd/actmi/lib.py b/act-plus-plus_amd/actmi/lib.py
--- a/act-plus-plus_amd/actmi/lib.py
+++ b/act-plus-plus_amd/actmi/lib.py
@@ -48,6 +48,7 @@
         ("Ax", C.c_void_p), ("kx_begin", C.c_int32), ("Hx", C.c_int32), ("Wx", C.c_int32), ("Cx", C.c_int32),
         ("stride_x", C.c_int32), ("gAx", C.c_int64),
         ("A_alt", C.c_void_p), ("alt_ncols", C.c_int32), ("k_tap_inner", C.c_int32),
+        ("c_split", C.c_int32), ("c_split_begin", C.c_int32),
     ]
 
 
@@ -69,6 +70,7 @@
         ("B", C.c_int32), ("H", C.c_int32), ("Nq", C.c_int32), ("Nk", C.c_int32), ("HD", C.c_int32),
         ("scale", C.c_float), ("ws", C.c_void_p), ("ws_floats", C.c_int64),
         ("drop_p", C.c_float), ("drop_seed", C.c_uint64), ("prec", C.c_int32), ("causal", C.c_int32),
+        ("kv_split", C.c_int32),
     ]
 
 
diff --git a/act-plus-plus_amd/actmi/ops.py b/act-plus-plus_amd/actmi/ops.py
--- a/act-plus-plus_amd/actmi/ops.py
+++ b/act-plus-plus_amd/actmi/ops.py
@@ -52,7 +52,7 @@
 
 def gemm(A, W, bias=None, scale=None, res=None, res_mod=0, relu=False, a_add=None, add_mod=0, add_ncols=0, rowmap=None,
          out=None, out_rows=None, drop_p=0.0, drop_seed=0, prec=None, w_split=False, a_scale=0.0, b_scale=0.0,
-         a_scale_dev=None, b_scale_dev=None, splitk=0):
+         a_scale_dev=None, b_scale_dev=None, splitk=0, c_split_begin=None):
     lib = L.load()
     M, K = A.shape
     N = W.shape[0]
@@ -60,7 +60,7 @@
         splitk = auto_splitk(M, N, K) if (rowmap is None and not res_mod and not drop_p and N % 4 == 0 and a_scale_dev is None
                                           and b_scale_dev is None) else 0
     if splitk and splitk > 1:
-        assert rowmap is None and not res_mod and not drop_p
+        assert rowmap is None and not res_mod and not drop_p and c_split_begin is None
         part = torch.empty((splitk, M, N), dtype=torch.float32, device=A.device)
         d = L.GemmDesc()
         d.A, d.lda, d.mode = A.data_ptr(), A.stride(0), 0
@@ -100,6 +100,8 @@
     d.a_scale = float(a_scale)
     d.a_scale_dev = a_scale_dev.data_ptr() if a_scale_dev is not None else None
     d.b_scale_dev = b_scale_dev.data_ptr() if b_scale_dev is not None else None
+    if c_split_begin is not None:
+        d.c_split, d.c_split_begin = 1, int(c_split_begin)
     L.check(lib.actmi_op_gemm(C.byref(d), L.current_stream_ptr()), None, "op_gemm")
     return out
 
@@ -260,7 +262,7 @@
 
 
 def attention(q, k, v, nheads, kpm=None, q_shared=False, want_lse=False, split=True, drop_p=0.0, drop_seed=0, prec=None,
-              causal=False):
+              causal=False, kv_split=False):
     lib = L.load()
     B, Nk, D = k.shape
     Nq = q.shape[-2]
@@ -283,6 +285,7 @@
     d.drop_p, d.drop_seed = float(drop_p), int(drop_seed)
     d.prec = PREC[prec]
     d.causal = 1 if causal else 0
+    d.kv_split = 1 if kv_split else 0
     L.check(lib.actmi_op_attention(C.byref(d), L.current_stream_ptr()), None, "op_attention")
     return (out, lse) if want_lse else out
 
diff --git a/act-plus-plus_amd/csrc/attn.hip b/act-plus-plus_amd/csrc/attn.hip
--- a/act-plus-plus_amd/csrc/attn.hip
+++ b/act-plus-plus_amd/csrc/attn.hip
@@ -206,15 +206,24 @@
     }
 }
 
-template <int HD>
+typedef short i16x4 __attribute__((ext_vector_type(4)));
+typedef short i16x8 __attribute__((ext_vector_type(8)));
+typedef __attribute__((address_space(3))) i16x4 lds_i16x4;
+__device__ __forceinline__ h16x8 lds_read_tr16x8(const unsigned char* a0, const unsigned char* a1) {
+    const i16x4 x = __builtin_amdgcn_ds_read_tr16_b64_v4i16((lds_i16x4*)a0);
+    const i16x4 y = __builtin_amdgcn_ds_read_tr16_b64_v4i16((lds_i16x4*)a1);
+    return __builtin_bit_cast(h16x8, __builtin_shufflevector(x, y, 0, 1, 2, 3, 4, 5, 6, 7));
+}
+
+template <int HD, bool KVS>
 __global__ __launch_bounds__(256, 3) void attn_f16x3_kernel(AttnArgs p, int nsplit, int chunk) {
     constexpr int NS = HD / 16;
     constexpr int DT = (HD + 31) / 32;
     constexpr int VD = DT * 32;
     constexpr int KROW = 4 * HD + 16;
-    constexpr int VROW = 4 * KT + 16;
+    constexpr int VROW = 4 * VD + 64;
     __shared__ __attribute__((aligned(16))) unsigned char s_k[KT * KROW];
-    __shared__ __attribute__((aligned(16))) unsigned char s_vt[VD * VROW];
+    __shared__ __attribute__((aligned(16))) unsigned char s_v[KT * VROW];
     __shared__ uint8_t s_dead[KT];
 
     const int t = threadIdx.x, lane = t & 63, wave = t >> 6;
@@ -254,16 +263,14 @@
     float m_run = -INFINITY, l_run = 0.f;
 
     if (HD < VD) {
-        for (int e = t; e < VD * VROW / 4; e += 256) reinterpret_cast<uint32_t*>(s_vt)[e] = 0u;
+        for (int e = t; e < KT * VROW / 4; e += 256) reinterpret_cast<uint32_t*>(s_v)[e] = 0u;
         __syncthreads();
     }
+    const unsigned char* vtr = s_v + (4 * lh + ((lane & 15) >> 2)) * VROW + (lane & 16) * 2 + (lane & 3) * 8;
 
     constexpr int C4 = HD / 4;
     constexpr int NLK = (KT * C4 + 255) / 256;
-    constexpr int NLV = (KT / 2 * C4 + 255) / 256;
-    f32x4 pk[NLK], pv[NLV][2];
-    auto vc = [&](int e) { return ((e >> 5) % (C4 / 4)) * 4 + (e & 3); };
-    auto vkp = [&](int e) { return ((e >> 5) / (C4 / 4)) * 8 + ((e >> 2) & 7); };
+    f32x4 pk[NLK], pv[NLK];
     auto fetch = [&](int kt0) {
         const f32x4 z = {0.f, 0.f, 0.f, 0.f};
 #pragma unroll
@@ -273,20 +280,17 @@
             const int key = kt0 + kr;
             const bool ok = e < KT * C4 && key < k_end;
             const f32x4 kv = *reinterpret_cast<const f32x4*>(Kb + (ok ? (int64_t)key * p.k_rs + c * 4 : 0));
+            const f32x4 vv = *reinterpret_cast<const f32x4*>(Vb + (ok ? (int64_t)key * p.v_rs + c * 4 : 0));
             pk[i] = ok ? kv : z;
-        }
-#pragma unroll
-        for (int i = 0; i < NLV; ++i) {
-            const int e = t + 256 * i;
-            const int kp = vkp(e), c = vc(e);
-#pragma unroll
-            for (int u = 0; u < 2; ++u) {
-                const int key = kt0 + 2 * kp + u;
-                const bool ok = e < KT / 2 * C4 && key < k_end;
-                const f32x4 vv = *reinterpret_cast<const f32x4*>(Vb + (ok ? (int64_t)key * p.v_rs + c * 4 : 0));
-                pv[i][u] = ok ? vv : z;
-            }
-        }
+            pv[i] = ok ? vv : z;
+        }
+    };
+    auto pieces = [](const f32x4 v, uint2& hi, uint2& lo) {
+        if (KVS) {
+            const uint4 u = __builtin_bit_cast(uint4, v);
+            hi = uint2{u.x, u.y};
+            lo = uint2{u.z, u.w};
+        } else split16(v, hi, lo);
     };
     if (!ATTN_NOPF) fetch(k_begin);
     for (int kt0 = k_begin; kt0 < k_end; kt0 += KT) {
@@ -297,33 +301,15 @@
             if (e < KT * C4) {
                 const int kr = e / C4, c = e - kr * C4;
                 uint2 hi, lo;
-                split16(pk[i], hi, lo);
+                pieces(pk[i], hi, lo);
                 *reinterpret_cast<uint2*>(s_k + kr * KROW + c * 8) = hi;
                 *reinterpret_cast<uint2*>(s_k + kr * KROW + 2 * HD + c * 8) = lo;
+                pieces(pv[i], hi, lo);
+                *reinterpret_cast<uint2*>(s_v + kr * VROW + c * 8) = hi;
+                *reinterpret_cast<uint2*>(s_v + kr * VROW + 2 * VD + c * 8) = lo;
             }
         }
-#pragma unroll
-        for (int i = 0; i < NLV; ++i) {
-            const int e = t + 256 * i;
-            if (e < KT / 2 * C4) {
-                const int kp = vkp(e), c = vc(e);
-                uint2 ha, la, hb, lb;
-                split16(pv[i][0], ha, la);
-                split16(pv[i][1], hb, lb);
-                const int kl = 2 * kp, r = kl & 15;
-                const int pos = (kl & ~15) | (r & 3) | ((r & 8) >> 1) | ((r & 4) << 1);
-                unsigned char* dst = s_vt + (c * 4) * VROW + pos * 2;
-                *reinterpret_cast<uint32_t*>(dst + 0 * VROW) = (ha.x & 0xffffu) | (hb.x << 16);
-                *reinterpret_cast<uint32_t*>(dst + 1 * VROW) = (ha.x >> 16) | (hb.x & 0xffff0000u);
-                *reinterpret_cast<uint32_t*>(dst + 2 * VROW) = (ha.y & 0xffffu) | (hb.y << 16);
-                *reinterpret_cast<uint32_t*>(dst + 3 * VROW) = (ha.y >> 16) | (hb.y & 0xffff0000u);
-                *reinterpret_cast<uint32_t*>(dst + 0 * VROW + 2 * KT) = (la.x & 0xffffu) | (lb.x << 16);
-                *reinterpret_cast<uint32_t*>(dst + 1 * VROW + 2 * KT) = (la.x >> 16) | (lb.x & 0xffff0000u);
-                *reinterpret_cast<uint32_t*>(dst + 2 * VROW + 2 * KT) = (la.y & 0xffffu) | (lb.y << 16);
-                *reinterpret_cast<uint32_t*>(dst + 3 * VROW + 2 * KT) = (la.y >> 16) | (lb.y & 0xffff0000u);
-            }
-        }
-        const bool ragged = kt0 + KT > k_end || kpm != nullptr;
+    const bool ragged = kt0 + KT > k_end || kpm != nullptr;
         if (ragged && t < KT) {
             const int key = kt0 + t;
             s_dead[t] = (key >= k_end) || (kpm && kpm[key] != 0);
@@ -396,11 +382,11 @@
                 for (int d = 0; d < DT; ++d) {
 #pragma unroll
                     for (int e = 0; e < 16; ++e) O[d][e] *= alpha;
-                    const unsigned char* vrow = s_vt + (d * 32 + li) * VROW + sub * 64 + lh * 16;
 #pragma unroll
                     for (int g2 = 0; g2 < 2; ++g2) {
-                        const h16x8 vh = __builtin_bit_cast(h16x8, *reinterpret_cast<const f32x4*>(vrow + g2 * 32));
-                        const h16x8 vl = __builtin_bit_cast(h16x8, *reinterpret_cast<const f32x4*>(vrow + 2 * KT + g2 * 32));
+                        const unsigned char* vblk = vtr + (sub * 32 + g2 * 16) * VROW + d * 64;
+                        const h16x8 vh = lds_read_tr16x8(vblk, vblk + 8 * VROW);
+                        const h16x8 vl = lds_read_tr16x8(vblk + 2 * VD, vblk + 8 * VROW + 2 * VD);
                         O[d] = __builtin_amdgcn_mfma_f32_32x32x16_f16(vl, ph[g2], O[d], 0, 0, 0);
                         O[d] = __builtin_amdgcn_mfma_f32_32x32x16_f16(vh, pl[g2], O[d], 0, 0, 0);
                         O[d] = __builtin_amdgcn_mfma_f32_32x32x16_f16(vh, ph[g2], O[d], 0, 0, 0);
@@ -488,6 +474,7 @@
     const int prec = a.prec ? a.prec : env_prec;
     if (prec != ACTMI_PREC_F32 && prec != ACTMI_PREC_F16X3) return fail("bad prec");
     const bool f16 = prec == ACTMI_PREC_F16X3;
+    if (a.kv_split && !f16) return fail("kv_split needs prec f16x3");
     const int qblocks = (a.Nq + 127) / 128;
     const int tiles = (a.Nk + KT - 1) / KT;
     int nsplit = 1;
@@ -508,11 +495,18 @@
         prof_begin(nm, 4.0 * a.B * a.H * (double)a.Nq * a.Nk * a.HD,
                    4.0 * a.B * a.H * a.HD * (2.0 * a.Nq + 2.0 * a.Nk), st);
     }
-    if (f16) {
+    if (f16 && a.kv_split) {
         switch (a.HD) {
-            case 64: hipLaunchKernelGGL(attn_f16x3_kernel<64>, grid, dim3(256), 0, st, a, nsplit, chunk); break;
-            case 32: hipLaunchKernelGGL(attn_f16x3_kernel<32>, grid, dim3(256), 0, st, a, nsplit, chunk); break;
-            case 16: hipLaunchKernelGGL(attn_f16x3_kernel<16>, grid, dim3(256), 0, st, a, nsplit, chunk); break;
+            case 64: hipLaunchKernelGGL((attn_f16x3_kernel<64, true>), grid, dim3(256), 0, st, a, nsplit, chunk); break;
+            case 32: hipLaunchKernelGGL((attn_f16x3_kernel<32, true>), grid, dim3(256), 0, st, a, nsplit, chunk); break;
+            case 16: hipLaunchKernelGGL((attn_f16x3_kernel<16, true>), grid, dim3(256), 0, st, a, nsplit, chunk); break;
+            default: return fail("head_dim must be 16, 32 or 64");
+        }
+    } else if (f16) {
+        switch (a.HD) {
+            case 64: hipLaunchKernelGGL((attn_f16x3_kernel<64, false>), grid, dim3(256), 0, st, a, nsplit, chunk); break;
+            case 32: hipLaunchKernelGGL((attn_f16x3_kernel<32, false>), grid, dim3(256), 0, st, a, nsplit, chunk); break;
+            case 16: hipLaunchKernelGGL((attn_f16x3_kernel<16, false>), grid, dim3(256), 0, st, a, nsplit, chunk); break;
             default: return fail("head_dim must be 16, 32 or 64");
         }
     } else
diff --git a/act-plus-plus_amd/csrc/engine.hip b/act-plus-plus_amd/csrc/engine.hip
--- a/act-plus-plus_amd/csrc/engine.hip
+++ b/act-plus-plus_amd/csrc/engine.hip
@@ -153,7 +153,7 @@
     constexpr int sk_target = 1536, sk_minnk = 12, sk_maxtiles = 768;
     constexpr int sk_target_long = 4864, sk_maxtiles_long = 1300, sk_long_nk = 128;
     if (ctx->fwd_splitk && ctx->splitk_ws && a.splitk <= 1 && a.tb == 0 && a.ta == 0 && (a.mode == 0 || a.mode == 1) &&
-        !a.rowmap && !a.C2 && !a.mask && a.drop_p == 0.f && a.res_mod == 0 && a.groups_inner == 0 && !a.stamps) {
+        !a.c_split && !a.rowmap && !a.C2 && !a.mask && a.drop_p == 0.f && a.res_mod == 0 && a.groups_inner == 0 && !a.stamps) {
         const int groups = a.groups > 0 ? a.groups : 1;
         const int64_t tiles = (int64_t)((a.M + 63) / 64) * ((a.N + 63) / 64) * groups * (ws_half >= 0 ? ctx->policy_mult : 1);
         const int nk = (a.K + 31) / 32;
@@ -982,6 +982,14 @@
     return v;
 }
 
+static bool engine_kv_split(const actmi_ctx* ctx, int D, GemmArgs* proj) {
+    if (engine_prec(ctx) != ACTMI_PREC_F16X3 || ctx->gemm_prec != ACTMI_PREC_F16X3) return false;
+    if (D % 128 == 0) return true;
+    if (D % 64 != 0) return false;
+    if (proj->tile_hint == 0) proj->tile_hint = 3;
+    return proj->tile_hint == 3;
+}
+
 int engine_encoder_layer(actmi_ctx* ctx, const EncW& w, const TView& V, const float* pos, int B, int n, const uint8_t* kpm,
                          hipStream_t st, bool xp_in, bool xp_out) {
     float* x = V.X;
@@ -990,8 +998,11 @@
     GemmArgs qkv = linear_args(x, D, M, D, w.attn.in_w, 3 * D, w.attn.in_b, V.QKV, 3 * D);
     if (xp_in) { qkv.A_alt = V.XP; qkv.alt_ncols = 2 * D; }
     else { qkv.A_add = pos; qkv.ld_add = D; qkv.add_mod = n; qkv.add_ncols = 2 * D; }
+    const bool kvs = engine_kv_split(ctx, D, &qkv);
+    if (kvs) { qkv.c_split = 1; qkv.c_split_begin = D; }
     CHK(ctx_gemm(ctx, qkv, st, V.half));
     AttnArgs at = packed_self_attn_args(ctx, V.QKV, V.ATT, B, n);
+    at.kv_split = kvs;
     at.kpm = kpm;
     at.ws = V.attn_ws; at.ws_floats = V.attn_ws_floats;
     at.prec = ctx->gemm_prec;
@@ -1024,8 +1035,11 @@
     GemmArgs kv = linear_args(V.X, D, B * N, D, d.cross.in_w + (int64_t)D * D, 2 * D, d.cross.in_b + D, KV, 2 * D);
     if (xp_in) { kv.A_alt = V.XP; kv.alt_ncols = D; }
     else { kv.A_add = ctx->pos_tokens; kv.ld_add = D; kv.add_mod = N; kv.add_ncols = D; }
+    const bool kvs = engine_kv_split(ctx, D, &kv);
+    if (kvs) { kv.c_split = 1; kv.c_split_begin = 0; }
     CHK(ctx_gemm(ctx, kv, st, V.half));
     AttnArgs at = cross_attn_args(ctx, ctx->dec_q, false, KV, V.dO, B);
+    at.kv_split = kvs;
     at.ws = V.attn_ws; at.ws_floats = V.attn_ws_floats;
     at.prec = ctx->gemm_prec;
     CHK(launch_attention(at, st, &ctx->err));
diff --git a/act-plus-plus_amd/csrc/gemm.hip b/act-plus-plus_amd/csrc/gemm.hip
--- a/act-plus-plus_amd/csrc/gemm.hip
+++ b/act-plus-plus_amd/csrc/gemm.hip
@@ -39,7 +39,7 @@
 
 __device__ __forceinline__ f32x4 ld4(const float* p) { return *reinterpret_cast<const f32x4*>(p); }
 
-template <int BM, int BN, int WM, int WN, int AMODE, int BMODE, int PREC, int BSPLIT, int UNMASKED, int XS = 0>
+template <int BM, int BN, int WM, int WN, int AMODE, int BMODE, int PREC, int BSPLIT, int UNMASKED, int XS = 0, int CS = 0>
 __global__ __launch_bounds__((BM / WM) * (BN / WN) * 64, (PREC && BM * BN <= 128 * 64 && (AMODE == 0  || AMODE == 3 ) && !(AMODE == 0 && BMODE == 1)) ? 3 : 2)
     void gemm_f32_kernel(GemmArgs p, int tiles_m, int tiles_n) {
     constexpr int NT = (BM / WM) * (BN / WN) * 64;
@@ -757,6 +757,11 @@
 #pragma unroll
                             for (int e = 0; e < 4; ++e) v[e] = 0.5f * v[e] * (1.f + erff(v[e] * 0.70710678118654752f));
                         }
+                        if (CS && n0 >= p.c_split_begin) {
+                            uint2 hi, lo;
+                            split16(v, hi, lo);
+                            v = __builtin_bit_cast(f32x4, uint4{hi.x, hi.y, lo.x, lo.y});
+                        }
                         *reinterpret_cast<f32x4*>(C + (uint32_t)(m * (int)p.ldc + ncol)) = v;
                         if (track) {
 #pragma unroll
@@ -864,12 +869,12 @@
     if (stamp && threadIdx.x == 0) stamp[3] = __builtin_amdgcn_s_memtime();
 }
 
-template <int BM, int BN, int WM, int WN, int AMODE, int BMODE, int PREC, int BSPLIT, int UNMASKED, int XS = 0>
+template <int BM, int BN, int WM, int WN, int AMODE, int BMODE, int PREC, int BSPLIT, int UNMASKED, int XS = 0, int CS = 0>
 int launch_cfg_u(const GemmArgs& a, hipStream_t st) {
     const int tiles_m = (a.M + BM - 1) / BM, tiles_n = (a.N + BN - 1) / BN;
     static const int lds_pad = getenv("ACTMI_GEMM_LDSPAD") ? atoi(getenv("ACTMI_GEMM_LDSPAD")) : 0;
     const int smem = 2 * stage_f4<BM, BN, PREC>() * 16 + lds_pad;
-    auto kern = gemm_f32_kernel<BM, BN, WM, WN, AMODE, BMODE, PREC, BSPLIT, UNMASKED, XS>;
+    auto kern = gemm_f32_kernel<BM, BN, WM, WN, AMODE, BMODE, PREC, BSPLIT, UNMASKED, XS, CS>;
     static bool attr_set = false;
     if (!attr_set) {
         hipError_t e = hipFuncSetAttribute(reinterpret_cast<const void*>(kern),
@@ -910,8 +915,12 @@
         if constexpr (AMODE == A_CONV && BSPLIT == 1) {
             if (a.Ax) return unmasked_ok ? launch_cfg_u<BM, BN, WM, WN, AMODE, BMODE, PREC, BSPLIT, 1, 1>(a, st) : -1001;
         }
+        if constexpr (PREC == PREC_F16X3 && (AMODE == A_N || AMODE == A_NADD)) {
+            if (a.c_split) return (unmasked_ok && a.N % BN == 0 && a.c_split_begin % BN == 0) ? launch_cfg_u<BM, BN, WM, WN, AMODE, BMODE, PREC, BSPLIT, 1, 0, 1>(a, st) : -1003;
+        }
         if (unmasked_ok) return launch_cfg_u<BM, BN, WM, WN, AMODE, BMODE, PREC, BSPLIT, 1>(a, st);
     }
+    if (a.c_split) return -1003;
     if (a.Ax) return -1001;
     return launch_cfg_u<BM, BN, WM, WN, AMODE, BMODE, PREC, BSPLIT, 0>(a, st);
 }
@@ -1082,6 +1091,19 @@
     static const int env_prec = env_gemm_prec(ACTMI_PREC_DEFAULT_IS);
     const int prec = a.prec ? a.prec : env_prec;
     if (prec != ACTMI_PREC_F32 && prec != ACTMI_PREC_F16X3 && prec != ACTMI_PREC_BF16) return fail("bad prec");
+    if (a.c_split) {
+        auto shape = [&](const char* m) { if (err) *err = std::string("gemm: c_split ") + m; return ACTMI_E_SHAPE; };
+        if (prec != ACTMI_PREC_F16X3) return shape("needs prec f16x3");
+        if (a.c_split_begin < 0 || a.c_split_begin > a.N) return shape("needs 0 <= c_split_begin <= N");
+        if (a.rowmap || a.C2 || a.drop_p > 0.f || a.res_mod != 0 || a.splitk > 1 || a.epi != 0 || a.mask || a.amax_out || a.finite_flag ||
+            a.groups_inner > 0)
+            return shape("is not available with a row map, C2, dropout, res_mod, a mask, split-K, epi, amax_out, finite_flag or groups_inner");
+        if ((a.ldc & 3) || ((uintptr_t)a.C & 15) || (a.gC & 3) || (a.res && ((a.ldres & 3) || ((uintptr_t)a.res & 15) || (a.gRes & 3))) ||
+            ((uintptr_t)a.scale & 15) || ((uintptr_t)a.bias & 15) || (a.gSB & 3))
+            return shape("needs 16-byte aligned C / res / scale / bias and ldc / ldres multiples of 4");
+        if ((int64_t)a.M * a.ldc >= ((int64_t)1 << 31) || (a.res && (int64_t)a.M * a.ldres >= ((int64_t)1 << 31)))
+            return shape("needs M*ldc and M*ldres below 2^31");
+    }
     if (a.b_split && (prec != ACTMI_PREC_F16X3 || bmode != B_N || !(amode == A_N || amode == A_CONV)))
         return fail("b_split needs prec f16x3 and the forward operand forms");
 #define ACTMI_DISPATCH(PREC)                                                                                       \
@@ -1100,6 +1122,9 @@
         if (rc == -1002) return fail("operand form combination not instantiated");
     } else if (prec == ACTMI_PREC_F16X3) { ACTMI_DISPATCH(PREC_F16X3) } else { ACTMI_DISPATCH(PREC_F32) }
 #undef ACTMI_DISPATCH
+    if (rc == -1003)
+        return fail("c_split needs the row-major forward form (mode 0, ta = tb = 0) with K % 32 == 0 and no operand pre-scales, N a whole "
+                    "number of column tiles and c_split_begin on a tile boundary");
     if (rc == -1001) return fail("a second source (Ax) needs prec f16x3, pre-split weights (b_split), K % 32 == 0 and a plain epilogue");
     if (rc != 0 && err) *err = std::string("gemm launch: ") + hipGetErrorString((hipError_t)rc);
     return rc == 0 ? 0 : -3;
diff --git a/include/actmi.h b/include/actmi.h
--- a/include/actmi.h
+++ b/include/actmi.h
@@ -105,6 +105,8 @@
     const float* A_alt;
     int32_t alt_ncols;
     int32_t k_tap_inner;
+    int32_t c_split;
+    int32_t c_split_begin;
 } actmi_gemm_desc;
 
 typedef struct actmi_attn_desc {
@@ -122,6 +124,7 @@
     uint64_t drop_seed;
     int32_t prec;
     int32_t causal;
+    int32_t kv_split;
 } actmi_attn_desc;
 
 int actmi_version(void);
```
